# sonbui25/Multimodal-Aspect-Category-Sentiment-Analysis

Hardware: AMD Instinct MI355X
Metric: train samples/sec (fwd+bwd+step) FCMF seq128x36ROI (higher is better)
Workload: dtype bf16; 1 GPU; FCMF-base fine-tune step, BASELINE configs[1]: batch 64 reviews x 6 aspects per GPU, seq 128, 7 images x (49 patches + 36 ROIs), precomputed ResNet-152 features, dropout 0.1, clip 1.0 + 4-group AdamW + linear schedule; global_batch=64, per_gpu_batch=64, seq_len=128, parallelism=dp1, sample_unit=1 review = 6 aspect forwards

## Files before the change

### include/fcmf_hip.h

```cpp
#ifndef FCMF_HIP_H
#define FCMF_HIP_H
#include <stdint.h>

#ifdef __cplusplus
extern "C" {
#endif

#define FCMF_OK 0
#define FCMF_ERR_ARG (-1)
#define FCMF_ERR_LAUNCH (-2)
#define FCMF_ERR_UNSUPPORTED (-3)
#define FCMF_ERR_COMM (-4)

#define FCMF_F32 0
#define FCMF_BF16 1
#define FCMF_F64 2

#define FCMF_EPI_NONE 0
#define FCMF_EPI_GELU 1
#define FCMF_EPI_TANH 2
#define FCMF_EPI_DGELU 3
#define FCMF_EPI_DTANH 4
#define FCMF_EPI_ADD 5

int fcmf_abi_version(void);
const char* fcmf_build_info(void);

typedef struct fcmf_gemm_ctx fcmf_gemm_ctx;
int fcmf_gemm_ctx_create(fcmf_gemm_ctx** ctx);
int fcmf_gemm_ctx_destroy(fcmf_gemm_ctx* ctx);
int fcmf_gemm_ctx_set_workspace(fcmf_gemm_ctx* ctx, void* ptr, int64_t bytes);
int fcmf_gemm_ctx_tune(fcmf_gemm_ctx* ctx, int force_tile, int kb, int num_cus, int64_t nt_min_bytes);
const char* fcmf_gemm_ctx_last_kernel(const fcmf_gemm_ctx* ctx);

int fcmf_gemm(fcmf_gemm_ctx* ctx, const void* A, const void* B, void* C, const float* bias, void* aux, float* colsum,
              int M, int N, int K, int64_t lda, int64_t ldb, int64_t ldc,
              int trans_a, int trans_b, int in_dtype, int out_dtype,
              int epilogue, int accumulate, void* stream);

int fcmf_quant_fp8_rows(const void* x, int64_t ldx, void* q, int64_t ldq, float* scale, int rows, int K, int dtype, void* stream);
int fcmf_gemm_fp8(fcmf_gemm_ctx* ctx, const void* A, const float* sa, const void* B, const float* sb, void* C,
                  const float* bias, void* aux, float* colsum, int M, int N, int K, int64_t lda, int64_t ldb, int64_t ldc,
                  int epilogue, void* stream);

int fcmf_colsum(const void* X, float* out, int M, int N, int64_t ldx, int dtype,
                int accumulate, void* stream);

typedef struct {
  int dtype, G, heads, d, R, T1, T2, group_div;
  int64_t q_sg, q_sr, k1_sg, k1_st, k2_sg, k2_sr, k2_st, o_sg, o_sr;
  const void *q, *k1, *v1, *k2, *v2;
  const float* mask;
  const float* bias;
  float scale, dropout_p;
  uint64_t seed;
  int causal, head_quirk;
} fcmf_attn_desc;

int fcmf_attn_small_fwd(const fcmf_attn_desc* desc , void* out, float* lse, void* stream);
int fcmf_attn_small_bwd(const fcmf_attn_desc* desc , const void* out, const void* dout,
                        const float* lse, void* dq, void* dk1, void* dv1, void* dk2, void* dv2,
                        float* dbias, void* stream);
int fcmf_attn_small_bwd_grouped(const fcmf_attn_desc* desc, const void* out, const void* dout,
                                const float* lse, void* dq, void* dk1, void* dv1, void* dk2, void* dv2,
                                float* dbias, float* scratch, int64_t scratch_bytes, void* stream);

int fcmf_attn_mfma_fwd(const void* q, const void* k, const void* v, const float* mask,
                       void* out, float* lse, int G, int heads, int Tq, int Tk,
                       int64_t ldq, int64_t ldk, int64_t ldo, float scale,
                       float dropout_p, uint64_t seed, void* stream);
int fcmf_attn_mfma_bwd(const void* q, const void* k, const void* v, const float* mask,
                       const void* out, const void* dout, const float* lse,
                       void* dq, void* dk, void* dv, int G, int heads, int Tq, int Tk,
                       int64_t ldq, int64_t ldk, int64_t ldo, float scale,
                       float dropout_p, uint64_t seed, float* colsum, void* stream);

int fcmf_attn_probs(const fcmf_attn_desc* desc , float* probs, int64_t p_sg, int64_t p_sh, void* stream);
int fcmf_attn_mfma_probs(const void* q, const void* k, const float* mask, float* probs, int G, int heads,
                         int Tq, int Tk, int64_t ldq, int64_t ldk, int64_t p_sg, int64_t p_sh,
                         float scale, void* stream);

int fcmf_add_ln_fwd(const void* x, const void* res, int64_t res_stride, const float* gamma,
                    const float* beta, void* y, void* z, float* mean, float* rstd,
                    int rows, int H, float eps, float dropout_p, uint64_t seed, int dtype,
                    void* stream);
int fcmf_add_ln_bwd(const void* dy, const void* z, const float* gamma, const float* mean,
                    const float* rstd, void* dz, void* dx, float* dgamma, float* dbeta, float* dxsum,
                    float* workspace, int rows, int H, float dropout_p, uint64_t seed, int dtype,
                    void* stream);
int fcmf_add_ln_fwd_fp8(const void* x, const void* res, int64_t res_stride, const float* gamma, const float* beta, void* y,
                        void* z, float* mean, float* rstd, int rows, int H, float eps, float dropout_p, uint64_t seed,
                        int dtype, void* q8, float* qscale, void* stream);
int fcmf_add_ln_bwd_fp8(const void* dy, const void* z, const float* gamma, const float* mean, const float* rstd, void* dz,
                        void* dx, float* dgamma, float* dbeta, float* dxsum, float* workspace, int rows, int H,
                        float dropout_p, uint64_t seed, int dtype, void* q8, float* qscale, void* stream);
int64_t fcmf_add_ln_bwd_workspace(int rows, int H);

int fcmf_position_ids(const int64_t* ids, int64_t* pos, int nseq, int S, int pad_id, void* stream);
int fcmf_embed_ln_fwd(const int64_t* ids, const int64_t* pos, const int64_t* type_ids,
                      const float* word, const float* pos_table, const float* type_table,
                      const float* gamma, const float* beta, void* y, void* z, float* mean,
                      float* rstd, int ntok, int H, float eps, float dropout_p, uint64_t seed,
                      int dtype, void* stream);
int fcmf_embed_bwd(const void* dz, const int64_t* ids, const int64_t* pos, const int64_t* type_ids,
                   float* dword, float* dpos, float* dtype_table, int ntok, int H, int pad_id,
                   int dtype, void* stream);
int fcmf_embed_pos_bwd(const void* dz, const int64_t* pos, float* dpos, int nseq, int S, int H, int pad_id,
                       int dtype, void* stream);
int fcmf_embed_pos_type_bwd(const void* dz, const int64_t* pos, const int64_t* type_ids, float* dpos,
                            float* dtype_table, int nseq, int S, int H, int pad_id, int dtype, void* stream);

#define FCMF_BOX_FAST_TRIG 0x100
int fcmf_box_bias_fwd(const void* coords, int coord_dtype, const float* dim_mat, const float* wg_w,
                      const float* wg_b, float* bias, int G, int N, int heads, void* stream);
int fcmf_box_bias_bwd(const void* coords, int coord_dtype, const float* dim_mat, const float* wg_w,
                      const float* wg_b, const float* dbias, float* dwg_w, float* dwg_b, int G, int N,
                      int heads, void* stream);
int fcmf_box_embedding(const void* coords, int coord_dtype, const float* dim_mat, float* emb, int G,
                       int N, void* stream);

int fcmf_xent_fwd(const void* logits, int64_t ld, const int64_t* labels, float* loss_rows,
                  float* nvalid, int n, int C, int64_t ignore_index, int dtype, void* stream);
int fcmf_xent_bwd(const void* logits, int64_t ld, const int64_t* labels, void* dlogits,
                  int64_t ldd, const float* scale_ptr, float extra_scale, int n, int C,
                  int64_t ignore_index, int dtype, void* stream);

int fcmf_xent_mean(const float* loss_rows, const int64_t* labels, int n, int64_t ignore_index,
                   float mult, float* out2, void* stream);

int fcmf_bce_logits(const void* logits, int64_t ld, const float* target, int64_t ldt, int n, int C, const float* dloss,
                    float* loss, void* dlogits, int64_t ldd, float* probs, int dtype, void* stream);

int fcmf_additive_mask(const int64_t* mask, int64_t ld, float* out, int rows, int cols, float value,
                       void* stream);

int fcmf_cast(const void* src, void* dst, int64_t n, int src_dtype, int dst_dtype, void* stream);
int fcmf_cast_transpose(const float* src, void* dst, int rows, int cols, void* stream);
int fcmf_multi_cast_transpose(const int64_t* src_ptrs, const int64_t* dst_ptrs, const int32_t* dims,
                              const int32_t* tile_desc, int ntiles, void* stream);
int fcmf_dropout(const void* x, void* y, int64_t n, float p, uint64_t seed, int dtype, void* stream);
int fcmf_act_bwd(const void* dy, const void* aux, void* out, int64_t n, int kind, int dtype,
                 void* stream);
int fcmf_sum_axis(const void* in, void* out, int64_t outer, int reps, int64_t inner, int dtype,
                  void* stream);

int fcmf_embed_scale_fwd(const int64_t* ids, const float* weight, const float* pos_table, void* out, int n, int H, int S,
                         int64_t V, float scale, int dtype, void* stream);
int fcmf_embed_scale_bwd(const void* dy, const int64_t* ids, float* dweight, int n, int H, int64_t V, int32_t* oob_count,
                         float scale, int dtype, void* stream);
int fcmf_head_gather(const void* slot, void* out, int64_t ldo, int G, int T, int heads, int d, int dtype, void* stream);

int fcmf_multi_sumsq(const int64_t* g_ptrs, const int64_t* sizes, const int32_t* chunk_tensor,
                     const int64_t* chunk_offset, int nchunks, int chunk_size,
                     double* sumsq , double* per_tensor ,
                     void* stream);
int fcmf_multi_adamw(const int64_t* p_ptrs, const int64_t* g_ptrs, const int64_t* m_ptrs,
                     const int64_t* v_ptrs, const int64_t* bf16_ptrs, const int64_t* sizes,
                     const int32_t* group_of, const int32_t* chunk_tensor,
                     const int64_t* chunk_offset, int nchunks, int chunk_size,
                     const float* lr , const float* wd , int ngroups,
                     float beta1, float beta2, float eps, int step, const double* sumsq,
                     float max_norm, void* stream);
int fcmf_bertadam(float* p, const float* g, float* m, float* v, int64_t n, float lr_scheduled,
                  float beta1, float beta2, float eps, float weight_decay, float max_grad_norm,
                  double* scratch, void* stream);

int fcmf_conv_im2col(const void* src, int src_dtype, void* dst, int dst_dtype, int N, int H, int W, int C,
                     int64_t sn, int64_t sh, int64_t sw, int64_t sc, int kh, int kw, int stride, int pad,
                     int Kpad, void* stream);
int64_t fcmf_bn_stats_workspace(int64_t rows_per_group, int groups, int C);
int fcmf_bn_stats(const void* x, double* sums, int64_t rows_per_group, int groups, int C, int dtype, void* stream);
int fcmf_bn_finalize(const double* sums, const float* gamma, const float* beta, float* running_mean,
                     float* running_var, float* scale, float* shift, float* mean_out, float* rstd_out, int C,
                     int groups, int64_t count, float momentum, float eps, void* stream);
int fcmf_bn_apply(const void* x, const void* res, void* y, const float* scale, const float* shift, int64_t rows,
                  int C, int64_t rows_per_group, int relu, int dtype, void* stream);
int fcmf_bn_apply_pad(const void* x, const void* res, void* y_padded, const float* scale, const float* shift,
                      int64_t rows, int C, int64_t rows_per_group, int relu, int H, int W, int pad, int dtype, void* stream);
int fcmf_bn_finalize_apply(const void* x, const void* res, void* y, const double* sums, const float* gamma, const float* beta,
                           float* running_mean, float* running_var, float* mean_out, float* rstd_out, int C, int groups,
                           int64_t rows_per_group, float momentum, float eps, int relu, int H, int W, int pad, int dtype, void* stream);
int fcmf_conv_gemm(fcmf_gemm_ctx* ctx, const void* x, const void* w, void* y, int n, int Hp, int Wp, int C, int Ho, int Wo,
                   int kh, int kw, int stride, int Cout, void* stream);
int fcmf_gemm_colblocks(fcmf_gemm_ctx* ctx, const void* A, const void* B, float* C, int M, int N, int K, int64_t lda,
                        int64_t ldb, int64_t ldc, int trans_a, int trans_b, int col_block, int64_t col_block_stride,
                        int accumulate, void* stream);

int fcmf_gemm_dw_batched(fcmf_gemm_ctx* ctx, int count, const void* const* A, const void* const* B, void* const* C, int M, int N, int K,
                         int64_t lda, int64_t ldb, int64_t ldc, int accumulate, void* stream);
int fcmf_conv_gemm_runs(fcmf_gemm_ctx* ctx, const void* x, const void* w, void* y, float* stats, int n, int Hp, int Wp, int pix, int run,
                        int Ho, int Wo, int kh, int stride, int Cout, void* stream);
int fcmf_pack_rgb0(const void* src, int src_dtype, void* dst, int N, int H, int W, int64_t sn, int64_t sh, int64_t sw, int64_t sc,
                   int pad, int Wp, void* stream);
int fcmf_gemm_colstats(fcmf_gemm_ctx* ctx, const void* A, const void* B, void* C, float* stats, int M, int N, int K, int64_t lda,
                       int64_t ldb, int64_t ldc, void* stream);
int fcmf_conv_gemm_colstats(fcmf_gemm_ctx* ctx, const void* x, const void* w, void* y, float* stats, int n, int Hp, int Wp, int C,
                            int Ho, int Wo, int kh, int kw, int stride, int Cout, void* stream);
int fcmf_gemm_colstats_block_rows(const fcmf_gemm_ctx* ctx, int M, int N, int K);
int fcmf_bn_stats_blocks(const float* blockstats, double* sums, int64_t rows_per_group, int groups, int C, int block_rows, void* stream);
int fcmf_maxpool3x3s2(const void* x, void* y, int N, int H, int W, int C, int dtype, void* stream);
int fcmf_adaptive_avgpool(const void* x, float* y, int N, int H, int W, int C, int oh, int ow, int layout,
                          int dtype, void* stream);

int fcmf_bn_bwd(const void* g, const void* z, const void* y, const float* mean, const float* rstd, const float* gamma,
                double* sums, void* dy, void* gres, float* dgamma, float* dbeta, int64_t rows_per_group, int groups,
                int C, int training, int dtype, void* stream);
int fcmf_conv_col2im(const void* dA, void* dX, int N, int H, int W, int C, int kh, int kw, int stride, int pad,
                     int Kpad, int dtype, void* stream);
int fcmf_maxpool3x3s2_bwd(const void* x, const void* dy, void* dx, int N, int H, int W, int C, int dtype, void* stream);
int fcmf_adaptive_avgpool_bwd(const float* dy, void* dx, int N, int H, int W, int C, int oh, int ow, int layout,
                              int dtype, void* stream);

typedef struct {
  int64_t offset;
  int H, W;
  int64_t sC, sH, sW;
  int r0, r1, c0, c1;
  int flip, reserved;
} fcmf_crop_desc;

int fcmf_crop_resize_normalize(const uint8_t* src, int64_t src_bytes, const fcmf_crop_desc* descs, int n, int max_rows, int S,
                               const float* mean, const float* std, float* scratch, int64_t scratch_bytes, void* out,
                               int dtype, void* stream);

#define FCMF_DP_UNIQUE_ID_BYTES 128
int fcmf_dp_unique_id(void* out_host);
int fcmf_dp_comm_create(void** comm, const void* unique_id_host, int nranks, int rank);
int fcmf_dp_comm_destroy(void* comm);
int fcmf_dp_allreduce_bucket(void* comm, void* buf, int64_t count, int dtype, int average, void* stream);

#ifdef __cplusplus
}
#endif
#endif
```

### multimodal-aspect-category-sentiment-analysis_amd/csrc/gemm.hip

```cpp
#include "common.h"
#include <cstdio>

struct GemmParams {
  const void* A; const void* B; void* C; const float* bias; void* aux;
  int M, N, K;
  int64_t lda, ldb, ldc;
  int epilogue, accumulate, ksplit, ktiles_per_split;
  unsigned a_bytes, b_bytes;
  unsigned c_bytes;
  float* colsum;
  int tiles, total_items;
  float* ws;
  int nt_out;
  const float* sa; const float* sb;
  int cv_C, cv_logC, cv_Hp, cv_Wp, cv_Ho, cv_Wo, cv_kw, cv_inv_kw, cv_stride;
  float* colstats;
  int cv_logP;
  int tiles_per_mat;
};
constexpr int BATCH_MAX = 32;
struct BatchPtrs { const void* A[BATCH_MAX]; const void* B[BATCH_MAX]; void* C[BATCH_MAX]; };

__device__ __forceinline__ int64_t conv_row_base(const GemmParams& p, int row) {
  const int hw = p.cv_Ho * p.cv_Wo, n = row / hw, rem = row - n * hw, oy = rem / p.cv_Wo, ox = rem - oy * p.cv_Wo;
// ... 1082 lines not shown
  int kchunk;
};

template <typename TI, typename TC>
__global__ __launch_bounds__(256) void gemm_generic_kernel(GenericParams p) {
  constexpr int GT = 64, GK = 16, LDT = GT + 4;
  __shared__ float As[GK][LDT];
  __shared__ float Bs[GK][LDT];
  const int tid = threadIdx.x, lane = tid & 63, wave = tid >> 6;
  const int wm = wave >> 1, wn = wave & 1;
  const int i0 = blockIdx.y * GT, j0 = blockIdx.x * GT;
  const TI* A = reinterpret_cast<const TI*>(p.A);
  const TI* B = reinterpret_cast<const TI*>(p.B);
  const bool a_kfast = (p.a_sk == 1), b_kfast = (p.b_sk == 1);

  f32x4 acc[2][2];
#pragma unroll
  for (int a = 0; a < 2; ++a)
#pragma unroll
    for (int b = 0; b < 2; ++b) acc[a][b] = f32x4{0.f, 0.f, 0.f, 0.f};

  const int kbeg = p.kchunk > 0 ? blockIdx.z * p.kchunk : 0;
  const int kend = p.kchunk > 0 ? min(p.K, kbeg + p.kchunk) : p.K;
  for (int k0 = kbeg; k0 < kend; k0 += GK) {
#pragma unroll
    for (int it = 0; it < 4; ++it) {
      int e = tid + 256 * it;
      int ia, ka, jb, kb;
      if (a_kfast) { ka = e & 15; ia = e >> 4; } else { ia = e & 63; ka = e >> 6; }
      if (b_kfast) { kb = e & 15; jb = e >> 4; } else { jb = e & 63; kb = e >> 6; }
      float va = 0.f, vb = 0.f;
      if (i0 + ia < p.M && k0 + ka < kend) va = to_f32<TI>(A[(int64_t)(i0 + ia) * p.a_si + (int64_t)(k0 + ka) * p.a_sk]);
      if (j0 + jb < p.N && k0 + kb < kend) vb = to_f32<TI>(B[(int64_t)(j0 + jb) * p.b_sj + (int64_t)(k0 + kb) * p.b_sk]);
      As[ka][ia] = va;
      Bs[kb][jb] = vb;
    }
    __syncthreads();
#pragma unroll
    for (int k4 = 0; k4 < GK / 4; ++k4) {
      float a[2], b[2];
#pragma unroll
      for (int f = 0; f < 2; ++f) {
        a[f] = As[k4 * 4 + (lane >> 4)][wm * 32 + f * 16 + (lane & 15)];
        b[f] = Bs[k4 * 4 + (lane >> 4)][wn * 32 + f * 16 + (lane & 15)];
      }
#pragma unroll
      for (int fi = 0; fi < 2; ++fi)
#pragma unroll
        for (int fj = 0; fj < 2; ++fj)
          acc[fi][fj] = __builtin_amdgcn_mfma_f32_16x16x4f32(a[fi], b[fj], acc[fi][fj], 0, 0, 0);
    }
    __syncthreads();
  }
  TC* C = reinterpret_cast<TC*>(p.C);
  TC* AUX = reinterpret_cast<TC*>(p.aux);
#pragma unroll
  for (int fi = 0; fi < 2; ++fi)
#pragma unroll
    for (int fj = 0; fj < 2; ++fj)
#pragma unroll
      for (int r = 0; r < 4; ++r) {
        int i = i0 + wm * 32 + fi * 16 + (lane >> 4) * 4 + r;
        int j = j0 + wn * 32 + fj * 16 + (lane & 15);
        if (i >= p.M || j >= p.N) continue;
        float v = acc[fi][fj][r];
        if (p.bias) v += p.bias[j];
        int64_t off = (int64_t)i * p.ldc + j;
        if (p.epilogue != FCMF_EPI_NONE) {
          float a = 0.f;
          if (p.epilogue == FCMF_EPI_GELU) { if (AUX) AUX[off] = from_f32<TC>(v); }
          else if (p.epilogue != FCMF_EPI_TANH) a = to_f32<TC>(AUX[off]);
          v = apply_epilogue(v, p.epilogue, a);
        }
        if constexpr (sizeof(TC) == 4) {
          if (p.kchunk > 0) { atomicAdd(reinterpret_cast<float*>(C) + off, v); continue; }
        }
        if (p.accumulate) v += to_f32<TC>(C[off]);
        C[off] = from_f32<TC>(v);
        if (p.colsum) atomicAdd(p.colsum + j, v);
      }
}

template <typename T>
__global__ __launch_bounds__(256) void colsum_kernel(const T* __restrict__ X, float* __restrict__ out, int M, int N,
                                                     int64_t ldx, int rows_per_block, int vec) {
  __shared__ float4 red[4][64];
  const int lane = threadIdx.x & 63, wave = threadIdx.x >> 6;
  const int col = blockIdx.x * 256 + lane * 4;
  const int r0 = blockIdx.y * rows_per_block;
  const int r1 = min(M, r0 + rows_per_block);
  float4 s = make_float4(0.f, 0.f, 0.f, 0.f);
  if (vec && col + 3 < N) {
    int r = r0 + wave;
    for (; r + 12 < r1; r += 16) {
      const float4 v0 = Vec4<T>::load(X + (int64_t)r * ldx + col), v1 = Vec4<T>::load(X + (int64_t)(r + 4) * ldx + col);
      const float4 v2 = Vec4<T>::load(X + (int64_t)(r + 8) * ldx + col), v3 = Vec4<T>::load(X + (int64_t)(r + 12) * ldx + col);
      s.x += (v0.x + v1.x) + (v2.x + v3.x); s.y += (v0.y + v1.y) + (v2.y + v3.y);
      s.z += (v0.z + v1.z) + (v2.z + v3.z); s.w += (v0.w + v1.w) + (v2.w + v3.w);
    }
    for (; r < r1; r += 4) {
      const float4 v = Vec4<T>::load(X + (int64_t)r * ldx + col);
      s.x += v.x; s.y += v.y; s.z += v.z; s.w += v.w;
    }
  } else if (col < N) {
    for (int r = r0 + wave; r < r1; r += 4) {
      const T* p = X + (int64_t)r * ldx + col;
      s.x += to_f32<T>(p[0]);
      if (col + 1 < N) s.y += to_f32<T>(p[1]);
      if (col + 2 < N) s.z += to_f32<T>(p[2]);
      if (col + 3 < N) s.w += to_f32<T>(p[3]);
    }
  }
  red[wave][lane] = s;
  __syncthreads();
  if (wave == 0 && col < N) {
    const float4 a = red[0][lane], b = red[1][lane], c = red[2][lane], d = red[3][lane];
    atomicAdd(out + col, a.x + b.x + c.x + d.x);
    if (col + 1 < N) atomicAdd(out + col + 1, a.y + b.y + c.y + d.y);
    if (col + 2 < N) atomicAdd(out + col + 2, a.z + b.z + c.z + d.z);
    if (col + 3 < N) atomicAdd(out + col + 3, a.w + b.w + c.w + d.w);
  }
}

template <bool A_TR, bool B_TR, typename TC, int EPI>
__global__ __launch_bounds__(512, 1) void gemm_bf16_tile256_kernel(GemmParams p) {
  gemm_bf16_tile256_body<A_TR, B_TR, TC, EPI, 8, 32>(p);
}
__global__ __launch_bounds__(512, 1) void gemm_bf16_tile256k64_n128_kernel(GemmParams p) {
  gemm_bf16_tile256_body<false, false, bf16_t, FCMF_EPI_NONE, 4, 64, false, false, 2>(p);
}
__global__ __launch_bounds__(512, 1) void gemm_bf16_tile256k64_n64_kernel(GemmParams p) {
  gemm_bf16_tile256_body<false, false, bf16_t, FCMF_EPI_NONE, 2, 64, false, false, 1>(p);
}
__global__ __launch_bounds__(512, 1) void gemm_bf16_dw_batched_kernel(GemmParams p, BatchPtrs bp) {
  gemm_bf16_tile256_body<true, true, float, FCMF_EPI_NONE, 8, 32, false, true>(p, &bp);
}
template <bool B_TR, int EPI>
__global__ __launch_bounds__(512, 1) void gemm_bf16_tile192_kernel(GemmParams p) {
  gemm_bf16_tile256_body<false, B_TR, bf16_t, EPI, 6, 32>(p);
}
template <int EPI>
__global__ __launch_bounds__(512, 1) void gemm_bf16_tile256k64_kernel(GemmParams p) {
  gemm_bf16_tile256_body<false, false, bf16_t, EPI, 8, 64>(p);
}
template <int EPI>
__global__ __launch_bounds__(512, 1) void gemm_bf16_tile192k64_kernel(GemmParams p) {
  gemm_bf16_tile256_body<false, false, bf16_t, EPI, 6, 64>(p);
}

template <int EPI>
__global__ __launch_bounds__(512, 1) void gemm_fp8_tile192_kernel(GemmParams p) {
  gemm_bf16_tile256_body<false, false, bf16_t, EPI, 6, 64, true>(p);
}

__global__ __launch_bounds__(256) void splitk_reduce_frag_kernel(const float* __restrict__ ws, float* __restrict__ C, int M, int N,
                                                                 int64_t ldc, int ksplit, int tiles, int tiles_n, int accumulate,
                                                                 int cblk, int64_t cblk_stride) {
  const int64_t total = (int64_t)tiles * (GB * GB / 4);
  for (int64_t i = (int64_t)blockIdx.x * 256 + threadIdx.x; i < total; i += (int64_t)gridDim.x * 256) {
    const int tile = (int)(i >> 14), r = (int)(i & 16383);
    const int lane = r & 63, frag = (r >> 6) & 31, wave = r >> 11;
    const int fj = frag >> 3, fi = frag & 7, wm = wave >> 2, wn = wave & 3;
    const int row = (tile / tiles_n) * GB + wm * 128 + fi * 16 + (lane & 15);
    const int col = (tile % tiles_n) * GB + wn * 64 + fj * 16 + (lane >> 4) * 4;
    if (row >= M || col >= N) continue;
    float* c = cblk ? C + (int64_t)(col / cblk) * cblk_stride + (int64_t)row * ldc + (col % cblk) : C + (int64_t)row * ldc + col;
    f32x4 s = accumulate ? *reinterpret_cast<const f32x4*>(c) : f32x4{0.f, 0.f, 0.f, 0.f};
#pragma unroll 4
    for (int z = 0; z < ksplit; ++z) s += *reinterpret_cast<const f32x4*>(ws + ((int64_t)z * tiles + tile) * (GB * GB) + (int64_t)r * 4);
    *reinterpret_cast<f32x4*>(c) = s;
  }
}

__global__ __launch_bounds__(256) void splitk_reduce_frag_batched_kernel(const float* __restrict__ ws, BatchPtrs bp, int tiles_per_mat, int M,
                                                                         int N, int64_t ldc, int ksplit, int tiles, int tiles_n,
                                                                         int accumulate) {
  const int64_t total = (int64_t)tiles * (GB * GB / 4);
  for (int64_t i = (int64_t)blockIdx.x * 256 + threadIdx.x; i < total; i += (int64_t)gridDim.x * 256) {
    const int tile = (int)(i >> 14), r = (int)(i & 16383);
    const int b = tile / tiles_per_mat, local = tile - b * tiles_per_mat;
    const int lane = r & 63, frag = (r >> 6) & 31, wave = r >> 11;
    const int fj = frag >> 3, fi = frag & 7, wm = wave >> 2, wn = wave & 3;
    const int row = (local / tiles_n) * GB + wm * 128 + fi * 16 + (lane & 15);
    const int col = (local % tiles_n) * GB + wn * 64 + fj * 16 + (lane >> 4) * 4;
    if (row >= M || col >= N) continue;
    float* c = reinterpret_cast<float*>(bp.C[b]) + (int64_t)row * ldc + col;
    f32x4 s = accumulate ? *reinterpret_cast<const f32x4*>(c) : f32x4{0.f, 0.f, 0.f, 0.f};
#pragma unroll 4
    for (int z = 0; z < ksplit; ++z) s += *reinterpret_cast<const f32x4*>(ws + ((int64_t)z * tiles + tile) * (GB * GB) + (int64_t)r * 4);
    *reinterpret_cast<f32x4*>(c) = s;
  }
}

__global__ __launch_bounds__(256) void splitk_reduce_kernel(const float* __restrict__ ws, float* __restrict__ C, int M, int N,
                                                            int64_t ldc, int ksplit, int accumulate) {
  const int64_t total4 = (int64_t)M * N / 4;
  for (int64_t i = (int64_t)blockIdx.x * 256 + threadIdx.x; i < total4; i += (int64_t)gridDim.x * 256) {
    const int64_t e = i * 4, row = e / N, col = e - row * N;
    f32x4 s = accumulate ? *reinterpret_cast<const f32x4*>(C + row * ldc + col) : f32x4{0.f, 0.f, 0.f, 0.f};
#pragma unroll 4
    for (int z = 0; z < ksplit; ++z) s += *reinterpret_cast<const f32x4*>(ws + (int64_t)z * M * N + e);
    *reinterpret_cast<f32x4*>(C + row * ldc + col) = s;
  }
}
// ... 552 lines not shown
    for (int i = 0; i < count; ++i) {
      a.A = A[i]; a.B = B[i]; a.C = C[i];
      const int rc = gemm_impl(ctx, a, stream);
      if (rc != FCMF_OK) return rc;
    }
    return FCMF_OK;
  }
  const int tpm = ((M + GB - 1) / GB) * ((N + GB - 1) / GB), nk = (K + 31) / 32;
  const int chunks = (count + BATCH_MAX - 1) / BATCH_MAX;
  for (int c = 0, first = 0; c < chunks; ++c) {
    const int n = (count - first + (chunks - c) - 1) / (chunks - c);
    BatchPtrs bp{};
    for (int i = 0; i < n; ++i) { bp.A[i] = A[first + i]; bp.B[i] = B[first + i]; bp.C[i] = C[first + i]; }
    a.A = bp.A[0]; a.B = bp.B[0]; a.C = bp.C[0];
    GemmPlan pl;
    plan_begin(&pl, a, GK_DW_BATCHED);
    pl.tm = 256; pl.batch = &bp;
    pl.p = base_params(a, 2);
    pl.p.c_bytes = 0;
    pl.p.tiles_per_mat = tpm;
    const int tiles = n * tpm;
    plan_persistent_launch(&pl, persistent_list(cfg, pl.p, tiles, nk, batched_ksplit(cfg, tiles, nk), false));
    if (pl.p.ksplit > 1) { pl.p.ws = cfg.ws; plan_frag_reduce(&pl, RED_FRAG_BATCHED); }
    snprintf(pl.name, sizeof pl.name, "gemm_bf16_dw_batched_kernel");
    const int rc = run_named(ctx, pl, stream);
    if (rc != FCMF_OK) return rc;
    first += n;
  }
  return FCMF_OK;
}

struct ConvShape { int n, Hp, Wp, C, Ho, Wo, kh, kw, stride, Cout; };
static int conv_gemm_impl(fcmf_gemm_ctx* ctx, const void* x, const void* w, void* y, float* colstats, const ConvShape& s, void* stream) {
  const int n = s.n, Hp = s.Hp, Wp = s.Wp, C = s.C, Ho = s.Ho, Wo = s.Wo, kh = s.kh, kw = s.kw, stride = s.stride, Cout = s.Cout;
  if (!x || !w || !y || n <= 0 || Hp <= 0 || Wp <= 0 || C <= 0 || Ho <= 0 || Wo <= 0 || kh <= 0 || kw <= 0 || stride <= 0 || Cout <= 0)
    return FCMF_ERR_ARG;
  if ((C & (C - 1)) || C < 64 || kh * kw > 64) return FCMF_ERR_UNSUPPORTED;
  if ((Ho - 1) * stride + kh > Hp || (Wo - 1) * stride + kw > Wp) return FCMF_ERR_ARG;
  const int64_t in_bytes = (int64_t)n * Hp * Wp * C * 2, M = (int64_t)n * Ho * Wo;
  if (in_bytes >= (1ll << 31) || M >= (1ll << 31)) return FCMF_ERR_UNSUPPORTED;
  int logC = 0;
  while ((1 << logC) < C) ++logC;
  const ConvGeom cv{C, logC, Hp, Wp, Ho, Wo, kw, stride, in_bytes, logC};
  GemmArgs a = plain_bf16_args(x, w, y, (int)M, Cout, kh * kw * C);
  a.cv = &cv; a.colstats = colstats;
  return gemm_impl(ctx, a, stream);
}
extern "C" int fcmf_conv_gemm(fcmf_gemm_ctx* ctx, const void* x, const void* w, void* y, int n, int Hp, int Wp, int C, int Ho,
                              int Wo, int kh, int kw, int stride, int Cout, void* stream) {
  return conv_gemm_impl(ctx, x, w, y, nullptr, ConvShape{n, Hp, Wp, C, Ho, Wo, kh, kw, stride, Cout}, stream);
}

extern "C" int fcmf_gemm_colstats(fcmf_gemm_ctx* ctx, const void* A, const void* B, void* C, float* stats, int M, int N, int K,
                                  int64_t lda, int64_t ldb, int64_t ldc, void* stream) {
  if (!stats) return FCMF_ERR_ARG;
  GemmArgs a = plain_bf16_args(A, B, C, M, N, K);
  a.lda = lda; a.ldb = ldb; a.ldc = ldc; a.colstats = stats;
  return gemm_impl(ctx, a, stream);
}
extern "C" int fcmf_conv_gemm_colstats(fcmf_gemm_ctx* ctx, const void* x, const void* w, void* y, float* stats, int n, int Hp, int Wp,
                                       int C, int Ho, int Wo, int kh, int kw, int stride, int Cout, void* stream) {
  if (!stats) return FCMF_ERR_ARG;
  return conv_gemm_impl(ctx, x, w, y, stats, ConvShape{n, Hp, Wp, C, Ho, Wo, kh, kw, stride, Cout}, stream);
}

extern "C" int fcmf_conv_gemm_runs(fcmf_gemm_ctx* ctx, const void* x, const void* w, void* y, float* stats, int n, int Hp, int Wp, int pix,
                                   int run, int Ho, int Wo, int kh, int stride, int Cout, void* stream) {
  if (!x || !w || !y || n <= 0 || Hp <= 0 || Wp <= 0 || pix <= 0 || run <= 0 || Ho <= 0 || Wo <= 0 || kh <= 0 || stride <= 0 || Cout <= 0)
    return FCMF_ERR_ARG;
  if ((pix & (pix - 1)) || (run & (run - 1)) || run < 32 || run % pix || kh > 64 || (stride * pix) % 8) return FCMF_ERR_UNSUPPORTED;
  if ((Ho - 1) * stride + kh > Hp) return FCMF_ERR_ARG;
  const int64_t in_elems = (int64_t)n * Hp * Wp * pix, M = (int64_t)n * Ho * Wo;
  if ((((int64_t)(n - 1) * Hp + (Ho - 1) * stride + kh - 1) * Wp + (int64_t)(Wo - 1) * stride) * pix + run > in_elems) return FCMF_ERR_ARG;
  if (in_elems * 2 >= (1ll << 31) || M >= (1ll << 31)) return FCMF_ERR_UNSUPPORTED;
  int logC = 0, logP = 0;
  while ((1 << logC) < run) ++logC;
  while ((1 << logP) < pix) ++logP;
  const ConvGeom cv{run, logC, Hp, Wp, Ho, Wo, 1, stride, in_elems * 2, logP};
  GemmArgs a = plain_bf16_args(x, w, y, (int)M, Cout, kh * run);
  a.cv = &cv; a.colstats = stats;
  return gemm_impl(ctx, a, stream);
}

extern "C" int fcmf_colsum(const void* X, float* out, int M, int N, int64_t ldx, int dtype, int accumulate,
                           void* stream) {
  if (!X || !out || M < 0 || N <= 0) return FCMF_ERR_ARG;
  hipStream_t st = reinterpret_cast<hipStream_t>(stream);
  if (!accumulate) { if (hipMemsetAsync(out, 0, sizeof(float) * N, st) != hipSuccess) return FCMF_ERR_LAUNCH; }
  if (M == 0) return FCMF_OK;
  const int vec = (ldx % 4 == 0) && ((reinterpret_cast<uintptr_t>(X) & 15) == 0);
  const int bx = (N + 255) / 256;
  int rpb = 256;
  if ((int64_t)((M + 255) / 256) * bx < 256) {
    rpb = (int)(((int64_t)M * bx / 1024 + 3) & ~3ll);
    rpb = rpb < 16 ? 16 : (rpb > 256 ? 256 : rpb);
  }
  dim3 grid(bx, (M + rpb - 1) / rpb);
  if (dtype == FCMF_F32) hipLaunchKernelGGL((colsum_kernel<float>), grid, dim3(256), 0, st, (const float*)X, out, M, N, ldx, rpb, vec);
  else if (dtype == FCMF_BF16) hipLaunchKernelGGL((colsum_kernel<bf16_t>), grid, dim3(256), 0, st, (const bf16_t*)X, out, M, N, ldx, rpb, vec);
  else return FCMF_ERR_UNSUPPORTED;
  FCMF_CHECK_LAUNCH();
  return FCMF_OK;
}
```

### multimodal-aspect-category-sentiment-analysis_amd/csrc/misc.hip

```cpp
#include "common.h"

template <typename T>
__global__ __launch_bounds__(256) void xent_fwd_kernel(const T* __restrict__ logits, int64_t ld,
                                                       const int64_t* __restrict__ labels, float* __restrict__ loss_rows,
                                                       float* __restrict__ nvalid, int n, int C, int64_t ignore_index) {
  const int lane = threadIdx.x & 63;
  const int row = blockIdx.x * 4 + (threadIdx.x >> 6);
  if (row >= n) return;
  const int64_t lab = labels[row];
  if (lab == ignore_index) { if (lane == 0) loss_rows[row] = 0.f; return; }
  const T* lr = logits + (int64_t)row * ld;
  float m = -INFINITY;
  for (int c = lane; c < C; c += 64) m = fmaxf(m, to_f32<T>(lr[c]));
  m = wave_max(m);
  float s = 0.f;
  for (int c = lane; c < C; c += 64) s += __expf(to_f32<T>(lr[c]) - m);
  s = wave_sum(s);
  if (lane == 0) {
    loss_rows[row] = (m + __logf(s)) - to_f32<T>(lr[lab]);
    if (nvalid) atomicAdd(nvalid, 1.0f);
  }
}

__global__ __launch_bounds__(256) void xent_mean_kernel(const float* __restrict__ loss_rows, const int64_t* __restrict__ labels,
// ... 216 lines not shown
  const int tx = threadIdx.x & 63, ty = threadIdx.x >> 6;
#pragma unroll
  for (int i = 0; i < 16; ++i) {
    const int r = r0 + ty * 16 + i, c = c0 + tx;
    tile[ty * 16 + i][tx] = (r < R && c < C) ? src[(int64_t)r * C + c] : 0.f;
  }
  __syncthreads();
#pragma unroll
  for (int i = 0; i < 16; ++i) {
    const int c = c0 + ty * 16 + i, r = r0 + tx;
    if (c < C && r < R) dst[(int64_t)c * R + r] = (bf16_t)tile[tx][ty * 16 + i];
  }
}

template <typename T>
__global__ __launch_bounds__(256) void dropout_kernel(const T* __restrict__ x, T* __restrict__ y, int64_t n, float p,
                                                      float inv_keep, uint64_t seed) {
  for (int64_t i = (int64_t)blockIdx.x * 256 + threadIdx.x; i < n; i += (int64_t)gridDim.x * 256)
    y[i] = from_f32<T>(to_f32<T>(x[i]) * dropout_mult(seed, (uint64_t)i, p, inv_keep));
}

template <typename T>
__global__ __launch_bounds__(256) void act_bwd_kernel(const T* __restrict__ dy, const T* __restrict__ aux, T* __restrict__ out,
                                                      int64_t n, int kind) {
  for (int64_t i = (int64_t)blockIdx.x * 256 + threadIdx.x; i < n; i += (int64_t)gridDim.x * 256) {
    const float a = to_f32<T>(aux[i]), d = to_f32<T>(dy[i]);
    out[i] = from_f32<T>(kind == 0 ? d * (1.0f - a * a) : d * dgelu_f(a));
  }
}

template <typename T>
__global__ __launch_bounds__(256) void sum_axis_kernel(const T* __restrict__ in, T* __restrict__ out, int64_t outer,
                                                       int reps, int64_t inner) {
  const int64_t total = outer * inner;
  for (int64_t i = (int64_t)blockIdx.x * 256 + threadIdx.x; i < total; i += (int64_t)gridDim.x * 256) {
    const int64_t o = i / inner, c = i - o * inner;
    float s = 0.f;
    for (int r = 0; r < reps; ++r) s += to_f32<T>(in[(o * reps + r) * inner + c]);
    out[i] = from_f32<T>(s);
  }
}

__global__ __launch_bounds__(256) void multi_sumsq_kernel(const int64_t* __restrict__ g_ptrs, const int64_t* __restrict__ sizes,
                                                          const int32_t* __restrict__ chunk_tensor,
                                                          const int64_t* __restrict__ chunk_offset, int chunk_size,
                                                          double* __restrict__ sumsq, double* __restrict__ per_tensor) {
  __shared__ double red[4];
  const int t = chunk_tensor[blockIdx.x];
  const int64_t off = chunk_offset[blockIdx.x];
  const float* g = reinterpret_cast<const float*>(g_ptrs[t]) + off;
  int64_t n = sizes[t] - off;
  if (n > chunk_size) n = chunk_size;
  double s = 0.0;
  const bool vec = (reinterpret_cast<uintptr_t>(g) & 15) == 0;
  if (vec) {
    const int64_t n4 = n >> 2;
    for (int64_t i = threadIdx.x; i < n4; i += 256) {
      const float4 v = *reinterpret_cast<const float4*>(g + i * 4);
      s += (double)v.x * v.x + (double)v.y * v.y + (double)v.z * v.z + (double)v.w * v.w;
    }
    for (int64_t i = n4 * 4 + threadIdx.x; i < n; i += 256) s += (double)g[i] * g[i];
  } else {
    for (int64_t i = threadIdx.x; i < n; i += 256) s += (double)g[i] * g[i];
  }
  s = wave_sum_d(s);
  if ((threadIdx.x & 63) == 0) red[threadIdx.x >> 6] = s;
  __syncthreads();
  if (threadIdx.x == 0) {
    const double tot = red[0] + red[1] + red[2] + red[3];
    if (sumsq) atomicAdd(sumsq, tot);
    if (per_tensor) atomicAdd(per_tensor + t, tot);
  }
}

struct AdamArgs {
  const int64_t *p_ptrs, *g_ptrs, *m_ptrs, *v_ptrs, *bf16_ptrs, *sizes;
  const int32_t *group_of, *chunk_tensor;
  const int64_t* chunk_offset;
  int chunk_size;
  float lr[8], wd[8];
  float beta1, beta2, eps, bc1, bc2_sqrt;
  const double* sumsq;
  float max_norm;
};

__global__ __launch_bounds__(256) void multi_adamw_kernel(AdamArgs a) {
  const int t = a.chunk_tensor[blockIdx.x];
  const int64_t off = a.chunk_offset[blockIdx.x];
  float* p = reinterpret_cast<float*>(a.p_ptrs[t]) + off;
  const float* g = reinterpret_cast<const float*>(a.g_ptrs[t]) + off;
  float* m = reinterpret_cast<float*>(a.m_ptrs[t]) + off;
  float* v = reinterpret_cast<float*>(a.v_ptrs[t]) + off;
  bf16_t* sh = a.bf16_ptrs && a.bf16_ptrs[t] ? reinterpret_cast<bf16_t*>(a.bf16_ptrs[t]) + off : nullptr;
  int64_t n = a.sizes[t] - off;
  if (n > a.chunk_size) n = a.chunk_size;
  const int grp = a.group_of[t];
  const float lr = a.lr[grp], wd = a.wd[grp];
  float coef = 1.0f;
  if (a.max_norm > 0.f && a.sumsq) {
    const float tn = (float)sqrt(*a.sumsq);
    coef = fminf(1.0f, a.max_norm / (tn + 1e-6f));
  }
  const float step_size = lr / a.bc1;
  typedef float f4 __attribute__((ext_vector_type(4)));
  int64_t i0 = 0;
  if (((reinterpret_cast<uintptr_t>(p) | reinterpret_cast<uintptr_t>(g) | reinterpret_cast<uintptr_t>(m) | reinterpret_cast<uintptr_t>(v)) & 15) == 0 &&
      (!sh || (reinterpret_cast<uintptr_t>(sh) & 7) == 0)) {
    const int64_t n4 = n >> 2;
    for (int64_t i = threadIdx.x; i < n4; i += 256) {
      const f4 g4 = __builtin_nontemporal_load(reinterpret_cast<const f4*>(g) + i) * coef;
      f4 p4 = reinterpret_cast<const f4*>(p)[i] * (1.0f - lr * wd);
      const f4 m4 = a.beta1 * __builtin_nontemporal_load(reinterpret_cast<const f4*>(m) + i) + (1.0f - a.beta1) * g4;
      const f4 v4 = a.beta2 * __builtin_nontemporal_load(reinterpret_cast<const f4*>(v) + i) + (1.0f - a.beta2) * g4 * g4;
#pragma unroll
      for (int e = 0; e < 4; ++e) p4[e] -= step_size * (m4[e] / (sqrtf(v4[e]) / a.bc2_sqrt + a.eps));
      reinterpret_cast<f4*>(p)[i] = p4;
      __builtin_nontemporal_store(m4, reinterpret_cast<f4*>(m) + i);
      __builtin_nontemporal_store(v4, reinterpret_cast<f4*>(v) + i);
      if (sh) {
        bf16x4 o;
        o[0] = (bf16_t)p4[0]; o[1] = (bf16_t)p4[1]; o[2] = (bf16_t)p4[2]; o[3] = (bf16_t)p4[3];
        reinterpret_cast<bf16x4*>(sh)[i] = o;
      }
    }
    i0 = n4 << 2;
  }
  for (int64_t i = i0 + threadIdx.x; i < n; i += 256) {
    const float gi = g[i] * coef;
    float pi = p[i] * (1.0f - lr * wd);
    const float mi = a.beta1 * m[i] + (1.0f - a.beta1) * gi;
    const float vi = a.beta2 * v[i] + (1.0f - a.beta2) * gi * gi;
    const float denom = sqrtf(vi) / a.bc2_sqrt + a.eps;
    pi -= step_size * (mi / denom);
    p[i] = pi; m[i] = mi; v[i] = vi;
    if (sh) sh[i] = (bf16_t)pi;
  }
}

__global__ __launch_bounds__(256) void sumsq_kernel(const float* __restrict__ g, int64_t n, double* __restrict__ out) {
  __shared__ double red[4];
  double s = 0.0;
  for (int64_t i = (int64_t)blockIdx.x * 256 + threadIdx.x; i < n; i += (int64_t)gridDim.x * 256) s += (double)g[i] * g[i];
  s = wave_sum_d(s);
  if ((threadIdx.x & 63) == 0) red[threadIdx.x >> 6] = s;
  __syncthreads();
  if (threadIdx.x == 0) atomicAdd(out, red[0] + red[1] + red[2] + red[3]);
}

__global__ __launch_bounds__(256) void bertadam_kernel(float* __restrict__ p, const float* __restrict__ g, float* __restrict__ m,
                                                       float* __restrict__ v, int64_t n, float lr, float b1, float b2, float e,
                                                       float wd, float max_norm, const double* __restrict__ sumsq) {
  float coef = 1.0f;
  if (max_norm > 0.f) coef = fminf(1.0f, max_norm / ((float)sqrt(*sumsq) + 1e-6f));
  for (int64_t i = (int64_t)blockIdx.x * 256 + threadIdx.x; i < n; i += (int64_t)gridDim.x * 256) {
    const float gi = g[i] * coef;
    const float mi = b1 * m[i] + (1.0f - b1) * gi;
    const float vi = b2 * v[i] + (1.0f - b2) * gi * gi;
    float upd = mi / (sqrtf(vi) + e);
    if (wd > 0.f) upd += wd * p[i];
    p[i] -= lr * upd;
    m[i] = mi; v[i] = vi;
  }
}

static int grid_for(int64_t n, int per) {
  int64_t b = (n + per - 1) / per;
  return (int)(b > 4096 ? 4096 : (b < 1 ? 1 : b));
}

extern "C" int fcmf_abi_version(void) { return 4; }
extern "C" const char* fcmf_build_info(void) { return "libfcmf_hip gfx950 (CDNA4, wave64) abi 4"; }

extern "C" int fcmf_xent_fwd(const void* logits, int64_t ld, const int64_t* labels, float* loss_rows, float* nvalid, int n,
                             int C, int64_t ignore_index, int dtype, void* stream) {
  if (!logits || !labels || !loss_rows || n < 0 || C <= 0) return FCMF_ERR_ARG;
  if (n == 0) return FCMF_OK;
  hipStream_t st = reinterpret_cast<hipStream_t>(stream);
  if (C >= 1024) {
    const int es = dtype == FCMF_F32 ? 4 : 2;
    const int vec = ((reinterpret_cast<uintptr_t>(logits) & 15) == 0) && ((ld * es) % 16 == 0);
    if (dtype == FCMF_F32) hipLaunchKernelGGL((xent_fwd_wide_kernel<float>), dim3(n), dim3(256), 0, st, (const float*)logits, ld, labels, loss_rows, nvalid, C, ignore_index, vec);
    else if (dtype == FCMF_BF16) hipLaunchKernelGGL((xent_fwd_wide_kernel<bf16_t>), dim3(n), dim3(256), 0, st, (const bf16_t*)logits, ld, labels, loss_rows, nvalid, C, ignore_index, vec);
    else return FCMF_ERR_UNSUPPORTED;
    FCMF_CHECK_LAUNCH();
    return FCMF_OK;
  }
  dim3 grid((n + 3) / 4);
  if (dtype == FCMF_F32) hipLaunchKernelGGL((xent_fwd_kernel<float>), grid, dim3(256), 0, st, (const float*)logits, ld, labels, loss_rows, nvalid, n, C, ignore_index);
  else if (dtype == FCMF_BF16) hipLaunchKernelGGL((xent_fwd_kernel<bf16_t>), grid, dim3(256), 0, st, (const bf16_t*)logits, ld, labels, loss_rows, nvalid, n, C, ignore_index);
  else return FCMF_ERR_UNSUPPORTED;
  FCMF_CHECK_LAUNCH();
  return FCMF_OK;
}

extern "C" int fcmf_xent_mean(const float* loss_rows, const int64_t* labels, int n, int64_t ignore_index, float mult,
                              float* out2, void* stream) {
  if (!loss_rows || !labels || !out2 || n < 0) return FCMF_ERR_ARG;
  hipLaunchKernelGGL(xent_mean_kernel, dim3(1), dim3(256), 0, reinterpret_cast<hipStream_t>(stream), loss_rows, labels, n,
                     ignore_index, mult, out2);
  FCMF_CHECK_LAUNCH();
  return FCMF_OK;
}

extern "C" int fcmf_bce_logits(const void* logits, int64_t ld, const float* target, int64_t ldt, int n, int C, const float* dloss,
                               float* loss, void* dlogits, int64_t ldd, float* probs, int dtype, void* stream) {
  if (!logits || (!target && (loss || dlogits)) || n < 0 || C <= 0 || ld < C || (target && ldt < C) || (dlogits && ldd < C))
    return FCMF_ERR_ARG;
  if (n == 0) return FCMF_OK;
  hipStream_t st = reinterpret_cast<hipStream_t>(stream);
  if (dtype == FCMF_F32)
    hipLaunchKernelGGL((bce_logits_kernel<float>), dim3(1), dim3(256), 0, st, (const float*)logits, ld, target, ldt, n, C, dloss, loss,
                       (float*)dlogits, ldd, probs);
  else if (dtype == FCMF_BF16)
    hipLaunchKernelGGL((bce_logits_kernel<bf16_t>), dim3(1), dim3(256), 0, st, (const bf16_t*)logits, ld, target, ldt, n, C, dloss, loss,
                       (bf16_t*)dlogits, ldd, probs);
  else return FCMF_ERR_UNSUPPORTED;
// ... 135 lines not shown
}
template <typename T>
__global__ __launch_bounds__(256) void head_gather_kernel(const T* __restrict__ slot, T* __restrict__ out, int64_t ldo, int G, int Tn,
                                                          int heads, int d) {
  const int d4 = d >> 2;
  const int64_t total = (int64_t)G * Tn * heads * d4;
  for (int64_t i = (int64_t)blockIdx.x * 256 + threadIdx.x; i < total; i += (int64_t)gridDim.x * 256) {
    const int c = (int)(i % d4) * 4;
    const int64_t r = i / d4;
    const int h = (int)(r % heads);
    const int64_t gt = r / heads;
    const int g = (int)(gt / Tn);
    float4 acc = make_float4(0.f, 0.f, 0.f, 0.f);
    for (int sl = 0; sl < heads; ++sl) {
      if ((int)(((int64_t)sl * G + g) % heads) != h) continue;
      const float4 v = Vec4<T>::load(slot + (gt * heads + sl) * d + c);
      acc.x += v.x; acc.y += v.y; acc.z += v.z; acc.w += v.w;
    }
    Vec4<T>::store(out + gt * ldo + (int64_t)h * d + c, acc);
  }
}

extern "C" int fcmf_embed_scale_fwd(const int64_t* ids, const float* weight, const float* pos_table, void* out, int n, int H, int S,
                                    int64_t V, float scale, int dtype, void* stream) {
  if (!ids || !weight || !out || n < 0 || H <= 0 || H % 4 || S <= 0 || V <= 0) return FCMF_ERR_ARG;
  if (n == 0) return FCMF_OK;
  hipStream_t st = reinterpret_cast<hipStream_t>(stream);
  dim3 grid((n + 3) / 4);
  if (dtype == FCMF_F32) hipLaunchKernelGGL((embed_scale_fwd_kernel<float>), grid, dim3(256), 0, st, ids, weight, pos_table, (float*)out, n, H, S, scale, V);
  else if (dtype == FCMF_BF16) hipLaunchKernelGGL((embed_scale_fwd_kernel<bf16_t>), grid, dim3(256), 0, st, ids, weight, pos_table, (bf16_t*)out, n, H, S, scale, V);
  else return FCMF_ERR_UNSUPPORTED;
  FCMF_CHECK_LAUNCH();
  return FCMF_OK;
}

extern "C" int fcmf_embed_scale_bwd(const void* dy, const int64_t* ids, float* dweight, int n, int H, int64_t V, int32_t* oob_count,
                                    float scale, int dtype, void* stream) {
  if (!dy || !ids || !dweight || n < 0 || H <= 0 || H % 4 || V <= 0) return FCMF_ERR_ARG;
  if (n == 0) return FCMF_OK;
  hipStream_t st = reinterpret_cast<hipStream_t>(stream);
  dim3 grid((n + 3) / 4);
  if (dtype == FCMF_F32) hipLaunchKernelGGL((embed_scale_bwd_kernel<float>), grid, dim3(256), 0, st, (const float*)dy, ids, dweight, n, H, scale, V, oob_count);
  else if (dtype == FCMF_BF16) hipLaunchKernelGGL((embed_scale_bwd_kernel<bf16_t>), grid, dim3(256), 0, st, (const bf16_t*)dy, ids, dweight, n, H, scale, V, oob_count);
  else return FCMF_ERR_UNSUPPORTED;
  FCMF_CHECK_LAUNCH();
  return FCMF_OK;
}

extern "C" int fcmf_head_gather(const void* slot, void* out, int64_t ldo, int G, int T, int heads, int d, int dtype, void* stream) {
  if (!slot || !out || G < 0 || T <= 0 || heads <= 0 || d <= 0 || d % 4 || ldo < (int64_t)heads * d) return FCMF_ERR_ARG;
  if (G == 0) return FCMF_OK;
  hipStream_t st = reinterpret_cast<hipStream_t>(stream);
  dim3 grid(grid_for((int64_t)G * T * heads * (d / 4), 256));
  if (dtype == FCMF_F32) hipLaunchKernelGGL((head_gather_kernel<float>), grid, dim3(256), 0, st, (const float*)slot, (float*)out, ldo, G, T, heads, d);
  else if (dtype == FCMF_BF16) hipLaunchKernelGGL((head_gather_kernel<bf16_t>), grid, dim3(256), 0, st, (const bf16_t*)slot, (bf16_t*)out, ldo, G, T, heads, d);
  else return FCMF_ERR_UNSUPPORTED;
  FCMF_CHECK_LAUNCH();
  return FCMF_OK;
}

extern "C" int fcmf_sum_axis(const void* in, void* out, int64_t outer, int reps, int64_t inner, int dtype, void* stream) {
  if (!in || !out || outer < 0 || reps <= 0 || inner <= 0) return FCMF_ERR_ARG;
  if (outer == 0) return FCMF_OK;
  hipStream_t st = reinterpret_cast<hipStream_t>(stream);
  dim3 grid(grid_for(outer * inner, 256));
  if (dtype == FCMF_F32) hipLaunchKernelGGL((sum_axis_kernel<float>), grid, dim3(256), 0, st, (const float*)in, (float*)out, outer, reps, inner);
  else if (dtype == FCMF_BF16) hipLaunchKernelGGL((sum_axis_kernel<bf16_t>), grid, dim3(256), 0, st, (const bf16_t*)in, (bf16_t*)out, outer, reps, inner);
  else return FCMF_ERR_UNSUPPORTED;
  FCMF_CHECK_LAUNCH();
  return FCMF_OK;
}

extern "C" int fcmf_multi_sumsq(const int64_t* g_ptrs, const int64_t* sizes, const int32_t* chunk_tensor,
                                const int64_t* chunk_offset, int nchunks, int chunk_size, double* sumsq,
                                double* per_tensor, void* stream) {
  if (!g_ptrs || !sizes || !chunk_tensor || !chunk_offset || nchunks < 0 || chunk_size <= 0) return FCMF_ERR_ARG;
  if (nchunks == 0) return FCMF_OK;
  hipLaunchKernelGGL(multi_sumsq_kernel, dim3(nchunks), dim3(256), 0, reinterpret_cast<hipStream_t>(stream), g_ptrs, sizes,
                     chunk_tensor, chunk_offset, chunk_size, sumsq, per_tensor);
  FCMF_CHECK_LAUNCH();
  return FCMF_OK;
}

extern "C" int fcmf_multi_adamw(const int64_t* p_ptrs, const int64_t* g_ptrs, const int64_t* m_ptrs, const int64_t* v_ptrs,
                                const int64_t* bf16_ptrs, const int64_t* sizes, const int32_t* group_of,
                                const int32_t* chunk_tensor, const int64_t* chunk_offset, int nchunks, int chunk_size,
                                const float* lr, const float* wd, int ngroups, float beta1, float beta2, float eps, int step,
                                const double* sumsq, float max_norm, void* stream) {
  if (!p_ptrs || !g_ptrs || !m_ptrs || !v_ptrs || !sizes || !group_of || !chunk_tensor || !chunk_offset || !lr || !wd)
    return FCMF_ERR_ARG;
  if (ngroups <= 0 || ngroups > 8 || step < 1 || chunk_size <= 0 || nchunks < 0) return FCMF_ERR_ARG;
  if (nchunks == 0) return FCMF_OK;
  AdamArgs a{};
  a.p_ptrs = p_ptrs; a.g_ptrs = g_ptrs; a.m_ptrs = m_ptrs; a.v_ptrs = v_ptrs; a.bf16_ptrs = bf16_ptrs; a.sizes = sizes;
  a.group_of = group_of; a.chunk_tensor = chunk_tensor; a.chunk_offset = chunk_offset; a.chunk_size = chunk_size;
  for (int i = 0; i < ngroups; ++i) { a.lr[i] = lr[i]; a.wd[i] = wd[i]; }
  a.beta1 = beta1; a.beta2 = beta2; a.eps = eps;
  a.bc1 = (float)(1.0 - pow((double)beta1, (double)step));
  a.bc2_sqrt = (float)sqrt(1.0 - pow((double)beta2, (double)step));
  a.sumsq = sumsq; a.max_norm = max_norm;
  hipLaunchKernelGGL(multi_adamw_kernel, dim3(nchunks), dim3(256), 0, reinterpret_cast<hipStream_t>(stream), a);
  FCMF_CHECK_LAUNCH();
  return FCMF_OK;
}

extern "C" int fcmf_bertadam(float* p, const float* g, float* m, float* v, int64_t n, float lr_scheduled, float beta1,
                             float beta2, float eps, float weight_decay, float max_grad_norm, double* scratch,
                             void* stream) {
  if (!p || !g || !m || !v || n < 0) return FCMF_ERR_ARG;
  if (max_grad_norm > 0.f && !scratch) return FCMF_ERR_ARG;
  if (n == 0) return FCMF_OK;
  hipStream_t st = reinterpret_cast<hipStream_t>(stream);
  dim3 grid(grid_for(n, 1024));
  if (max_grad_norm > 0.f) {
    if (hipMemsetAsync(scratch, 0, sizeof(double), st) != hipSuccess) return FCMF_ERR_LAUNCH;
    hipLaunchKernelGGL(sumsq_kernel, grid, dim3(256), 0, st, g, n, scratch);
  }
  hipLaunchKernelGGL(bertadam_kernel, grid, dim3(256), 0, st, p, g, m, v, n, lr_scheduled, beta1, beta2, eps, weight_decay,
                     max_grad_norm, scratch);
  FCMF_CHECK_LAUNCH();
  return FCMF_OK;
}
```

### multimodal-aspect-category-sentiment-analysis_amd/csrc/norm.hip

```cpp
#include "common.h"

constexpr int LN_MAXP = 8;

template <typename T, int NP>
__global__ __launch_bounds__(256) void add_ln_fwd_kernel(const T* __restrict__ x, const T* __restrict__ res,
                                                         int64_t res_stride, const float* __restrict__ gamma,
                                                         const float* __restrict__ beta, T* __restrict__ y,
                                                         T* __restrict__ z, float* __restrict__ mean,
                                                         float* __restrict__ rstd, int rows, int H, float eps,
                                                         float p, uint64_t seed, unsigned char* __restrict__ q8 = nullptr,
                                                         float* __restrict__ qscale = nullptr) {
  const int lane = threadIdx.x & 63;
  const float inv_keep = p > 0.f ? 1.0f / (1.0f - p) : 1.0f;
  typedef typename Vec4<T>::raw Raw;
  const int stride = gridDim.x * 4;
  int row = blockIdx.x * 4 + (threadIdx.x >> 6);
  Raw nx[NP], nr[NP];
  auto fetch = [&](int r) {
    if (r < rows) {
#pragma unroll
      for (int i = 0; i < NP; ++i) {
        const int c = (i * 64 + lane) * 4;
        if (c < H) {
          nx[i] = Vec4<T>::load_raw(x + (int64_t)r * H + c);
// ... 145 lines not shown
      if (c < H) {
        float4 o;
        o.x = rs * (gy[i].x - s1 - xh[i].x * s2); o.y = rs * (gy[i].y - s1 - xh[i].y * s2);
        o.z = rs * (gy[i].z - s1 - xh[i].z * s2); o.w = rs * (gy[i].w - s1 - xh[i].w * s2);
        Vec4<T>::store(dz + (int64_t)row * H + c, o);
        if (dx) {
          const uint64_t base = (uint64_t)row * H + c;
          float dm[4];
          dropout_mult4(seed, base, p, inv_keep, dm);
          o.x *= dm[0]; o.y *= dm[1]; o.z *= dm[2]; o.w *= dm[3];
          Vec4<T>::store(dx + (int64_t)row * H + c, o);
        }
        ax[i].x += o.x; ax[i].y += o.y; ax[i].z += o.z; ax[i].w += o.w;
        if (q8) {
          o.x = to_f32<T>(from_f32<T>(o.x)); o.y = to_f32<T>(from_f32<T>(o.y)); o.z = to_f32<T>(from_f32<T>(o.z)); o.w = to_f32<T>(from_f32<T>(o.w));
          gy[i] = o;
        }
      }
    }
    if (q8) {
      float amax = 0.f;
#pragma unroll
      for (int i = 0; i < NP; ++i)
        if ((i * 64 + lane) * 4 < H) amax = fmaxf(amax, fmaxf(fmaxf(fabsf(gy[i].x), fabsf(gy[i].y)), fmaxf(fabsf(gy[i].z), fabsf(gy[i].w))));
      amax = wave_max(amax);
      const float sc = amax > 0.f ? amax * (1.0f / 448.0f) : 1.0f, inv = 1.0f / sc;
      if (lane == 0) qscale[row] = sc;
#pragma unroll
      for (int i = 0; i < NP; ++i) {
        const int c = (i * 64 + lane) * 4;
        if (c < H) {
          int w8 = 0;
          w8 = __builtin_amdgcn_cvt_pk_fp8_f32(gy[i].x * inv, gy[i].y * inv, w8, false);
          w8 = __builtin_amdgcn_cvt_pk_fp8_f32(gy[i].z * inv, gy[i].w * inv, w8, true);
          *reinterpret_cast<int*>(q8 + (int64_t)row * H + c) = w8;
        }
      }
    }
  }
#pragma unroll
  for (int step = 0; step < 2; ++step) {
    const int half = step == 0 ? 2 : 1;
    if (w >= half && w < 2 * half) {
#pragma unroll
      for (int i = 0; i < NP; ++i) { red[w - half][0][i][lane] = ag[i]; red[w - half][1][i][lane] = ab[i]; red[w - half][2][i][lane] = ax[i]; }
    }
    __syncthreads();
    if (w < half) {
#pragma unroll
      for (int i = 0; i < NP; ++i) {
        float4 a = red[w][0][i][lane], b = red[w][1][i][lane], c2 = red[w][2][i][lane];
        ag[i].x += a.x; ag[i].y += a.y; ag[i].z += a.z; ag[i].w += a.w;
        ab[i].x += b.x; ab[i].y += b.y; ab[i].z += b.z; ab[i].w += b.w;
        ax[i].x += c2.x; ax[i].y += c2.y; ax[i].z += c2.z; ax[i].w += c2.w;
      }
    }
    __syncthreads();
  }
  if (w == 0) {
#pragma unroll
    for (int i = 0; i < NP; ++i) {
      const int c = (i * 64 + lane) * 4;
      if (c < H) {
        if (partial) {
          float* pb = partial + (int64_t)blockIdx.x * 3 * H + c;
          *reinterpret_cast<float4*>(pb) = ag[i];
          *reinterpret_cast<float4*>(pb + H) = ab[i];
          *reinterpret_cast<float4*>(pb + 2 * H) = ax[i];
        } else {
          atomicAdd(dgamma + c + 0, ag[i].x); atomicAdd(dgamma + c + 1, ag[i].y);
          atomicAdd(dgamma + c + 2, ag[i].z); atomicAdd(dgamma + c + 3, ag[i].w);
          atomicAdd(dbeta + c + 0, ab[i].x); atomicAdd(dbeta + c + 1, ab[i].y);
          atomicAdd(dbeta + c + 2, ab[i].z); atomicAdd(dbeta + c + 3, ab[i].w);
          if (dxsum) {
            atomicAdd(dxsum + c + 0, ax[i].x); atomicAdd(dxsum + c + 1, ax[i].y);
            atomicAdd(dxsum + c + 2, ax[i].z); atomicAdd(dxsum + c + 3, ax[i].w);
          }
        }
      }
    }
  }
}

__global__ __launch_bounds__(256) void ln_partial_reduce_kernel(const float* __restrict__ partial, int nblocks, int H,
                                                                float* __restrict__ dgamma, float* __restrict__ dbeta,
                                                                float* __restrict__ dxsum) {
  __shared__ float red[4][64];
  const int lane = threadIdx.x & 63, w = threadIdx.x >> 6;
  const int col = blockIdx.x * 64 + lane, which = blockIdx.y;
  float* out = which == 0 ? dgamma : (which == 1 ? dbeta : dxsum);
  if (!out) return;
  const int per = (nblocks + gridDim.z - 1) / gridDim.z;
  const int b0 = blockIdx.z * per, b1 = min(nblocks, b0 + per);
  float s = 0.f;
  if (col < H)
    for (int b = b0 + w; b < b1; b += 4) s += partial[((int64_t)b * 3 + which) * H + col];
  red[w][lane] = s;
  __syncthreads();
  if (w == 0 && col < H) atomicAdd(out + col, red[0][lane] + red[1][lane] + red[2][lane] + red[3][lane]);
}

__global__ __launch_bounds__(64) void position_ids_kernel(const int64_t* __restrict__ ids, int64_t* __restrict__ pos,
                                                          int S, int pad_id) {
  const int lane = threadIdx.x;
  const int64_t* row = ids + (int64_t)blockIdx.x * S;
  int64_t* out = pos + (int64_t)blockIdx.x * S;
  int running = 0;
  for (int t0 = 0; t0 < S; t0 += 64) {
    const int t = t0 + lane;
    const bool nz = t < S && row[t] != pad_id;
    const unsigned long long b = __ballot(nz);
    const int incl = __popcll(b & ((lane == 63) ? ~0ull : ((1ull << (lane + 1)) - 1)));
    if (t < S) out[t] = nz ? (int64_t)(running + incl + pad_id) : (int64_t)pad_id;
    running += __popcll(b);
  }
}

template <typename T, int NP>
__global__ __launch_bounds__(256) void embed_ln_fwd_kernel(const int64_t* __restrict__ ids, const int64_t* __restrict__ pos,
                                                           const int64_t* __restrict__ tt, const float* __restrict__ word,
                                                           const float* __restrict__ ptab, const float* __restrict__ ttab,
                                                           const float* __restrict__ gamma, const float* __restrict__ beta,
                                                           T* __restrict__ y, T* __restrict__ z, float* __restrict__ mean,
                                                           float* __restrict__ rstd, int ntok, int H, float eps, float p,
                                                           uint64_t seed) {
  const int lane = threadIdx.x & 63;
  const int row = blockIdx.x * 4 + (threadIdx.x >> 6);
  if (row >= ntok) return;
  const float* wr = word + ids[row] * H;
  const float* pr = ptab + pos[row] * H;
  const float* tr = ttab + (tt ? tt[row] : 0) * H;
  float4 v[NP];
  float s = 0.f;
#pragma unroll
  for (int i = 0; i < NP; ++i) {
    const int c = (i * 64 + lane) * 4;
    if (c < H) {
      const float4 a = *reinterpret_cast<const float4*>(wr + c);
      const float4 b = *reinterpret_cast<const float4*>(tr + c);
      const float4 d = *reinterpret_cast<const float4*>(pr + c);
      float4 o; o.x = (a.x + b.x) + d.x; o.y = (a.y + b.y) + d.y; o.z = (a.z + b.z) + d.z; o.w = (a.w + b.w) + d.w;
      v[i] = o;
      s += o.x + o.y + o.z + o.w;
    }
  }
  const float mu = wave_sum(s) / (float)H;
  float q = 0.f;
#pragma unroll
  for (int i = 0; i < NP; ++i) {
    const int c = (i * 64 + lane) * 4;
    if (c < H) {
      float dx = v[i].x - mu, dy = v[i].y - mu, dz = v[i].z - mu, dw = v[i].w - mu;
      q += dx * dx + dy * dy + dz * dz + dw * dw;
    }
  }
  const float rs = rsqrtf(wave_sum(q) / (float)H + eps);
  if (lane == 0) { mean[row] = mu; rstd[row] = rs; }
  const float inv_keep = p > 0.f ? 1.0f / (1.0f - p) : 1.0f;
#pragma unroll
  for (int i = 0; i < NP; ++i) {
    const int c = (i * 64 + lane) * 4;
    if (c < H) {
      if (z) Vec4<T>::store(z + (int64_t)row * H + c, v[i]);
      const float4 g = *reinterpret_cast<const float4*>(gamma + c);
      const float4 b = *reinterpret_cast<const float4*>(beta + c);
      float4 o;
      o.x = (v[i].x - mu) * rs * g.x + b.x; o.y = (v[i].y - mu) * rs * g.y + b.y;
      o.z = (v[i].z - mu) * rs * g.z + b.z; o.w = (v[i].w - mu) * rs * g.w + b.w;
      if (p > 0.f) {
        const uint64_t base = (uint64_t)row * H + c;
        float dm[4];
        dropout_mult4(seed, base, p, inv_keep, dm);
        o.x *= dm[0]; o.y *= dm[1]; o.z *= dm[2]; o.w *= dm[3];
      }
      Vec4<T>::store(y + (int64_t)row * H + c, o);
    }
  }
}

template <typename T>
__global__ __launch_bounds__(256) void embed_bwd_kernel(const T* __restrict__ dz, const int64_t* __restrict__ ids,
                                                        const int64_t* __restrict__ pos, const int64_t* __restrict__ tt,
// ... 87 lines not shown
#pragma unroll
        for (int j = 0; j < E; ++j) atomicAdd(dpos + id * H + c0 + j, (float)v[j]);
      }
    }
#pragma unroll
    for (int j = 0; j < E; ++j) { rp[slot * H + c0 + j] = acc[j]; rt[slot * H + c0 + j] = tsum[j]; }
    if (cg == 0) p0s[slot] = (int)p0;
  }
  __syncthreads();
  for (int c = tid; c < H; c += 256) {
    float ts = 0.f;
    for (int k = 0; k < slots; ++k) ts += rt[k * H + c];
    if (dtt) atomicAdd(dtt + c, ts);
    for (int k = 0; k < slots; ++k) {
      const int pk = p0s[k];
      if (pk < 0) continue;
      bool first = true;
      for (int m = 0; m < k; ++m) first = first && p0s[m] != pk;
      if (!first) continue;
      float ps = 0.f;
      for (int m = k; m < slots; ++m)
        if (p0s[m] == pk) ps += rp[m * H + c];
      atomicAdd(dpos + (int64_t)pk * H + c, ps);
    }
  }
}

#define LN_DISPATCH_T(T, H)                         \
  do {                                              \
    const int np__ = ((H) + 255) / 256;             \
    if (np__ <= 1) LAUNCH_(T, 1);                   \
    else if (np__ <= 2) LAUNCH_(T, 2);              \
    else if (np__ <= 3) LAUNCH_(T, 3);              \
    else if (np__ <= 4) LAUNCH_(T, 4);              \
    else LAUNCH_(T, 8);                             \
  } while (0)
#define LN_DISPATCH(dtype, H)                                     \
  do {                                                            \
    if ((dtype) == FCMF_F32) LN_DISPATCH_T(float, H);             \
    else LN_DISPATCH_T(bf16_t, H);                                \
  } while (0)

static int add_ln_fwd_impl(const void* x, const void* res, int64_t res_stride, const float* gamma, const float* beta, void* y,
                           void* z, float* mean, float* rstd, int rows, int H, float eps, float dropout_p, uint64_t seed,
                           int dtype, void* stream, void* q8, float* qscale);
extern "C" int fcmf_add_ln_fwd(const void* x, const void* res, int64_t res_stride, const float* gamma,
                               const float* beta, void* y, void* z, float* mean, float* rstd, int rows, int H,
                               float eps, float dropout_p, uint64_t seed, int dtype, void* stream) {
  return add_ln_fwd_impl(x, res, res_stride, gamma, beta, y, z, mean, rstd, rows, H, eps, dropout_p, seed, dtype, stream, nullptr, nullptr);
}
extern "C" int fcmf_add_ln_fwd_fp8(const void* x, const void* res, int64_t res_stride, const float* gamma,
                                   const float* beta, void* y, void* z, float* mean, float* rstd, int rows, int H,
                                   float eps, float dropout_p, uint64_t seed, int dtype, void* q8, float* qscale, void* stream) {
  if (!q8 || !qscale) return FCMF_ERR_ARG;
  return add_ln_fwd_impl(x, res, res_stride, gamma, beta, y, z, mean, rstd, rows, H, eps, dropout_p, seed, dtype, stream, q8, qscale);
}
static int add_ln_fwd_impl(const void* x, const void* res, int64_t res_stride, const float* gamma, const float* beta, void* y,
                           void* z, float* mean, float* rstd, int rows, int H, float eps, float dropout_p, uint64_t seed,
                           int dtype, void* stream, void* q8, float* qscale) {
  if (!x || !gamma || !beta || !y || !mean || !rstd || rows < 0 || H <= 0) return FCMF_ERR_ARG;
  if (H % 4 != 0 || H > LN_MAXP * 256 || (res && res_stride % 4 != 0)) return FCMF_ERR_UNSUPPORTED;
  if (rows == 0) return FCMF_OK;
  hipStream_t st = reinterpret_cast<hipStream_t>(stream);
  const int nblk = (rows + 3) / 4;
  dim3 grid(nblk > 2048 ? 2048 : nblk);
  if (dtype != FCMF_F32 && dtype != FCMF_BF16) return FCMF_ERR_UNSUPPORTED;
#define LAUNCH_(T, NP) hipLaunchKernelGGL((add_ln_fwd_kernel<T, NP>), grid, dim3(256), 0, st, (const T*)x, (const T*)res, \
    res_stride, gamma, beta, (T*)y, (T*)z, mean, rstd, rows, H, eps, dropout_p, seed, (unsigned char*)q8, qscale)
  LN_DISPATCH(dtype, H);
#undef LAUNCH_
  FCMF_CHECK_LAUNCH();
  return FCMF_OK;
}

static int ln_bwd_blocks(int rows) {
  int blocks = (rows + 3) / 4;
  return blocks > 1024 ? 1024 : blocks;
}

extern "C" int64_t fcmf_add_ln_bwd_workspace(int rows, int H) { return (int64_t)ln_bwd_blocks(rows) * 3 * H; }

static int add_ln_bwd_impl(const void* dy, const void* z, const float* gamma, const float* mean, const float* rstd, void* dz,
                           void* dx, float* dgamma, float* dbeta, float* dxsum, float* workspace, int rows, int H,
                           float dropout_p, uint64_t seed, int dtype, void* stream, void* q8, float* qscale);
extern "C" int fcmf_add_ln_bwd(const void* dy, const void* z, const float* gamma, const float* mean, const float* rstd,
                               void* dz, void* dx, float* dgamma, float* dbeta, float* dxsum, float* workspace,
                               int rows, int H, float dropout_p, uint64_t seed, int dtype, void* stream) {
  return add_ln_bwd_impl(dy, z, gamma, mean, rstd, dz, dx, dgamma, dbeta, dxsum, workspace, rows, H, dropout_p, seed, dtype, stream, nullptr, nullptr);
}
extern "C" int fcmf_add_ln_bwd_fp8(const void* dy, const void* z, const float* gamma, const float* mean, const float* rstd,
                                   void* dz, void* dx, float* dgamma, float* dbeta, float* dxsum, float* workspace,
                                   int rows, int H, float dropout_p, uint64_t seed, int dtype, void* q8, float* qscale, void* stream) {
  if (!q8 || !qscale) return FCMF_ERR_ARG;
  return add_ln_bwd_impl(dy, z, gamma, mean, rstd, dz, dx, dgamma, dbeta, dxsum, workspace, rows, H, dropout_p, seed, dtype, stream, q8, qscale);
}
static int add_ln_bwd_impl(const void* dy, const void* z, const float* gamma, const float* mean, const float* rstd, void* dz,
                           void* dx, float* dgamma, float* dbeta, float* dxsum, float* workspace, int rows, int H,
                           float dropout_p, uint64_t seed, int dtype, void* stream, void* q8, float* qscale) {
  if (!dy || !z || !gamma || !mean || !rstd || !dz || !dgamma || !dbeta || rows < 0 || H <= 0) return FCMF_ERR_ARG;
  if (H % 4 != 0 || H > LN_MAXP * 256) return FCMF_ERR_UNSUPPORTED;
  if (dropout_p > 0.f && !dx) return FCMF_ERR_ARG;
  if (rows == 0) return FCMF_OK;
  hipStream_t st = reinterpret_cast<hipStream_t>(stream);
  const int blocks = ln_bwd_blocks(rows);
  if (dtype != FCMF_F32 && dtype != FCMF_BF16) return FCMF_ERR_UNSUPPORTED;
#define LAUNCH_(T, NP) hipLaunchKernelGGL((add_ln_bwd_kernel<T, NP>), dim3(blocks), dim3(256), 0, st, (const T*)dy, (const T*)z, \
    gamma, mean, rstd, (T*)dz, (T*)(dropout_p > 0.f ? dx : nullptr), dgamma, dbeta, dxsum, workspace, rows, H, dropout_p, seed, \
    (unsigned char*)q8, qscale)
  LN_DISPATCH(dtype, H);
#undef LAUNCH_
  if (workspace)
    hipLaunchKernelGGL(ln_partial_reduce_kernel, dim3((H + 63) / 64, 3, 8), dim3(256), 0, st, workspace, blocks, H, dgamma, dbeta, dxsum);
  FCMF_CHECK_LAUNCH();
  return FCMF_OK;
}

extern "C" int fcmf_position_ids(const int64_t* ids, int64_t* pos, int nseq, int S, int pad_id, void* stream) {
  if (!ids || !pos || nseq < 0 || S <= 0) return FCMF_ERR_ARG;
  if (nseq == 0) return FCMF_OK;
  hipLaunchKernelGGL(position_ids_kernel, dim3(nseq), dim3(64), 0, reinterpret_cast<hipStream_t>(stream), ids, pos, S, pad_id);
  FCMF_CHECK_LAUNCH();
  return FCMF_OK;
}

extern "C" int fcmf_embed_ln_fwd(const int64_t* ids, const int64_t* pos, const int64_t* type_ids, const float* word,
                                 const float* pos_table, const float* type_table, const float* gamma, const float* beta,
                                 void* y, void* z, float* mean, float* rstd, int ntok, int H, float eps, float dropout_p,
                                 uint64_t seed, int dtype, void* stream) {
  if (!ids || !pos || !word || !pos_table || !type_table || !gamma || !beta || !y || !mean || !rstd) return FCMF_ERR_ARG;
  if (H % 4 != 0 || H > LN_MAXP * 256) return FCMF_ERR_UNSUPPORTED;
  if (ntok <= 0) return ntok == 0 ? FCMF_OK : FCMF_ERR_ARG;
  hipStream_t st = reinterpret_cast<hipStream_t>(stream);
  dim3 grid((ntok + 3) / 4);
  if (dtype != FCMF_F32 && dtype != FCMF_BF16) return FCMF_ERR_UNSUPPORTED;
#define LAUNCH_(T, NP) hipLaunchKernelGGL((embed_ln_fwd_kernel<T, NP>), grid, dim3(256), 0, st, ids, pos, type_ids, word, \
    pos_table, type_table, gamma, beta, (T*)y, (T*)z, mean, rstd, ntok, H, eps, dropout_p, seed)
  LN_DISPATCH(dtype, H);
#undef LAUNCH_
  FCMF_CHECK_LAUNCH();
  return FCMF_OK;
}

extern "C" int fcmf_embed_bwd(const void* dz, const int64_t* ids, const int64_t* pos, const int64_t* type_ids, float* dword,
                              float* dpos, float* dtype_table, int ntok, int H, int pad_id, int dtype, void* stream) {
  if (!dz || !ids || !pos || !dword) return FCMF_ERR_ARG;
  if (H % 4 != 0) return FCMF_ERR_UNSUPPORTED;
  if (ntok <= 0) return ntok == 0 ? FCMF_OK : FCMF_ERR_ARG;
  hipStream_t st = reinterpret_cast<hipStream_t>(stream);
  dim3 grid((ntok + 3) / 4);
  const int rpb = 512;
  dim3 g2((H + 63) / 64, (ntok + rpb - 1) / rpb);
  if (dtype == FCMF_F32) {
    hipLaunchKernelGGL((embed_bwd_kernel<float>), grid, dim3(256), 0, st, (const float*)dz, ids, pos, type_ids, dword, dpos, dtype_table, ntok, H, pad_id);
    if (dtype_table) hipLaunchKernelGGL((embed_type0_kernel<float>), g2, dim3(256), 0, st, (const float*)dz, type_ids, dtype_table, ntok, H, rpb);
  } else if (dtype == FCMF_BF16) {
    hipLaunchKernelGGL((embed_bwd_kernel<bf16_t>), grid, dim3(256), 0, st, (const bf16_t*)dz, ids, pos, type_ids, dword, dpos, dtype_table, ntok, H, pad_id);
    if (dtype_table) hipLaunchKernelGGL((embed_type0_kernel<bf16_t>), g2, dim3(256), 0, st, (const bf16_t*)dz, type_ids, dtype_table, ntok, H, rpb);
  } else return FCMF_ERR_UNSUPPORTED;
  FCMF_CHECK_LAUNCH();
  return FCMF_OK;
}

extern "C" int fcmf_embed_pos_type_bwd(const void* dz, const int64_t* pos, const int64_t* type_ids, float* dpos, float* dtype_table,
                                       int nseq, int S, int H, int pad_id, int dtype, void* stream) {
  if (!dz || !pos || !dpos || nseq < 0 || S <= 0 || H <= 0) return FCMF_ERR_ARG;
  if (nseq == 0) return FCMF_OK;
  if (dtype != FCMF_F32 && dtype != FCMF_BF16) return FCMF_ERR_UNSUPPORTED;
  const int E = dtype == FCMF_F32 ? 4 : 8;
  if (H % E != 0 || H / E > 256 || (reinterpret_cast<uintptr_t>(dz) & 15)) return FCMF_ERR_UNSUPPORTED;
  hipStream_t st = reinterpret_cast<hipStream_t>(stream);
  const int slots = 256 / (H / E);
  const size_t smem = sizeof(float) * 2 * (size_t)slots * H + sizeof(int) * slots;
  dim3 grid(S, (nseq + 63) / 64);
  if (dtype == FCMF_F32) hipLaunchKernelGGL((embed_pos_type_bwd_kernel<float>), grid, dim3(256), smem, st, (const float*)dz, pos, type_ids, dpos, dtype_table, nseq, S, H, pad_id);
  else hipLaunchKernelGGL((embed_pos_type_bwd_kernel<bf16_t>), grid, dim3(256), smem, st, (const bf16_t*)dz, pos, type_ids, dpos, dtype_table, nseq, S, H, pad_id);
  FCMF_CHECK_LAUNCH();
  return FCMF_OK;
}

extern "C" int fcmf_embed_pos_bwd(const void* dz, const int64_t* pos, float* dpos, int nseq, int S, int H, int pad_id,
                                  int dtype, void* stream) {
  if (!dz || !pos || !dpos || nseq < 0 || S <= 0 || H <= 0) return FCMF_ERR_ARG;
  if (nseq == 0) return FCMF_OK;
  hipStream_t st = reinterpret_cast<hipStream_t>(stream);
  dim3 grid(S, (H + 255) / 256, (nseq + 63) / 64);
  if (dtype == FCMF_F32) hipLaunchKernelGGL((embed_pos_bwd_kernel<float>), grid, dim3(256), 0, st, (const float*)dz, pos, dpos, nseq, S, H, pad_id);
  else if (dtype == FCMF_BF16) hipLaunchKernelGGL((embed_pos_bwd_kernel<bf16_t>), grid, dim3(256), 0, st, (const bf16_t*)dz, pos, dpos, nseq, S, H, pad_id);
  else return FCMF_ERR_UNSUPPORTED;
  FCMF_CHECK_LAUNCH();
  return FCMF_OK;
}
```

### multimodal-aspect-category-sentiment-analysis_amd/fcmf_framework/_hip.py

```python
import ctypes
import os

import torch

_HERE = os.path.dirname(os.path.abspath(__file__))
LIB_PATH = os.path.join(_HERE, "libfcmf_hip.so")

F32, BF16, F64 = 0, 1, 2
BOX_FAST_TRIG = 0x100
EPI_NONE, EPI_GELU, EPI_TANH, EPI_DGELU, EPI_DTANH, EPI_ADD = 0, 1, 2, 3, 4, 5
ERR_UNSUPPORTED = -3

_c = ctypes
_vp, _i, _i64, _f, _u64 = _c.c_void_p, _c.c_int, _c.c_int64, _c.c_float, _c.c_uint64


class AttnDesc(ctypes.Structure):
    _fields_ = [
        ("dtype", _i), ("G", _i), ("heads", _i), ("d", _i), ("R", _i), ("T1", _i), ("T2", _i), ("group_div", _i),
        ("q_sg", _i64), ("q_sr", _i64), ("k1_sg", _i64), ("k1_st", _i64), ("k2_sg", _i64), ("k2_sr", _i64),
        ("k2_st", _i64), ("o_sg", _i64), ("o_sr", _i64),
        ("q", _vp), ("k1", _vp), ("v1", _vp), ("k2", _vp), ("v2", _vp),
        ("mask", _vp), ("bias", _vp),
        ("scale", _f), ("dropout_p", _f), ("seed", _u64), ("causal", _i), ("head_quirk", _i),
    ]


class CropDesc(ctypes.Structure):
    _fields_ = [
        ("offset", _i64), ("H", _i), ("W", _i), ("sC", _i64), ("sH", _i64), ("sW", _i64),
        ("r0", _i), ("r1", _i), ("c0", _i), ("c1", _i), ("flip", _i), ("reserved", _i),
    ]


SIGNATURES = {
    "fcmf_abi_version": [],
    "fcmf_build_info": [],
    "fcmf_gemm": [_vp, _vp, _vp, _vp, _vp, _vp, _vp, _i, _i, _i, _i64, _i64, _i64, _i, _i, _i, _i, _i, _i, _vp],
    "fcmf_gemm_ctx_create": [_c.POINTER(_vp)],
    "fcmf_gemm_ctx_destroy": [_vp],
    "fcmf_gemm_ctx_set_workspace": [_vp, _vp, _i64],
    "fcmf_gemm_ctx_tune": [_vp, _i, _i, _i, _i64],
    "fcmf_gemm_ctx_last_kernel": [_vp],
    "fcmf_gemm_colblocks": [_vp, _vp, _vp, _vp, _i, _i, _i, _i64, _i64, _i64, _i, _i, _i, _i64, _i, _vp],
    "fcmf_quant_fp8_rows": [_vp, _i64, _vp, _i64, _vp, _i, _i, _i, _vp],
    "fcmf_gemm_fp8": [_vp, _vp, _vp, _vp, _vp, _vp, _vp, _vp, _vp, _i, _i, _i, _i64, _i64, _i64, _i, _vp],
    "fcmf_colsum": [_vp, _vp, _i, _i, _i64, _i, _i, _vp],
    "fcmf_attn_small_fwd": [_c.POINTER(AttnDesc), _vp, _vp, _vp],
    "fcmf_attn_small_bwd": [_c.POINTER(AttnDesc), _vp, _vp, _vp, _vp, _vp, _vp, _vp, _vp, _vp, _vp],
    "fcmf_attn_small_bwd_grouped": [_c.POINTER(AttnDesc), _vp, _vp, _vp, _vp, _vp, _vp, _vp, _vp, _vp, _vp, _i64, _vp],
    "fcmf_attn_mfma_fwd": [_vp, _vp, _vp, _vp, _vp, _vp, _i, _i, _i, _i, _i64, _i64, _i64, _f, _f, _u64, _vp],
    "fcmf_attn_mfma_bwd": [_vp, _vp, _vp, _vp, _vp, _vp, _vp, _vp, _vp, _vp, _i, _i, _i, _i, _i64, _i64, _i64, _f, _f,
                           _u64, _vp, _vp],
    "fcmf_attn_probs": [_c.POINTER(AttnDesc), _vp, _i64, _i64, _vp],
    "fcmf_attn_mfma_probs": [_vp, _vp, _vp, _vp, _i, _i, _i, _i, _i64, _i64, _i64, _i64, _f, _vp],
    "fcmf_add_ln_fwd": [_vp, _vp, _i64, _vp, _vp, _vp, _vp, _vp, _vp, _i, _i, _f, _f, _u64, _i, _vp],
    "fcmf_add_ln_bwd": [_vp, _vp, _vp, _vp, _vp, _vp, _vp, _vp, _vp, _vp, _vp, _i, _i, _f, _u64, _i, _vp],
    "fcmf_add_ln_fwd_fp8": [_vp, _vp, _i64, _vp, _vp, _vp, _vp, _vp, _vp, _i, _i, _f, _f, _u64, _i, _vp, _vp, _vp],
    "fcmf_add_ln_bwd_fp8": [_vp, _vp, _vp, _vp, _vp, _vp, _vp, _vp, _vp, _vp, _vp, _i, _i, _f, _u64, _i, _vp, _vp, _vp],
    "fcmf_add_ln_bwd_workspace": [_i, _i],
    "fcmf_position_ids": [_vp, _vp, _i, _i, _i, _vp],
    "fcmf_embed_ln_fwd": [_vp, _vp, _vp, _vp, _vp, _vp, _vp, _vp, _vp, _vp, _vp, _vp, _i, _i, _f, _f, _u64, _i, _vp],
    "fcmf_embed_bwd": [_vp, _vp, _vp, _vp, _vp, _vp, _vp, _i, _i, _i, _i, _vp],
    "fcmf_embed_pos_bwd": [_vp, _vp, _vp, _i, _i, _i, _i, _i, _vp],
    "fcmf_embed_pos_type_bwd": [_vp, _vp, _vp, _vp, _vp, _i, _i, _i, _i, _i, _vp],
    "fcmf_box_bias_fwd": [_vp, _i, _vp, _vp, _vp, _vp, _i, _i, _i, _vp],
    "fcmf_box_bias_bwd": [_vp, _i, _vp, _vp, _vp, _vp, _vp, _vp, _i, _i, _i, _vp],
    "fcmf_box_embedding": [_vp, _i, _vp, _vp, _i, _i, _vp],
    "fcmf_xent_fwd": [_vp, _i64, _vp, _vp, _vp, _i, _i, _i64, _i, _vp],
    "fcmf_xent_bwd": [_vp, _i64, _vp, _vp, _i64, _vp, _f, _i, _i, _i64, _i, _vp],
    "fcmf_xent_mean": [_vp, _vp, _i, _i64, _f, _vp, _vp],
    "fcmf_bce_logits": [_vp, _i64, _vp, _i64, _i, _i, _vp, _vp, _vp, _i64, _vp, _i, _vp],
    "fcmf_crop_resize_normalize": [_vp, _i64, _vp, _i, _i, _i, _c.POINTER(_f), _c.POINTER(_f), _vp, _i64, _vp, _i, _vp],
    "fcmf_additive_mask": [_vp, _i64, _vp, _i, _i, _f, _vp],
    "fcmf_cast": [_vp, _vp, _i64, _i, _i, _vp],
    "fcmf_cast_transpose": [_vp, _vp, _i, _i, _vp],
    "fcmf_multi_cast_transpose": [_vp, _vp, _vp, _vp, _i, _vp],
    "fcmf_dropout": [_vp, _vp, _i64, _f, _u64, _i, _vp],
    "fcmf_act_bwd": [_vp, _vp, _vp, _i64, _i, _i, _vp],
    "fcmf_sum_axis": [_vp, _vp, _i64, _i, _i64, _i, _vp],
    "fcmf_embed_scale_fwd": [_vp, _vp, _vp, _vp, _i, _i, _i, _i64, _f, _i, _vp],
    "fcmf_embed_scale_bwd": [_vp, _vp, _vp, _i, _i, _i64, _vp, _f, _i, _vp],
    "fcmf_head_gather": [_vp, _vp, _i64, _i, _i, _i, _i, _i, _vp],
    "fcmf_multi_sumsq": [_vp, _vp, _vp, _vp, _i, _i, _vp, _vp, _vp],
    "fcmf_multi_adamw": [_vp, _vp, _vp, _vp, _vp, _vp, _vp, _vp, _vp, _i, _i, _c.POINTER(_f), _c.POINTER(_f), _i, _f, _f,
                         _f, _i, _vp, _f, _vp],
    "fcmf_bertadam": [_vp, _vp, _vp, _vp, _i64, _f, _f, _f, _f, _f, _f, _vp, _vp],
    "fcmf_conv_im2col": [_vp, _i, _vp, _i, _i, _i, _i, _i, _i64, _i64, _i64, _i64, _i, _i, _i, _i, _i, _vp],
    "fcmf_bn_stats": [_vp, _vp, _i64, _i, _i, _i, _vp],
    "fcmf_bn_stats_workspace": [_i64, _i, _i],
    "fcmf_bn_finalize": [_vp, _vp, _vp, _vp, _vp, _vp, _vp, _vp, _vp, _i, _i, _i64, _f, _f, _vp],
    "fcmf_bn_bwd": [_vp, _vp, _vp, _vp, _vp, _vp, _vp, _vp, _vp, _vp, _vp, _i64, _i, _i, _i, _i, _vp],
    "fcmf_conv_col2im": [_vp, _vp, _i, _i, _i, _i, _i, _i, _i, _i, _i, _i, _vp],
    "fcmf_maxpool3x3s2_bwd": [_vp, _vp, _vp, _i, _i, _i, _i, _i, _vp],
    "fcmf_adaptive_avgpool_bwd": [_vp, _vp, _i, _i, _i, _i, _i, _i, _i, _i, _vp],
    "fcmf_bn_apply": [_vp, _vp, _vp, _vp, _vp, _i64, _i, _i64, _i, _i, _vp],
    "fcmf_bn_apply_pad": [_vp, _vp, _vp, _vp, _vp, _i64, _i, _i64, _i, _i, _i, _i, _i, _vp],
    "fcmf_conv_gemm": [_vp, _vp, _vp, _vp, _i, _i, _i, _i, _i, _i, _i, _i, _i, _i, _vp],
    "fcmf_gemm_dw_batched": [_vp, _i, _vp, _vp, _vp, _i, _i, _i, _i64, _i64, _i64, _i, _vp],
    "fcmf_conv_gemm_runs": [_vp, _vp, _vp, _vp, _vp, _i, _i, _i, _i, _i, _i, _i, _i, _i, _i, _vp],
    "fcmf_pack_rgb0": [_vp, _i, _vp, _i, _i, _i, _i64, _i64, _i64, _i64, _i, _i, _vp],
    "fcmf_gemm_colstats": [_vp, _vp, _vp, _vp, _vp, _i, _i, _i, _i64, _i64, _i64, _vp],
    "fcmf_conv_gemm_colstats": [_vp, _vp, _vp, _vp, _vp, _i, _i, _i, _i, _i, _i, _i, _i, _i, _i, _vp],
    "fcmf_gemm_colstats_block_rows": [_vp, _i, _i, _i],
    "fcmf_bn_stats_blocks": [_vp, _vp, _i64, _i, _i, _i, _vp],
    "fcmf_bn_finalize_apply": [_vp, _vp, _vp, _vp, _vp, _vp, _vp, _vp, _vp, _vp, _i, _i, _i64, _f, _f, _i, _i, _i, _i, _i, _vp],
    "fcmf_maxpool3x3s2": [_vp, _vp, _i, _i, _i, _i, _i, _vp],
    "fcmf_adaptive_avgpool": [_vp, _vp, _i, _i, _i, _i, _i, _i, _i, _i, _vp],
    "fcmf_dp_unique_id": [_vp],
    "fcmf_dp_comm_create": [_c.POINTER(_vp), _vp, _i, _i],
    "fcmf_dp_comm_destroy": [_vp],
    "fcmf_dp_allreduce_bucket": [_vp, _vp, _i64, _i, _i, _vp],
}

_lib = None


class HipLibraryError(RuntimeError):
    pass


def lib():
    global _lib
    if _lib is None:
        if not os.path.exists(LIB_PATH):
            raise HipLibraryError(
                f"{LIB_PATH} not found: build it with `python __graft_entry__.py` or "
                f"`make -C multimodal-aspect-category-sentiment-analysis_amd/csrc` (hipcc, gfx950). "
                f"fcmf_framework has no CPU/PyTorch fallback.")
        l = ctypes.CDLL(LIB_PATH)
        for name, args in SIGNATURES.items():
            fn = getattr(l, name)
            fn.argtypes = args
            fn.restype = (ctypes.c_char_p if name in ("fcmf_build_info", "fcmf_gemm_ctx_last_kernel") else
                          ctypes.c_int64 if name in ("fcmf_add_ln_bwd_workspace", "fcmf_bn_stats_workspace") else ctypes.c_int)
        _lib = l
    return _lib


_ERR = {-1: "bad argument", -2: "kernel launch failed", -3: "unsupported configuration",
        -4: "RCCL unavailable or collective failed"}


def check(rc, what):
    if rc != 0:
        raise HipLibraryError(f"{what} failed: {_ERR.get(rc, rc)}")


def dt(t):
    if t.dtype == torch.float32:
        return F32
    if t.dtype == torch.bfloat16:
        return BF16
    if t.dtype == torch.float64:
        return F64
    raise HipLibraryError(f"unsupported dtype {t.dtype}")


def ptr(t):
    return 0 if t is None else t.data_ptr()


def stream():
    return _raw_stream(torch.cuda.current_device())


_raw_stream = getattr(torch._C, "_cuda_getCurrentRawStream", None) or (lambda idx: torch.cuda.current_stream(idx).cuda_stream)


# ... 50 lines not shown
```

### multimodal-aspect-category-sentiment-analysis_amd/fcmf_framework/fused.py

```python
import math

import os

import torch

from . import _hip as H
from . import ops


class QKVStorageMixin:

    def _fuse_qkv_storage(self):
        q, k, v = self.query, self.key, self.value
        Hh = q.weight.shape[0]
        W = torch.empty((3 * Hh, q.weight.shape[1]), dtype=q.weight.dtype, device=q.weight.device)
        b = torch.empty((3 * Hh,), dtype=q.bias.dtype, device=q.bias.device)
        for i, lin in enumerate((q, k, v)):
            W[i * Hh:(i + 1) * Hh].copy_(lin.weight.data)
            b[i * Hh:(i + 1) * Hh].copy_(lin.bias.data)
            lin.weight.data = W[i * Hh:(i + 1) * Hh]
            lin.bias.data = b[i * Hh:(i + 1) * Hh]
        self._qkv_w, self._qkv_b = W, b

    def _apply(self, fn, *a, **kw):
# ... 34 lines not shown
    st = _side.get(device)
    if st is None:
        st = _side[device] = torch.cuda.Stream(device=device)
    return st


class _SideGemms:

    def __init__(self, device):
        self.dev = device
        self.on = USE_SIDE_STREAM and not ops.tracing()
        self.used = False

    def launch(self, tensors, *a, **kw):
        if not self.on:
            return ops.gemm(*a, **kw)
        main, side = torch.cuda.current_stream(self.dev), _side_stream(self.dev)
        side.wait_stream(main)
        with torch.cuda.stream(side):
            ops.gemm(*a, **kw)
        for t in tensors:
            t.record_stream(side)
        self.used = True

    def join(self):
        if self.on and self.used:
            torch.cuda.current_stream(self.dev).wait_stream(_side_stream(self.dev))


def _use_mfma(dtype, Hd, heads, T):
    return dtype == torch.bfloat16 and Hd // heads == 64 and T <= 256 and ops.USE_MFMA_ATTENTION


def _qkv_desc(qkv, G, T, Hd, heads, mask, scale, p, seed):
    es = qkv.element_size()
    a = H.AttnDesc()
    a.dtype, a.G, a.heads, a.d, a.R, a.T1, a.T2, a.group_div = H.dt(qkv), G, heads, Hd // heads, T, T, 0, 1
    a.q_sg, a.q_sr, a.k1_sg, a.k1_st = T * 3 * Hd, 3 * Hd, T * 3 * Hd, 3 * Hd
    a.o_sg, a.o_sr = T * Hd, Hd
    base = qkv.data_ptr()
    a.q, a.k1, a.v1 = base, base + Hd * es, base + 2 * Hd * es
    a.mask, a.scale, a.dropout_p, a.seed = H.ptr(mask), scale, p, seed
    return a


def self_attention_fwd(qkv, mask, G, T, Hd, heads, p, seed):
    scale = 1.0 / math.sqrt(Hd // heads)
    out = torch.empty((G * T, Hd), dtype=qkv.dtype, device=qkv.device)
    lse = torch.empty((G, heads, T), dtype=torch.float32, device=qkv.device)
    es, base, L = qkv.element_size(), qkv.data_ptr(), H.lib()
    if _use_mfma(qkv.dtype, Hd, heads, T):
        H.check(L.fcmf_attn_mfma_fwd(base, base + Hd * es, base + 2 * Hd * es, H.ptr(mask), H.ptr(out), H.ptr(lse), G, heads,
                                     T, T, 3 * Hd, 3 * Hd, Hd, scale, p, seed, H.stream()), "fcmf_attn_mfma_fwd")
    else:
        a = _qkv_desc(qkv, G, T, Hd, heads, mask, scale, p, seed)
        H.check(L.fcmf_attn_small_fwd(a, H.ptr(out), H.ptr(lse), H.stream()), "fcmf_attn_small_fwd")
    return out, lse


def self_attention_probs(qkv, mask, G, T, Hd, heads, probs):
    scale = 1.0 / math.sqrt(Hd // heads)
    if tuple(probs.shape) != (G, heads, T, T) or probs.dtype != torch.float32 or not probs.is_contiguous():
        raise H.HipLibraryError(f"attention probabilities: need a contiguous float32 {(G, heads, T, T)} tensor")
    es, base, L = qkv.element_size(), qkv.data_ptr(), H.lib()
    if _use_mfma(qkv.dtype, Hd, heads, T):
        H.check(L.fcmf_attn_mfma_probs(base, base + Hd * es, H.ptr(mask), H.ptr(probs), G, heads, T, T, 3 * Hd, 3 * Hd,
                                       heads * T * T, T * T, scale, H.stream()), "fcmf_attn_mfma_probs")
    else:
        a = _qkv_desc(qkv, G, T, Hd, heads, mask, scale, 0.0, 0)
        H.check(L.fcmf_attn_probs(a, H.ptr(probs), heads * T * T, T * T, H.stream()), "fcmf_attn_probs")


def self_attention_bwd(qkv, mask, out, lse, dout, G, T, Hd, heads, p, seed, bias_grad=None):
    scale = 1.0 / math.sqrt(Hd // heads)
    es, base, L = qkv.element_size(), qkv.data_ptr(), H.lib()
    if _use_mfma(qkv.dtype, Hd, heads, T):
        dqkv = torch.empty_like(qkv)
        db = dqkv.data_ptr()
        part = None if bias_grad is None else torch.empty((G, 3 * Hd), dtype=torch.float32, device=qkv.device)
        H.check(L.fcmf_attn_mfma_bwd(base, base + Hd * es, base + 2 * Hd * es, H.ptr(mask), H.ptr(out), H.ptr(dout), H.ptr(lse),
                                     db, db + Hd * es, db + 2 * Hd * es, G, heads, T, T, 3 * Hd, 3 * Hd, Hd, scale, p, seed,
                                     H.ptr(part), H.stream()), "fcmf_attn_mfma_bwd")
        if part is not None:
            H.check(L.fcmf_colsum(H.ptr(part), H.ptr(bias_grad), G, 3 * Hd, 3 * Hd, H.dt(part), 1, H.stream()), "fcmf_colsum")
        return dqkv
    a = _qkv_desc(qkv, G, T, Hd, heads, mask, scale, p, seed)
    nch = max(1, (T + 127) // 128)
    dq = torch.empty((nch, G, T, Hd), dtype=qkv.dtype, device=qkv.device)
    dk = torch.empty((G, T, Hd), dtype=qkv.dtype, device=qkv.device)
    dv = torch.empty((G, T, Hd), dtype=qkv.dtype, device=qkv.device)
    H.check(L.fcmf_attn_small_bwd(a, H.ptr(out), H.ptr(dout), H.ptr(lse), H.ptr(dq), H.ptr(dk), H.ptr(dv), 0, 0, 0, H.stream()),
            "fcmf_attn_small_bwd")
    dqkv = torch.cat((ops._sum_leading(dq), dk, dv), dim=-1).view(G * T, 3 * Hd)
    if bias_grad is not None:
        H.check(L.fcmf_colsum(H.ptr(dqkv), H.ptr(bias_grad), G * T, 3 * Hd, 3 * Hd, H.dt(dqkv), 1, H.stream()), "fcmf_colsum")
    return dqkv


def _want_q(rows, Hd, dtype):
    return ops.fp8_enabled() and dtype == torch.bfloat16 and Hd % 128 == 0 and rows >= 256


def _q_buffers(rows, Hd, device):
    return torch.empty((rows, Hd), dtype=torch.uint8, device=device), torch.empty(rows, dtype=torch.float32, device=device)


def _ln_fwd(x, res, res_ld, g, b, eps, p, seed, quant=False):
    rows, Hd = x.shape
    y = torch.empty_like(x)
    mean = torch.empty(rows, dtype=torch.float32, device=x.device)
    rstd = torch.empty(rows, dtype=torch.float32, device=x.device)
    if quant:
        q, sc = _q_buffers(rows, Hd, x.device)
        H.check(H.lib().fcmf_add_ln_fwd_fp8(H.ptr(x), H.ptr(res), res_ld, H.ptr(g), H.ptr(b), H.ptr(y), H.ptr(x), H.ptr(mean),
                                            H.ptr(rstd), rows, Hd, eps, p, seed, H.dt(x), H.ptr(q), H.ptr(sc), H.stream()), "fcmf_add_ln_fwd_fp8")
        return y, x, mean, rstd, (q, sc)
    H.check(H.lib().fcmf_add_ln_fwd(H.ptr(x), H.ptr(res), res_ld, H.ptr(g), H.ptr(b), H.ptr(y), H.ptr(x), H.ptr(mean),
                                    H.ptr(rstd), rows, Hd, eps, p, seed, H.dt(x), H.stream()), "fcmf_add_ln_fwd")
    return y, x, mean, rstd, None


def _ln_bwd(dy, z, g, mean, rstd, p, seed, dg, db, dxsum, quant=False):
    dz = torch.empty_like(z)
    dx = torch.empty_like(z) if p > 0 else None
    ws = ops.ln_workspace(z.shape[0], z.shape[1], z.device)
    if quant:
        q, sc = _q_buffers(z.shape[0], z.shape[1], z.device)
        H.check(H.lib().fcmf_add_ln_bwd_fp8(H.ptr(dy), H.ptr(z), H.ptr(g), H.ptr(mean), H.ptr(rstd), H.ptr(dz), H.ptr(dx), H.ptr(dg),
                                            H.ptr(db), H.ptr(dxsum), H.ptr(ws), z.shape[0], z.shape[1], p, seed, H.dt(z), H.ptr(q),
                                            H.ptr(sc), H.stream()), "fcmf_add_ln_bwd_fp8")
        return dz, (dx if dx is not None else dz), (q, sc)
    H.check(H.lib().fcmf_add_ln_bwd(H.ptr(dy), H.ptr(z), H.ptr(g), H.ptr(mean), H.ptr(rstd), H.ptr(dz), H.ptr(dx), H.ptr(dg),
                                    H.ptr(db), H.ptr(dxsum), H.ptr(ws), z.shape[0], z.shape[1], p, seed, H.dt(z), H.stream()),
            "fcmf_add_ln_bwd")
    return dz, (dx if dx is not None else dz), None


def _post_fwd(c, res, res_ld, wo, bo, g1, be1, w1, b1, w2, b2, g2, be2, eps, p, seeds):
    dt = c.dtype
    M, Hd = c.shape
    I = w1.shape[0]
    co, c1, c2 = ops.as_compute(wo, dt), ops.as_compute(w1, dt), ops.as_compute(w2, dt)
    h = torch.empty((M, Hd), dtype=dt, device=c.device)
    ops.gemm_nt(c, wo, co, h, M, Hd, Hd, Hd, bias=bo.detach())
    h1, z1, m1, r1, h1q = _ln_fwd(h, res, res_ld, g1, be1, eps, p, seeds[0], quant=_want_q(M, Hd, dt))
    u = torch.empty((M, I), dtype=dt, device=c.device)
    a = torch.empty((M, I), dtype=dt, device=c.device)
    ops.gemm_nt(h1, w1, c1, a, M, I, Hd, Hd, bias=b1.detach(), aux=u, epi=H.EPI_GELU, xq=h1q)
    f = torch.empty((M, Hd), dtype=dt, device=c.device)
    ops.gemm_nt(a, w2, c2, f, M, Hd, I, I, bias=b2.detach())
    y, z2, m2, r2, _ = _ln_fwd(f, h1, Hd, g2, be2, eps, p, seeds[1])
    return y, (z1, m1, r1, h1, u, a, z2, m2, r2)


def _post_bwd(dy, c, saved, wo, w1, w2, g1, g2, p, seeds, G, side):
    z1, m1, r1, h1, u, a, z2, m2, r2 = saved
    dt = c.dtype
    M, Hd = c.shape
    I = w1.shape[0]
    co, c1, c2 = ops.as_compute(wo, dt), ops.as_compute(w1, dt), ops.as_compute(w2, dt)
    dz2, df, dfq = _ln_bwd(dy, z2, g2, m2, r2, p, seeds[1], G["g2"], G["be2"], G["b2"], quant=_want_q(M, Hd, dt))
    du = torch.empty((M, I), dtype=dt, device=c.device)
    ops.gemm_dx(df, w2, c2, du, M, I, Hd, aux=u, epi=H.EPI_DGELU, colsum=G["b1"], dyq=dfq)
    side.launch((df, a), df, a, G["w2"], Hd, I, M, Hd, I, I, 1, 1, acc=True)
    dh1 = torch.empty((M, Hd), dtype=dt, device=c.device)
    ops.gemm_dx(du, w1, c1, dh1, M, Hd, I, aux=dz2, epi=H.EPI_ADD)
    side.launch((du, h1), du, h1, G["w1"], I, Hd, M, I, Hd, Hd, 1, 1, acc=True)
    dz1, dh, dhq = _ln_bwd(dh1, z1, g1, m1, r1, p, seeds[0], G["g1"], G["be1"], G["bo"], quant=_want_q(M, Hd, dt))
    dc = torch.empty((M, Hd), dtype=dt, device=c.device)
    ops.gemm_dx(dh, wo, co, dc, M, Hd, Hd, dyq=dhq)
    side.launch((dh, c), dh, c, G["wo"], Hd, Hd, M, Hd, Hd, Hd, 1, 1, acc=True)
    return dc, dz1


def _layer_grads(device, Hd, I, params):
    shapes = dict(wqkv=(3 * Hd, Hd), bqkv=(3 * Hd,), wo=(Hd, Hd), w1=(I, Hd), w2=(Hd, I), bo=(Hd,), b1=(I,), b2=(Hd,),
                  g1=(Hd,), be1=(Hd,), g2=(Hd,), be2=(Hd,))
    G, R = {}, {}
    for n, q in params.items():
        G[n], R[n] = ops.grad_dest(q, shapes[n], temp=False)
    rest = [n for n in params if G[n] is None]
    if rest:
        flat = torch.zeros(sum(math.prod(shapes[n]) for n in rest), dtype=torch.float32, device=device)
        off = 0
        for n in rest:
            k = math.prod(shapes[n])
            G[n] = R[n] = flat[off:off + k].view(shapes[n])
            off += k
    return G, R


def _split3(g, Hd):
    return (None, None, None) if g is None else (g[:Hd], g[Hd:2 * Hd], g[2 * Hd:])


class PostAttentionFn(torch.autograd.Function):

    @staticmethod
    def forward(ctx, c, res, wo, bo, g1, be1, w1, b1, w2, b2, g2, be2, eps, p, seed0, seed1):
        c2 = ops._rows(c).contiguous()
        r2 = ops._rows(res)
        if r2.stride(1) != 1:
            r2 = r2.contiguous()
        y, saved = _post_fwd(c2, r2, ops._ld(r2), wo, bo, g1, be1, w1, b1, w2, b2, g2, be2, eps, p, (seed0, seed1))
        ctx.save_for_backward(c2, wo, w1, w2, g1, g2, bo, be1, b1, b2, be2, *saved)
        ctx.cfg = (p, seed0, seed1, c.shape, res.shape)
        return y.view(c.shape)

    @staticmethod
    def backward(ctx, dy):
        c2, wo, w1, w2, g1, g2, bo, be1, b1, b2, be2, *saved = ctx.saved_tensors
        p, s0, s1, cshape, rshape = ctx.cfg
        G, R = _layer_grads(c2.device, c2.shape[1], w1.shape[0],
                            dict(wo=wo, w1=w1, w2=w2, bo=bo, b1=b1, b2=b2, g1=g1, be1=be1, g2=g2, be2=be2))
        side = _SideGemms(c2.device)
        dc, dres = _post_bwd(dy.reshape(c2.shape).contiguous(), c2, saved, wo, w1, w2, g1, g2, p, (s0, s1), G, side)
        side.join()
# ... 52 lines not shown
```

### multimodal-aspect-category-sentiment-analysis_amd/fcmf_framework/ops.py

```python
import ctypes
import math
import os
import weakref

import torch

from . import _hip as H

_compute_dtype = torch.float32


def set_compute_dtype(dtype):
    global _compute_dtype
    if dtype not in (torch.float32, torch.bfloat16):
        raise ValueError("compute dtype must be torch.float32 or torch.bfloat16")
    _compute_dtype = dtype


def compute_dtype():
    return _compute_dtype


_fp8 = False


def set_fp8(on):
    global _fp8
    _fp8 = bool(on)


def fp8_enabled():
    return _fp8 and _compute_dtype == torch.bfloat16


_output_attentions = False


def set_output_attentions(on):
    global _output_attentions
    _output_attentions = bool(on)


def output_attentions():
    return _output_attentions


_seed_base = 0x5DEECE66D
_seed_ctr = 0


def manual_seed(seed):
    global _seed_base, _seed_ctr
    _seed_base = (int(seed) * 0x9E3779B97F4A7C15 + 0x632BE59BD9B4E019) & 0xFFFFFFFFFFFFFFFF
    _seed_ctr = 0


def next_seed():
    global _seed_ctr
    _seed_ctr += 1
    x = (_seed_base + _seed_ctr * 0xD1342543DE82EF95) & 0xFFFFFFFFFFFFFFFF
    x ^= x >> 29
    return (x * 0xBF58476D1CE4E5B9) & 0xFFFFFFFFFFFFFFFF


VOCAB_PAD = 32


class _Shadows:

    def __init__(self):
        self.map = {}
        self.pad = {}
        self.mapT = {}
        self.mapD = {}
        self.mapQ = {}
        self.mapQT = {}
        self.mapH = {}
        self._mt_tables = None

    def get_t(self, w, owner=None):
        key = (w.data_ptr(), tuple(w.shape))
        ent = self.mapT.get(key)
        owner = w if owner is None else owner
        if ent is not None and ent[1] == w._version and not ent[2] and ent[4]() is owner:
            return ent[0]
        sh = ent[0] if ent is not None else torch.empty((w.shape[1], w.shape[0]), dtype=torch.bfloat16, device=w.device)
        src = w.detach()
        if not src.is_contiguous():
            src = src.contiguous()
        H.check(H.lib().fcmf_cast_transpose(H.ptr(src), H.ptr(sh), w.shape[0], w.shape[1], H.stream()), "fcmf_cast_transpose")
        self.mapT[key] = [sh, w._version, False, w.is_contiguous(), weakref.ref(owner), w.data_ptr() - owner.data_ptr()]
        return sh

    def _prune_transposed(self):
        dead = []
        for k, ent in self.mapT.items():
            o = ent[4]()
            if o is None or o.data_ptr() + ent[5] != k[0]:
                dead.append(k)
        for k in dead:
            del self.mapT[k]
        if dead:
            self._mt_tables = None

    def refresh_transposed(self):
        if not self.mapT:
            return
        self._prune_transposed()
        items = [(k, ent) for k, ent in self.mapT.items() if ent[3]]
        if not items:
            return
        sig = tuple((k[0], ent[0].data_ptr()) for k, ent in items)
        if self._mt_tables is None or self._mt_tables[0] != sig:
            dev = items[0][1][0].device
            desc = []
            for t, (k, ent) in enumerate(items):
                R, C = k[1]
                desc += [(t, r, c) for r in range((R + 63) // 64) for c in range((C + 63) // 64)]
            self._mt_tables = (sig,
                               torch.tensor([k[0] for k, _ in items], dtype=torch.int64, device=dev),
                               torch.tensor([ent[0].data_ptr() for _, ent in items], dtype=torch.int64, device=dev),
                               torch.tensor([list(k[1]) for k, _ in items], dtype=torch.int32, device=dev),
                               torch.tensor(desc, dtype=torch.int32, device=dev), len(desc))
        _, src, dst, dims, desc, n = self._mt_tables
        H.check(H.lib().fcmf_multi_cast_transpose(H.ptr(src), H.ptr(dst), H.ptr(dims), H.ptr(desc), n, H.stream()),
                "fcmf_multi_cast_transpose")
        for _, ent in items:
            ent[2] = False
            ent[1] = ent[4]()._version

    def head_nk(self, ws):
        key = tuple(w.data_ptr() for w in ws) + (tuple(ws[0].shape),)
        ent = self.mapH.get(key)
        if ent is None or any(r() is None for r in ent[2]):
            nh, E, d = ws[0].shape
            buf = torch.empty((len(ws) * nh * d, E), dtype=torch.bfloat16, device=ws[0].device)
            pieces = []
            for i, w in enumerate(ws):
                if w.dtype != torch.float32 or not w.is_contiguous() or tuple(w.shape) != (nh, E, d):
                    raise H.HipLibraryError("head_nk: dense float32 [n_head, E, d] parameters expected")
                for h in range(nh):
                    src, dst = w.detach()[h], buf[(i * nh + h) * d:(i * nh + h + 1) * d]
                    k2 = (src.data_ptr(), (E, d), key)
                    self.mapT[k2] = [dst, -1, True, True, weakref.ref(w), src.data_ptr() - w.data_ptr()]
                    pieces.append(k2)
            self._mt_tables = None
            ent = self.mapH[key] = (buf, pieces, [weakref.ref(w) for w in ws])
        buf, pieces, owners = ent
        for k2 in pieces:
            e = self.mapT.get(k2)
            if e is None or e[2] or e[1] != e[4]()._version:
                if e is None:
                    del self.mapH[key]
                    return self.head_nk(ws)
                self.refresh_transposed()
                break
        return buf

    def get_fp8(self, w, owner=None):
        key = (w.data_ptr(), tuple(w.shape))
        ent = self.mapQ.get(key)
        owner = w if owner is None else owner
        if ent is not None and ent[1] == w._version and not ent[2] and ent[3]() is owner:
            return ent[0]
        src = self.get(w) if w.is_contiguous() else w.detach().contiguous()
        q, sc = quant_fp8_rows(src, w.shape[0], w.shape[1], w.shape[1], out=None if ent is None else ent[0])
        self.mapQ[key] = [(q, sc), w._version, False, weakref.ref(owner)]
        return q, sc

    def get_fp8_t(self, w, owner=None):
        key = (w.data_ptr(), tuple(w.shape))
        ent = self.mapQT.get(key)
        owner = w if owner is None else owner
        if ent is not None and ent[1] == w._version and not ent[2] and ent[3]() is owner:
            return ent[0]
        wt = self.get_t(w, owner)
        q, sc = quant_fp8_rows(wt, wt.shape[0], wt.shape[1], wt.shape[1], out=None if ent is None else ent[0])
        self.mapQT[key] = [(q, sc), w._version, False, weakref.ref(owner)]
        return q, sc

    def padded(self, w):
        sh = self.get(w)
        return self.pad.get((w.data_ptr(), tuple(w.shape)), sh)

    def get(self, w):
        key = (w.data_ptr(), tuple(w.shape))
        ent = self.map.get(key)
        if ent is not None and ent[1] == w._version and not ent[2]:
            return ent[0]
        if ent is not None:
            sh = ent[0]
        elif w.dim() == 2 and w.shape[0] % VOCAB_PAD != 0:
            rows = (w.shape[0] + VOCAB_PAD - 1) // VOCAB_PAD * VOCAB_PAD
            full = torch.zeros((rows, w.shape[1]), dtype=torch.bfloat16, device=w.device)
            sh = full[:w.shape[0]]
            self.pad[key] = full
        else:
            sh = torch.empty(w.shape, dtype=torch.bfloat16, device=w.device)
        src = w.detach()
        if not src.is_contiguous():
            src = src.contiguous()
        H.check(H.lib().fcmf_cast(H.ptr(src), H.ptr(sh), src.numel(), H.F32, H.BF16, H.stream()), "fcmf_cast")
        self.map[key] = [sh, w._version, False]
        return sh

    def derived(self, w, tag, build):
        key = (w.data_ptr(), tuple(w.shape), tag)
        ent = self.mapD.get(key)
        if ent is not None and ent[1] == w._version and not ent[2]:
            return ent[0]
        t = build(w.detach())
        self.mapD[key] = [t, w._version, False]
        return t

    def peek(self, w):
        ent = self.map.get((w.data_ptr(), tuple(w.shape)))
        return None if ent is None else ent[0]

    def mark_fresh(self, w):
        ent = self.map.get((w.data_ptr(), tuple(w.shape)))
        if ent is not None:
            ent[1] = w._version
            ent[2] = False

    def mark_all_stale(self):
        for ent in self.map.values():
            ent[2] = True
        for ent in self.mapT.values():
            ent[2] = True
        for ent in self.mapD.values():
            ent[2] = True
        for m in (self.mapQ, self.mapQT):
            for k in [k for k, ent in m.items() if ent[3]() is None]:
                del m[k]
            for ent in m.values():
                ent[2] = True

    def clear(self):
        self.map.clear()
        self.pad.clear()
        self.mapT.clear()
        self.mapD.clear()
        self.mapQ.clear()
        self.mapQT.clear()
        self.mapH.clear()
        self._mt_tables = None


shadows = _Shadows()

_grad_arena = None


def set_grad_arena(arena):
    global _grad_arena
    _grad_arena = arena
    if arena is not None and deferred_dw.reset not in arena.on_zero:
        arena.on_zero.append(deferred_dw.reset)


def grad_arena():
    return _grad_arena


def grad_dest(param, shape, *, rows=None, in_place=True, temp=True, device=None):
    a = _grad_arena
    if a is not None and param is not None:
        if isinstance(param, (list, tuple)):
            ok = all(q.dtype == torch.float32 and q.is_contiguous() for q in param) and sum(q.numel() for q in param) == math.prod(shape)
        else:
            ok = param.dtype == torch.float32 and param.is_contiguous() and param.numel() == math.prod(shape)
        got = a.claim(param, rows) if ok else None
        if got is not None and (got[1] or in_place):
            buf, first = got
            if rows is None:
                buf = buf.view(shape)
                return buf, (buf if first else None)
            return buf, (a.grad_alias(param, shape) if first else None)
    if not temp:
        return None, None
    if device is None:
        device = (param[0] if isinstance(param, (list, tuple)) else param).device
    if rows is None:
        buf = torch.zeros(shape, dtype=torch.float32, device=device)
        return buf, buf
    buf = torch.zeros((rows,) + tuple(shape[1:]), dtype=torch.float32, device=device)
    return buf, buf[:shape[0]]


def as_compute(w, dtype):
    if dtype == torch.float32:
        return w.detach()
    return shadows.get(w)


def cast(x, dtype):
    if x.dtype == dtype:
        return x
    H.require_cuda(x)
    x = x.contiguous()
    y = torch.empty(x.shape, dtype=dtype, device=x.device)
    H.check(H.lib().fcmf_cast(H.ptr(x), H.ptr(y), x.numel(), H.dt(x), H.dt(y), H.stream()), "fcmf_cast")
    return y


class _CastFn(torch.autograd.Function):
    @staticmethod
    def forward(ctx, x, dtype):
        ctx.src = x.dtype
        return cast(x, dtype)

    @staticmethod
    def backward(ctx, dy):
        return cast(dy.contiguous(), ctx.src), None


def cast_ad(x, dtype):
    return x if x.dtype == dtype else _CastFn.apply(x, dtype)


def _rows(x):
    if x.dim() != 2:
        x = x.reshape(-1, x.shape[-1])
    if x.stride(1) != 1 or (x.shape[0] > 1 and x.stride(0) < x.shape[1]):
        x = x.contiguous()
    return x


_gemm_trace = None


def gemm_trace_begin():
    global _gemm_trace
    _gemm_trace = []


def gemm_trace_end():
    global _gemm_trace
    tr, _gemm_trace = _gemm_trace, None
    if not tr:
        return []
# ... 12 lines not shown

    def __enter__(self):
        if _gemm_trace is not None:
            self.e0, self.e1 = torch.cuda.Event(enable_timing=True), torch.cuda.Event(enable_timing=True)
            self.e0.record()
        return self

    def __exit__(self, *exc):
        if _gemm_trace is not None and exc[0] is None and self.flops is not None:
            self.e1.record()
            _gemm_trace.append((H.lib().fcmf_gemm_ctx_last_kernel(H.gemm_ctx()).decode(), float(self.flops), self.e0, self.e1))
        return False


DEFER_DW = os.environ.get("FCMF_DEFER_DW", "1") == "1"
DEFER_DW_MAX_BYTES = 48 << 30


class _DeferredDW:
    def __init__(self):
        self.q, self.bytes, self.armed = [], 0, False
        self.batched_launches = self.batched_matrices = 0

    def reset(self):
        self.q, self.bytes, self.armed = [], 0, False

    def wanted(self, A, B, C, ta, tb, bias, aux, epi, colsum):
        if not (DEFER_DW and ta and tb and bias is None and aux is None and colsum is None and epi == H.EPI_NONE
                and C.dtype == torch.float32 and A.dtype == torch.bfloat16 and B.dtype == torch.bfloat16):
            return False
        arena = _grad_arena
        if not (arena is not None and C.device == arena.flat.device
                and C.untyped_storage().data_ptr() == arena.flat.untyped_storage().data_ptr()):
            return False
        n = arena.uses(C.data_ptr())
        return n == 1 or (n > 1 and DEFER_SHARED_DW)

    def push(self, A, B, C, M, N, K, lda, ldb, ldc, acc):
        if not self.armed:
            try:
                torch.autograd.Variable._execution_engine.queue_callback(self.flush)
            except RuntimeError:
                return False
            self.armed = True
        self.q.append((A, B, C.data_ptr(), M, N, K, lda, ldb, ldc, bool(acc)))
        self.bytes += A.numel() * A.element_size() + B.numel() * B.element_size()
        if self.bytes > DEFER_DW_MAX_BYTES:
            self.flush(final=False)
        return True

    def flush(self, final=True, lo=None, hi=None):
        if lo is not None:
            q = [e for e in self.q if lo <= e[2] < hi]
            if not q:
                return
            self.q = [e for e in self.q if not (lo <= e[2] < hi)]
            self.bytes = sum(e[0].numel() * e[0].element_size() + e[1].numel() * e[1].element_size() for e in self.q)
        else:
            q, self.q, self.bytes = self.q, [], 0
        if final:
            self.armed = False
        groups = {}
        for e in q:
            groups.setdefault((e[0].device,) + e[3:], []).append(e)
        for key, es in groups.items():
            _, M, N, K, lda, ldb, ldc, acc = key
            H.require_cuda(es[0][0])
            with torch.cuda.device(key[0]):
                ctx = H.gemm_ctx(workspace=True)
                arr = lambda i: (ctypes.c_void_p * len(es))(*[e[i] if i == 2 else e[i].data_ptr() for e in es])
                with trace_launch(2.0 * M * N * K * len(es)):
                    H.check(H.lib().fcmf_gemm_dw_batched(ctx, len(es), arr(0), arr(1), arr(2), M, N, K, lda, ldb, ldc, int(acc), H.stream()),
                            "fcmf_gemm_dw_batched")
            self.batched_launches += 1
            self.batched_matrices += len(es)


deferred_dw = _DeferredDW()


def flush_deferred_dw(lo=None, hi=None):
    if deferred_dw.q:
        deferred_dw.flush(final=False, lo=lo, hi=hi)


def gemm(A, B, C, M, N, K, lda, ldb, ldc, ta, tb, bias=None, aux=None, epi=H.EPI_NONE, acc=False, colsum=None):
    H.require_cuda(A, B, C)
    if deferred_dw.wanted(A, B, C, ta, tb, bias, aux, epi, colsum) and deferred_dw.push(A, B, C, M, N, K, lda, ldb, ldc, acc):
        return
    ctx = H.gemm_ctx(workspace=acc or C.dtype == torch.float32)
    with trace_launch(2.0 * M * N * K):
        H.check(H.lib().fcmf_gemm(ctx, H.ptr(A), H.ptr(B), H.ptr(C), H.ptr(bias), H.ptr(aux), H.ptr(colsum), M, N, K, lda, ldb, ldc,
                                  int(ta), int(tb), H.dt(A), H.dt(C), epi, int(acc), H.stream()), "fcmf_gemm")


DEFER_SHARED_DW = os.environ.get("FCMF_DEFER_SHARED_DW", "0") == "1"
HEAD_WGRAD_DIRECT = os.environ.get("FCMF_HEAD_WGRAD_DIRECT", "1") == "1"


def head_weight_grad(x2, dy2, params):
    a = _grad_arena
    if a is None or dy2.dtype != torch.bfloat16 or x2.dtype != torch.bfloat16 or not HEAD_WGRAD_DIRECT:
        return None
    nh, E, d = params[0].shape
    if any(p.dtype != torch.float32 or tuple(p.shape) != (nh, E, d) for p in params) or d % 4:
        return None
    M, N = x2.shape[0], len(params) * nh * d
    if E < 256 or N < 256 or dy2.shape[1] != N or not dy2.is_contiguous():
        return None
    got = a.claim(list(params))
    if got is None or not got[1]:
        return None
    with trace_launch(2.0 * E * N * M) as t:
        rc = H.lib().fcmf_gemm_colblocks(H.gemm_ctx(workspace=True), H.ptr(x2), H.ptr(dy2), H.ptr(got[0]), E, N, M, _ld(x2), N, d, 1, 1,
                                         d, E * d, 0, H.stream())
        if rc == H.ERR_UNSUPPORTED:
            t.flops = None
            a.release(params)
            return None
        H.check(rc, "fcmf_gemm_colblocks")
    return [a.grad_alias(p, (nh, E, d)) for p in params]


def quant_fp8_rows(x, rows, K, ldx, out=None):
    H.require_cuda(x)
    if out is None:
        q = torch.empty((rows, K), dtype=torch.uint8, device=x.device)
        sc = torch.empty(rows, dtype=torch.float32, device=x.device)
    else:
        q, sc = out
    H.check(H.lib().fcmf_quant_fp8_rows(H.ptr(x), ldx, H.ptr(q), K, H.ptr(sc), rows, K, H.dt(x), H.stream()), "fcmf_quant_fp8_rows")
    return q, sc


def _fp8_ok(M, N, K, ldc, *tensors):
    return (fp8_enabled() and K % 128 == 0 and N % 8 == 0 and ldc % 8 == 0 and M >= 256 and N >= 256
            and all(t is None or t.dtype == torch.bfloat16 for t in tensors))


def gemm_fp8(xq, sx, wq, sw, C, M, N, K, bias=None, aux=None, epi=H.EPI_NONE, colsum=None):
    with trace_launch(2.0 * M * N * K):
        H.check(H.lib().fcmf_gemm_fp8(H.gemm_ctx(), H.ptr(xq), H.ptr(sx), H.ptr(wq), H.ptr(sw), H.ptr(C), H.ptr(bias), H.ptr(aux), H.ptr(colsum),
                                      M, N, K, K, K, N, epi, H.stream()), "fcmf_gemm_fp8")


def gemm_nt(x, weight, w_compute, y, M, N, K, ldx, bias=None, aux=None, epi=H.EPI_NONE, colsum=None, owner=None, xq=None):
    if _grad_arena is not None and (owner is not None or weight is not None):
        _grad_arena.note_forward((owner if owner is not None else weight).data_ptr())
    if weight is not None and weight.dtype == torch.float32 and weight.dim() == 2 and _fp8_ok(M, N, K, N, x, y, aux):
        xq, sx = quant_fp8_rows(x, M, K, ldx) if xq is None else xq
        wq, sw = shadows.get_fp8(weight, owner)
        gemm_fp8(xq, sx, wq, sw, y, M, N, K, bias=bias, aux=aux, epi=epi, colsum=colsum)
    else:
        gemm(x, w_compute, y, M, N, K, ldx, K, N, 0, 0, bias=bias, aux=aux, epi=epi, colsum=colsum)


def colsum(X, M, N, ldx):
    out = torch.empty(N, dtype=torch.float32, device=X.device)
    H.check(H.lib().fcmf_colsum(H.ptr(X), H.ptr(out), M, N, ldx, H.dt(X), 0, H.stream()), "fcmf_colsum")
    return out


def _ld(x):
    return x.stride(0) if x.shape[0] > 1 else x.shape[1]


# ... 300 lines not shown
        scale = (g.float() / nvalid[0]).reshape(1).contiguous()
        d = logits
        H.check(H.lib().fcmf_xent_bwd(H.ptr(logits), Vp, H.ptr(lb), H.ptr(d), Vp, H.ptr(scale), 1.0, M, V, ignore_index,
                                      H.dt(logits), H.stream()), "fcmf_xent_bwd")
        if Vp != V:
            d[:, V:].zero_()
        dx = dw = db = None
        if ctx.needs_input_grad[0]:
            dx = gemm_dx_long_k(d, w, M, K, Vp, K).view(xshape)
        if ctx.needs_input_grad[1]:
            dwp, dw = grad_dest(weight, (V, K), rows=Vp, device=x2.device)
            gemm(d, x2, dwp, Vp, K, M, Vp, _ld(x2), K, 1, 1, acc=True)
        if has_bias and ctx.needs_input_grad[2]:
            db = colsum(d, M, Vp, Vp)[:V]
        return dx, dw, db, None, None


def vocab_cross_entropy(x, weight, bias, labels, ignore_index=-100):
    return VocabCrossEntropyFn.apply(x, weight, bias, labels, int(ignore_index))


class FFNFn(torch.autograd.Function):

    @staticmethod
    def forward(ctx, x, w1, b1, w2, b2):
        x2 = _rows(x)
        c1, c2 = as_compute(w1, x2.dtype), as_compute(w2, x2.dtype)
        M = x2.shape[0]
        u = torch.empty((M, w1.shape[0]), dtype=x2.dtype, device=x2.device)
        a = _linear_fwd(x2, c1, b1.detach(), H.EPI_GELU, aux=u, master=w1)
        y = _linear_fwd(a, c2, b2.detach(), master=w2)
        ctx.save_for_backward(x2, w1, w2, u, a)
        ctx.xshape = x.shape
        return y.view(*x.shape[:-1], w2.shape[0])

    @staticmethod
    def backward(ctx, dy):
        x2, w1, w2, u, a = ctx.saved_tensors
        dy2 = dy.reshape(-1, dy.shape[-1]).contiguous()
        c1, c2 = as_compute(w1, x2.dtype), as_compute(w2, x2.dtype)
        du, dw2, db2 = _linear_bwd(a, c2, dy2, True, True, True, dx_epi=H.EPI_DGELU, dx_aux=u, master=w2)
        dx, dw1, db1 = _linear_bwd(x2, c1, du, ctx.needs_input_grad[0], True, True, master=w1)
        return (None if dx is None else dx.view(ctx.xshape)), dw1, db1, dw2, db2


def ffn(x, w1, b1, w2, b2):
    return FFNFn.apply(x, w1, b1, w2, b2)


def ln_workspace(rows, Hd, device):
    n = H.lib().fcmf_add_ln_bwd_workspace(rows, Hd)
    return torch.empty(n, dtype=torch.float32, device=device)


class AddLNFn(torch.autograd.Function):

    @staticmethod
    def forward(ctx, x, res, gamma, beta, eps, p, seed):
        x2 = _rows(x).contiguous()
        rows, Hd = x2.shape
        r2 = None if res is None else _rows(res)
        y = torch.empty_like(x2)
        z = torch.empty_like(x2)
        mean = torch.empty(rows, dtype=torch.float32, device=x2.device)
        rstd = torch.empty(rows, dtype=torch.float32, device=x2.device)
        H.require_cuda(x2)
        H.check(H.lib().fcmf_add_ln_fwd(H.ptr(x2), H.ptr(r2), 0 if r2 is None else _ld(r2), H.ptr(gamma), H.ptr(beta),
                                        H.ptr(y), H.ptr(z), H.ptr(mean), H.ptr(rstd), rows, Hd, eps, p, seed,
                                        H.dt(x2), H.stream()), "fcmf_add_ln_fwd")
        ctx.save_for_backward(z, gamma, mean, rstd, beta)
        ctx.p, ctx.seed, ctx.xshape = p, seed, x.shape
        ctx.res_shape = None if res is None else res.shape
        return y.view(x.shape)

    @staticmethod
    def backward(ctx, dy):
        z, gamma, mean, rstd, beta = ctx.saved_tensors
        rows, Hd = z.shape
        dy2 = dy.reshape(rows, Hd).contiguous()
        dz = torch.empty_like(z)
        dx = torch.empty_like(z) if ctx.p > 0 else None
        dgbuf, dg = grad_dest(gamma, (Hd,))
        dbbuf, db = grad_dest(beta, (Hd,))
        H.check(H.lib().fcmf_add_ln_bwd(H.ptr(dy2), H.ptr(z), H.ptr(gamma), H.ptr(mean), H.ptr(rstd), H.ptr(dz),
                                        H.ptr(dx), H.ptr(dgbuf), H.ptr(dbbuf), 0, H.ptr(ln_workspace(rows, Hd, z.device)), rows, Hd, ctx.p, ctx.seed, H.dt(z),
                                        H.stream()), "fcmf_add_ln_bwd")
        dxo = (dx if dx is not None else dz).view(ctx.xshape)
        dres = None if ctx.res_shape is None else dz.view(ctx.res_shape)
        return dxo, dres, dg, db, None, None, None


def add_layer_norm(x, res, gamma, beta, eps, p=0.0, training=False):
    p = float(p) if training else 0.0
    return AddLNFn.apply(x, res, gamma, beta, float(eps), p, next_seed() if p > 0 else 0)


class DropoutFn(torch.autograd.Function):
    @staticmethod
    def forward(ctx, x, p, seed):
        x2 = x.contiguous()
        y = torch.empty_like(x2)
        H.require_cuda(x2)
        H.check(H.lib().fcmf_dropout(H.ptr(x2), H.ptr(y), x2.numel(), p, seed, H.dt(x2), H.stream()), "fcmf_dropout")
        ctx.p, ctx.seed = p, seed
        return y

    @staticmethod
    def backward(ctx, dy):
        d = dy.contiguous()
        o = torch.empty_like(d)
        H.check(H.lib().fcmf_dropout(H.ptr(d), H.ptr(o), d.numel(), ctx.p, ctx.seed, H.dt(d), H.stream()), "fcmf_dropout")
        return o, None, None


def dropout(x, p, training):
    if not training or p <= 0:
        return x
    return DropoutFn.apply(x, float(p), next_seed())


def position_ids(input_ids, pad_id):
    ids = input_ids.contiguous()
    H.require_cuda(ids)
    pos = torch.empty_like(ids)
    H.check(H.lib().fcmf_position_ids(H.ptr(ids), H.ptr(pos), ids.shape[0], ids.shape[1], pad_id, H.stream()),
            "fcmf_position_ids")
    return pos


class EmbedLNFn(torch.autograd.Function):

    @staticmethod
    def forward(ctx, ids, pos, tt, word, ptab, ttab, gamma, beta, eps, p, seed, pad_id, out_dtype):
        ids, pos = ids.contiguous(), pos.contiguous()
        tt = None if tt is None else tt.contiguous()
        ntok, Hd = ids.numel(), word.shape[1]
        y = torch.empty((ntok, Hd), dtype=out_dtype, device=word.device)
        z = torch.empty_like(y)
        mean = torch.empty(ntok, dtype=torch.float32, device=word.device)
        rstd = torch.empty(ntok, dtype=torch.float32, device=word.device)
        H.require_cuda(ids, word)
        H.check(H.lib().fcmf_embed_ln_fwd(H.ptr(ids), H.ptr(pos), H.ptr(tt), H.ptr(word), H.ptr(ptab), H.ptr(ttab),
                                          H.ptr(gamma), H.ptr(beta), H.ptr(y), H.ptr(z), H.ptr(mean), H.ptr(rstd),
                                          ntok, Hd, eps, p, seed, H.dt(y), H.stream()), "fcmf_embed_ln_fwd")
        ctx.save_for_backward(ids, pos, tt, z, gamma, mean, rstd)
        ctx.p, ctx.seed, ctx.pad_id = p, seed, pad_id
        ctx.params = (word, ptab, ttab, gamma, beta)
        return y.view(*ids.shape, Hd)

    @staticmethod
    def backward(ctx, dy):
        ids, pos, tt, z, gamma, mean, rstd = ctx.saved_tensors
        ntok, Hd = z.shape
        d = dy.reshape(ntok, Hd).contiguous()
        L = H.lib()
        if ctx.p > 0:
            o = torch.empty_like(d)
            H.check(L.fcmf_dropout(H.ptr(d), H.ptr(o), d.numel(), ctx.p, ctx.seed, H.dt(d), H.stream()), "fcmf_dropout")
            d = o
        dz = torch.empty_like(z)
        word, ptab, ttab, gpar, bpar = ctx.params
        dg, _ = grad_dest(gpar, (Hd,), in_place=False, device=z.device)
        db, _ = grad_dest(bpar, (Hd,), in_place=False, device=z.device)
        H.check(L.fcmf_add_ln_bwd(H.ptr(d), H.ptr(z), H.ptr(gamma), H.ptr(mean), H.ptr(rstd), H.ptr(dz), 0, H.ptr(dg),
                                  H.ptr(db), 0, H.ptr(ln_workspace(ntok, Hd, z.device)), ntok, Hd, 0.0, 0, H.dt(z), H.stream()), "fcmf_add_ln_bwd")
        dwordbuf, dword = grad_dest(word, word.shape, device=z.device)
        dpos, _ = grad_dest(ptab, ptab.shape, in_place=False, device=z.device)
        dtt, _ = grad_dest(ttab, ttab.shape, in_place=False, device=z.device)
        two_d = ids.dim() == 2 and pos.is_contiguous()
# ... 328 lines not shown
```

### multimodal-aspect-category-sentiment-analysis_amd/fcmf_framework/optimization.py

```python
import ctypes
import math

import torch
from torch.optim import Optimizer
from torch.optim.optimizer import required

from . import _hip as H
from . import ops


def warmup_cosine(x, warmup=0.002):
    if x < warmup:
        return x / warmup
    return 0.5 * (1.0 + math.cos(math.pi * x))


def warmup_constant(x, warmup=0.002):
    if x < warmup:
        return x / warmup
    return 1.0


def warmup_linear(x, warmup=0.002):
    if x < warmup:
        return x / warmup
    return 1.0 - x


SCHEDULES = {
    'warmup_cosine': warmup_cosine,
    'warmup_constant': warmup_constant,
    'warmup_linear': warmup_linear,
}


def get_linear_schedule_with_warmup(optimizer, num_warmup_steps, num_training_steps, last_epoch=-1):
    def lr_lambda(step):
        if step < num_warmup_steps:
            return float(step) / float(max(1, num_warmup_steps))
        return max(0.0, float(num_training_steps - step) / float(max(1, num_training_steps - num_warmup_steps)))
    return torch.optim.lr_scheduler.LambdaLR(optimizer, lr_lambda, last_epoch)


class BertAdam(Optimizer):

    def __init__(self, params, lr=required, warmup=-1, t_total=-1, schedule='warmup_linear',
                 b1=0.9, b2=0.999, e=1e-6, weight_decay=0.01, max_grad_norm=1.0):
        if lr is not required and lr < 0.0:
            raise ValueError("Invalid learning rate: {} - should be >= 0.0".format(lr))
        if schedule not in SCHEDULES:
            raise ValueError("Invalid schedule parameter: {}".format(schedule))
        if not 0.0 <= warmup < 1.0 and not warmup == -1:
            raise ValueError("Invalid warmup: {} - should be in [0.0, 1.0[ or -1".format(warmup))
        if not 0.0 <= b1 < 1.0:
            raise ValueError("Invalid b1 parameter: {} - should be in [0.0, 1.0[".format(b1))
        if not 0.0 <= b2 < 1.0:
            raise ValueError("Invalid b2 parameter: {} - should be in [0.0, 1.0[".format(b2))
        if not e >= 0.0:
            raise ValueError("Invalid epsilon value: {} - should be >= 0.0".format(e))
        defaults = dict(lr=lr, schedule=schedule, warmup=warmup, t_total=t_total, b1=b1, b2=b2, e=e,
                        weight_decay=weight_decay, max_grad_norm=max_grad_norm)
        super().__init__(params, defaults)
        self._scratch = None

    def _lr(self, group, state):
        if group['t_total'] != -1:
            return group['lr'] * SCHEDULES[group['schedule']](state['step'] / group['t_total'], group['warmup'])
        return group['lr']

    def get_lr(self):
        lr = []
        for group in self.param_groups:
            for p in group['params']:
                state = self.state[p]
                if len(state) == 0:
                    return [0]
                lr.append(self._lr(group, state))
        return lr

    def step(self, closure=None):
        loss = closure() if closure is not None else None
        L = H.lib()
        for group in self.param_groups:
            for p in group['params']:
                if p.grad is None:
                    continue
                grad = p.grad.data
                if grad.is_sparse:
                    raise RuntimeError('Adam does not support sparse gradients, please consider SparseAdam instead')
                H.require_cuda(p)
                state = self.state[p]
                if len(state) == 0:
                    state['step'] = 0
                    state['next_m'] = torch.zeros_like(p.data)
                    state['next_v'] = torch.zeros_like(p.data)
                if self._scratch is None or self._scratch.device != p.device:
                    self._scratch = torch.zeros(1, dtype=torch.float64, device=p.device)
                g = grad.contiguous().float()
                H.check(L.fcmf_bertadam(H.ptr(p.data), H.ptr(g), H.ptr(state['next_m']), H.ptr(state['next_v']),
                                        p.numel(), float(self._lr(group, state)), group['b1'], group['b2'], group['e'],
                                        group['weight_decay'], group['max_grad_norm'], H.ptr(self._scratch),
                                        H.stream()), "fcmf_bertadam")
                state['step'] += 1
        ops.shadows.mark_all_stale()
        return loss


class FusedAdamW(Optimizer):
    CHUNK = 65536

    def __init__(self, params, lr=1e-3, betas=(0.9, 0.999), eps=1e-8, weight_decay=1e-2):
        if lr < 0.0 or eps < 0.0 or not 0.0 <= betas[0] < 1.0 or not 0.0 <= betas[1] < 1.0:
            raise ValueError("invalid AdamW hyper-parameter")
        super().__init__(params, dict(lr=lr, betas=betas, eps=eps, weight_decay=weight_decay))
        if len(self.param_groups) > 8:
            raise ValueError("FusedAdamW supports at most 8 parameter groups")
        self._tables = None
        self._sumsq = None
        self.last_grad_norm = None

    def _build(self, plist, device):
        sizes = [p.numel() for p, _ in plist]
        ct, co = [], []
        for t, n in enumerate(sizes):
            for off in range(0, n, self.CHUNK):
                ct.append(t)
                co.append(off)
        for p, _ in plist:
            st = self.state[p]
            if len(st) == 0:
                st['step'] = 0
                st['exp_avg'] = torch.zeros_like(p.data)
                st['exp_avg_sq'] = torch.zeros_like(p.data)
        i64 = lambda xs: torch.tensor(xs, dtype=torch.int64, device=device)
        self._tables = dict(
            key=tuple(id(p) for p, _ in plist),
            p=i64([p.data_ptr() for p, _ in plist]),
            m=i64([self.state[p]['exp_avg'].data_ptr() for p, _ in plist]),
            v=i64([self.state[p]['exp_avg_sq'].data_ptr() for p, _ in plist]),
            sizes=i64(sizes),
            group=torch.tensor([g for _, g in plist], dtype=torch.int32, device=device),
            ct=torch.tensor(ct, dtype=torch.int32, device=device), co=i64(co), nchunks=len(ct),
            pptr=[p.data_ptr() for p, _ in plist],
            mvptr=[(self.state[p]['exp_avg'].data_ptr(), self.state[p]['exp_avg_sq'].data_ptr()) for p, _ in plist])

    def load_state_dict(self, state_dict):
        super().load_state_dict(state_dict)
        for st in self.state.values():
            if 'step' in st and torch.is_tensor(st['step']):
                st['step'] = int(st['step'].item())
        self._tables = None

    @torch.no_grad()
    def step(self, closure=None, max_grad_norm=None):
        loss = None
        if closure is not None:
            with torch.enable_grad():
                loss = closure()
        plist = [(p, gi) for gi, g in enumerate(self.param_groups) for p in g['params'] if p.grad is not None]
        if not plist:
            return loss
        device = plist[0][0].device
        for p, _ in plist:
            H.require_cuda(p)
            if p.dtype != torch.float32 or p.grad.dtype != torch.float32:
                raise H.HipLibraryError("FusedAdamW expects float32 master parameters and gradients")
            if not p.is_contiguous() or not p.grad.is_contiguous():
                raise H.HipLibraryError("FusedAdamW expects contiguous parameters and gradients")
        T = self._tables
        if (T is None or T['key'] != tuple(id(p) for p, _ in plist) or T['pptr'] != [p.data_ptr() for p, _ in plist]
                or T['mvptr'] != [(self.state[p]['exp_avg'].data_ptr(), self.state[p]['exp_avg_sq'].data_ptr())
                                  if len(self.state[p]) else None for p, _ in plist]):
            self._build(plist, device)
            T = self._tables
        sh = [ops.shadows.peek(p) for p, _ in plist]
        gl, sl = [p.grad.data_ptr() for p, _ in plist], [0 if s is None else s.data_ptr() for s in sh]
        if T.get('gl') != gl:
            T['gl'], T['g_ptrs'] = gl, torch.tensor(gl, dtype=torch.int64).to(device, non_blocking=True)
        if T.get('sl') != sl:
            T['sl'], T['sh_ptrs'] = sl, torch.tensor(sl, dtype=torch.int64).to(device, non_blocking=True)
        g_ptrs, sh_ptrs = T['g_ptrs'], T['sh_ptrs']
        L = H.lib()
        st = H.stream()
        if self._sumsq is None or self._sumsq.device != device:
            self._sumsq = torch.zeros(1, dtype=torch.float64, device=device)
        mg = -1.0
        if max_grad_norm is not None and max_grad_norm > 0:
            self._sumsq.zero_()
            H.check(L.fcmf_multi_sumsq(H.ptr(g_ptrs), H.ptr(T['sizes']), H.ptr(T['ct']), H.ptr(T['co']), T['nchunks'],
                                       self.CHUNK, H.ptr(self._sumsq), 0, st), "fcmf_multi_sumsq")
            mg = float(max_grad_norm)
            self.last_grad_norm = self._sumsq
        steps = {int(self.state[p]['step']) for p, _ in plist}
        if len(steps) != 1:
            raise H.HipLibraryError("FusedAdamW: parameters with different step counts are not supported")
        step = steps.pop() + 1
        ng = len(self.param_groups)
        lr = (ctypes.c_float * 8)(*[float(g['lr']) for g in self.param_groups] + [0.0] * (8 - ng))
        wd = (ctypes.c_float * 8)(*[float(g['weight_decay']) for g in self.param_groups] + [0.0] * (8 - ng))
        b1, b2 = self.param_groups[0]['betas']
        eps = self.param_groups[0]['eps']
        H.check(L.fcmf_multi_adamw(H.ptr(T['p']), H.ptr(g_ptrs), H.ptr(T['m']), H.ptr(T['v']), H.ptr(sh_ptrs),
                                   H.ptr(T['sizes']), H.ptr(T['group']), H.ptr(T['ct']), H.ptr(T['co']), T['nchunks'],
                                   self.CHUNK, lr, wd, ng, b1, b2, eps, step, H.ptr(self._sumsq), mg, st),
                "fcmf_multi_adamw")
        ops.shadows.mark_all_stale()
        ops.shadows.refresh_transposed()
        for (p, _), s in zip(plist, sh):
            self.state[p]['step'] = step
            if s is not None:
                ops.shadows.mark_fresh(p)
        return loss

    def grad_norm(self):
        return None if self.last_grad_norm is None else self.last_grad_norm.sqrt().float()
```

Measured before the change: 1742 samples/s.

## Fuse transposed bf16 shadow refresh into AdamW and batch deferred LN/colsum reductions

```diff
diff --git a/include/fcmf_hip.h b/include/fcmf_hip.h
--- a/include/fcmf_hip.h
+++ b/include/fcmf_hip.h
@@ -95,6 +95,29 @@
                         void* dx, float* dgamma, float* dbeta, float* dxsum, float* workspace, int rows, int H,
                         float dropout_p, uint64_t seed, int dtype, void* q8, float* qscale, void* stream);
 int64_t fcmf_add_ln_bwd_workspace(int rows, int H);
+int fcmf_add_ln_bwd_partials(const void* dy, const void* z, const float* gamma, const float* mean, const float* rstd,
+                             void* dz, void* dx, float* workspace, int rows, int H, float dropout_p, uint64_t seed,
+                             int dtype, void* stream);
+typedef struct {
+  const float* partial;
+  float* dgamma;
+  float* dbeta;
+  float* dxsum;
+  int nblocks;
+  int H;
+  int accumulate;
+  int reserved;
+} fcmf_ln_reduce_entry;
+int fcmf_ln_partial_reduce_batched(const fcmf_ln_reduce_entry* entries , int n, void* stream);
+typedef struct {
+  const float* X;
+  float* out;
+  int64_t ldx;
+  int M, N;
+  int accumulate;
+  int reserved;
+} fcmf_colsum_entry;
+int fcmf_colsum_batched(const fcmf_colsum_entry* entries , int n, void* stream);
 
 int fcmf_position_ids(const int64_t* ids, int64_t* pos, int nseq, int S, int pad_id, void* stream);
 int fcmf_embed_ln_fwd(const int64_t* ids, const int64_t* pos, const int64_t* type_ids,
@@ -161,6 +184,14 @@
                      const float* lr , const float* wd , int ngroups,
                      float beta1, float beta2, float eps, int step, const double* sumsq,
                      float max_norm, void* stream);
+int fcmf_multi_adamw_wt(const int64_t* p_ptrs, const int64_t* g_ptrs, const int64_t* m_ptrs,
+                        const int64_t* v_ptrs, const int64_t* bf16_ptrs, const int64_t* sizes,
+                        const int32_t* group_of, const int32_t* chunk_tensor,
+                        const int64_t* chunk_offset, int nchunks, int chunk_size,
+                        const float* lr , const float* wd , int ngroups,
+                        float beta1, float beta2, float eps, int step, const double* sumsq,
+                        float max_norm, const int64_t* t_ptrs, const int32_t* t_dims,
+                        const int32_t* tile_desc, int ntiles, void* stream);
 int fcmf_bertadam(float* p, const float* g, float* m, float* v, int64_t n, float lr_scheduled,
                   float beta1, float beta2, float eps, float weight_decay, float max_grad_norm,
                   double* scratch, void* stream);
diff --git a/multimodal-aspect-category-sentiment-analysis_amd/csrc/gemm.hip b/multimodal-aspect-category-sentiment-analysis_amd/csrc/gemm.hip
--- a/multimodal-aspect-category-sentiment-analysis_amd/csrc/gemm.hip
+++ b/multimodal-aspect-category-sentiment-analysis_amd/csrc/gemm.hip
@@ -1188,12 +1188,11 @@
 }
 
 template <typename T>
-__global__ __launch_bounds__(256) void colsum_kernel(const T* __restrict__ X, float* __restrict__ out, int M, int N,
-                                                     int64_t ldx, int rows_per_block, int vec) {
-  __shared__ float4 red[4][64];
+__device__ __forceinline__ void colsum_body(const T* __restrict__ X, float* __restrict__ out, int M, int N, int64_t ldx,
+                                            int rows_per_block, int vec, int colblock, int rowblock, float4 (*red)[64]) {
   const int lane = threadIdx.x & 63, wave = threadIdx.x >> 6;
-  const int col = blockIdx.x * 256 + lane * 4;
-  const int r0 = blockIdx.y * rows_per_block;
+  const int col = colblock * 256 + lane * 4;
+  const int r0 = rowblock * rows_per_block;
   const int r1 = min(M, r0 + rows_per_block);
   float4 s = make_float4(0.f, 0.f, 0.f, 0.f);
   if (vec && col + 3 < N) {
@@ -1226,6 +1225,27 @@
     if (col + 2 < N) atomicAdd(out + col + 2, a.z + b.z + c.z + d.z);
     if (col + 3 < N) atomicAdd(out + col + 3, a.w + b.w + c.w + d.w);
   }
+}
+
+template <typename T>
+__global__ __launch_bounds__(256) void colsum_kernel(const T* __restrict__ X, float* __restrict__ out, int M, int N,
+                                                     int64_t ldx, int rows_per_block, int vec) {
+  __shared__ float4 red[4][64];
+  colsum_body<T>(X, out, M, N, ldx, rows_per_block, vec, blockIdx.x, blockIdx.y, red);
+}
+
+constexpr int COLSUM_BATCH = 64;
+struct ColsumBatch {
+  const float* X[COLSUM_BATCH];
+  float* out[COLSUM_BATCH];
+  int M[COLSUM_BATCH], N[COLSUM_BATCH], rpb[COLSUM_BATCH], vec[COLSUM_BATCH];
+  int64_t ldx[COLSUM_BATCH];
+};
+__global__ __launch_bounds__(256) void colsum_batched_kernel(ColsumBatch t) {
+  __shared__ float4 red[4][64];
+  const int e = blockIdx.z;
+  if ((int)blockIdx.x * 256 >= t.N[e] || (int)blockIdx.y * t.rpb[e] >= t.M[e]) return;
+  colsum_body<float>(t.X[e], t.out[e], t.M[e], t.N[e], t.ldx[e], t.rpb[e], t.vec[e], blockIdx.x, blockIdx.y, red);
 }
 
 template <bool A_TR, bool B_TR, typename TC, int EPI>
@@ -1944,6 +1964,16 @@
   return gemm_impl(ctx, a, stream);
 }
 
+static int colsum_rows_per_block(int M, int N) {
+  const int bx = (N + 255) / 256;
+  int rpb = 256;
+  if ((int64_t)((M + 255) / 256) * bx < 256) {
+    rpb = (int)(((int64_t)M * bx / 1024 + 3) & ~3ll);
+    rpb = rpb < 16 ? 16 : (rpb > 256 ? 256 : rpb);
+  }
+  return rpb;
+}
+
 extern "C" int fcmf_colsum(const void* X, float* out, int M, int N, int64_t ldx, int dtype, int accumulate,
                            void* stream) {
   if (!X || !out || M < 0 || N <= 0) return FCMF_ERR_ARG;
@@ -1952,11 +1982,7 @@
   if (M == 0) return FCMF_OK;
   const int vec = (ldx % 4 == 0) && ((reinterpret_cast<uintptr_t>(X) & 15) == 0);
   const int bx = (N + 255) / 256;
-  int rpb = 256;
-  if ((int64_t)((M + 255) / 256) * bx < 256) {
-    rpb = (int)(((int64_t)M * bx / 1024 + 3) & ~3ll);
-    rpb = rpb < 16 ? 16 : (rpb > 256 ? 256 : rpb);
-  }
+  const int rpb = colsum_rows_per_block(M, N);
   dim3 grid(bx, (M + rpb - 1) / rpb);
   if (dtype == FCMF_F32) hipLaunchKernelGGL((colsum_kernel<float>), grid, dim3(256), 0, st, (const float*)X, out, M, N, ldx, rpb, vec);
   else if (dtype == FCMF_BF16) hipLaunchKernelGGL((colsum_kernel<bf16_t>), grid, dim3(256), 0, st, (const bf16_t*)X, out, M, N, ldx, rpb, vec);
@@ -1964,3 +1990,32 @@
   FCMF_CHECK_LAUNCH();
   return FCMF_OK;
 }
+
+extern "C" int fcmf_colsum_batched(const fcmf_colsum_entry* entries, int n, void* stream) {
+  if (n < 0 || (n > 0 && !entries)) return FCMF_ERR_ARG;
+  for (int i = 0; i < n; ++i)
+    if (!entries[i].X || !entries[i].out || entries[i].M <= 0 || entries[i].N <= 0 || entries[i].ldx < entries[i].N) return FCMF_ERR_ARG;
+  hipStream_t st = reinterpret_cast<hipStream_t>(stream);
+  for (int i = 0; i < n; ++i)
+    if (!entries[i].accumulate && hipMemsetAsync(entries[i].out, 0, sizeof(float) * entries[i].N, st) != hipSuccess) return FCMF_ERR_LAUNCH;
+  int i0 = 0;
+  while (i0 < n) {
+    ColsumBatch t{};
+    int k = 0, gx = 0, gy = 0;
+    for (; i0 + k < n && k < COLSUM_BATCH; ++k) {
+      const fcmf_colsum_entry& e = entries[i0 + k];
+      bool clash = false;
+      for (int j = 0; j < k; ++j) clash = clash || t.out[j] == e.out;
+      if (clash) break;
+      t.X[k] = e.X; t.out[k] = e.out; t.M[k] = e.M; t.N[k] = e.N; t.ldx[k] = e.ldx;
+      t.rpb[k] = colsum_rows_per_block(e.M, e.N);
+      t.vec[k] = (e.ldx % 4 == 0) && ((reinterpret_cast<uintptr_t>(e.X) & 15) == 0);
+      gx = max(gx, (e.N + 255) / 256);
+      gy = max(gy, (e.M + t.rpb[k] - 1) / t.rpb[k]);
+    }
+    hipLaunchKernelGGL(colsum_batched_kernel, dim3(gx, gy, k), dim3(256), 0, st, t);
+    i0 += k;
+  }
+  FCMF_CHECK_LAUNCH();
+  return FCMF_OK;
+}
diff --git a/multimodal-aspect-category-sentiment-analysis_amd/csrc/misc.hip b/multimodal-aspect-category-sentiment-analysis_amd/csrc/misc.hip
--- a/multimodal-aspect-category-sentiment-analysis_amd/csrc/misc.hip
+++ b/multimodal-aspect-category-sentiment-analysis_amd/csrc/misc.hip
@@ -322,9 +322,130 @@
   float beta1, beta2, eps, bc1, bc2_sqrt;
   const double* sumsq;
   float max_norm;
+  int nflat;
+  const int64_t* t_ptrs;
+  const int32_t* t_dims;
+  const int32_t* tile_desc;
 };
 
+typedef float adam_f4 __attribute__((ext_vector_type(4)));
+
+__device__ __forceinline__ void adam_update4(const AdamArgs& a, float lr, float wd, float coef, float step_size, adam_f4 graw,
+                                             adam_f4 praw, adam_f4 mraw, adam_f4 vraw, adam_f4& p4, adam_f4& m4, adam_f4& v4) {
+  const adam_f4 g4 = graw * coef;
+  p4 = praw * (1.0f - lr * wd);
+  m4 = a.beta1 * mraw + (1.0f - a.beta1) * g4;
+  v4 = a.beta2 * vraw + (1.0f - a.beta2) * g4 * g4;
+#pragma unroll
+  for (int e = 0; e < 4; ++e) p4[e] -= step_size * (m4[e] / (sqrtf(v4[e]) / a.bc2_sqrt + a.eps));
+}
+__device__ __forceinline__ void adam_update1(const AdamArgs& a, float lr, float wd, float coef, float step_size, float graw,
+                                             float& pi, float& mi, float& vi) {
+  const float gi = graw * coef;
+  pi = pi * (1.0f - lr * wd);
+  mi = a.beta1 * mi + (1.0f - a.beta1) * gi;
+  vi = a.beta2 * vi + (1.0f - a.beta2) * gi * gi;
+  const float denom = sqrtf(vi) / a.bc2_sqrt + a.eps;
+  pi -= step_size * (mi / denom);
+}
+
+__device__ __forceinline__ void adamw_tiles(const AdamArgs& a, int item) {
+  __shared__ float tile[64][65];
+  const int32_t* d = a.tile_desc + 4 * (int64_t)item;
+  const int t = d[0], r0 = d[1] * 64, ct0 = d[2], nct = d[3];
+  const int R = a.t_dims[4 * t], C = a.t_dims[4 * t + 1], ldT = a.t_dims[4 * t + 2], roff = a.t_dims[4 * t + 3];
+  float* p = reinterpret_cast<float*>(a.p_ptrs[t]);
+  const float* g = reinterpret_cast<const float*>(a.g_ptrs[t]);
+  float* m = reinterpret_cast<float*>(a.m_ptrs[t]);
+  float* v = reinterpret_cast<float*>(a.v_ptrs[t]);
+  bf16_t* sh = a.bf16_ptrs && a.bf16_ptrs[t] ? reinterpret_cast<bf16_t*>(a.bf16_ptrs[t]) : nullptr;
+  bf16_t* dstT = reinterpret_cast<bf16_t*>(a.t_ptrs[t]);
+  const int grp = a.group_of[t];
+  const float lr = a.lr[grp], wd = a.wd[grp];
+  float coef = 1.0f;
+  if (a.max_norm > 0.f && a.sumsq) {
+    const float tn = (float)sqrt(*a.sumsq);
+    coef = fminf(1.0f, a.max_norm / (tn + 1e-6f));
+  }
+  const float step_size = lr / a.bc1;
+  const bool vec = (C & 3) == 0 &&
+      ((reinterpret_cast<uintptr_t>(p) | reinterpret_cast<uintptr_t>(g) | reinterpret_cast<uintptr_t>(m) | reinterpret_cast<uintptr_t>(v)) & 15) == 0 &&
+      (!sh || (reinterpret_cast<uintptr_t>(sh) & 7) == 0);
+  const bool vecT = (ldT & 7) == 0 && (roff & 7) == 0 && (reinterpret_cast<uintptr_t>(dstT) & 15) == 0;
+  const int tid = threadIdx.x;
+  for (int ct = ct0; ct < ct0 + nct; ++ct) {
+    const int c0 = ct * 64;
+    if (vec) {
+#pragma unroll
+      for (int it = 0; it < 4; ++it) {
+        const int idx = it * 256 + tid, r = idx >> 4, c = (idx & 15) * 4;
+        const int gr = r0 + r, gc = c0 + c;
+        if (gr < R && gc < C) {
+          const int64_t i = ((int64_t)gr * C + gc) >> 2;
+          adam_f4 p4, m4, v4;
+          adam_update4(a, lr, wd, coef, step_size, __builtin_nontemporal_load(reinterpret_cast<const adam_f4*>(g) + i),
+                       reinterpret_cast<const adam_f4*>(p)[i], __builtin_nontemporal_load(reinterpret_cast<const adam_f4*>(m) + i),
+                       __builtin_nontemporal_load(reinterpret_cast<const adam_f4*>(v) + i), p4, m4, v4);
+          reinterpret_cast<adam_f4*>(p)[i] = p4;
+          __builtin_nontemporal_store(m4, reinterpret_cast<adam_f4*>(m) + i);
+          __builtin_nontemporal_store(v4, reinterpret_cast<adam_f4*>(v) + i);
+          if (sh) {
+            bf16x4 o;
+            o[0] = (bf16_t)p4[0]; o[1] = (bf16_t)p4[1]; o[2] = (bf16_t)p4[2]; o[3] = (bf16_t)p4[3];
+            reinterpret_cast<bf16x4*>(sh)[i] = o;
+          }
+          tile[r][c] = p4[0]; tile[r][c + 1] = p4[1]; tile[r][c + 2] = p4[2]; tile[r][c + 3] = p4[3];
+        }
+      }
+    } else {
+      for (int it = 0; it < 16; ++it) {
+        const int idx = it * 256 + tid, r = idx >> 6, c = idx & 63;
+        const int gr = r0 + r, gc = c0 + c;
+        if (gr < R && gc < C) {
+          const int64_t i = (int64_t)gr * C + gc;
+          float pi = p[i], mi = m[i], vi = v[i];
+          adam_update1(a, lr, wd, coef, step_size, g[i], pi, mi, vi);
+          p[i] = pi; m[i] = mi; v[i] = vi;
+          if (sh) sh[i] = (bf16_t)pi;
+          tile[r][c] = pi;
+        }
+      }
+    }
+    __syncthreads();
+    if (vecT) {
+#pragma unroll
+      for (int it = 0; it < 2; ++it) {
+        const int idx = it * 256 + tid, cc = idx >> 3, rr = (idx & 7) * 8;
+        const int gc = c0 + cc, gr = r0 + rr;
+        if (gc < C && gr < R) {
+          bf16_t* o = dstT + (int64_t)gc * ldT + roff + gr;
+          if (gr + 8 <= R) {
+            bf16x8 w;
+#pragma unroll
+            for (int j = 0; j < 8; ++j) w[j] = (bf16_t)tile[rr + j][cc];
+            *reinterpret_cast<bf16x8*>(o) = w;
+          } else {
+            for (int j = 0; gr + j < R; ++j) o[j] = (bf16_t)tile[rr + j][cc];
+          }
+        }
+      }
+    } else {
+      const int tx = tid & 63, ty = tid >> 6;
+#pragma unroll
+      for (int i = 0; i < 16; ++i) {
+        const int gc = c0 + ty * 16 + i, gr = r0 + tx;
+        if (gc < C && gr < R) dstT[(int64_t)gc * ldT + roff + gr] = (bf16_t)tile[tx][ty * 16 + i];
+      }
+    }
+    __syncthreads();
+  }
+}
+
 __global__ __launch_bounds__(256) void multi_adamw_kernel(AdamArgs a) {
+  if ((int)blockIdx.x >= a.nflat) {
+    adamw_tiles(a, blockIdx.x - a.nflat);
+    return;
+  }
   const int t = a.chunk_tensor[blockIdx.x];
   const int64_t off = a.chunk_offset[blockIdx.x];
   float* p = reinterpret_cast<float*>(a.p_ptrs[t]) + off;
@@ -342,18 +463,16 @@
     coef = fminf(1.0f, a.max_norm / (tn + 1e-6f));
   }
   const float step_size = lr / a.bc1;
-  typedef float f4 __attribute__((ext_vector_type(4)));
+  typedef adam_f4 f4;
   int64_t i0 = 0;
   if (((reinterpret_cast<uintptr_t>(p) | reinterpret_cast<uintptr_t>(g) | reinterpret_cast<uintptr_t>(m) | reinterpret_cast<uintptr_t>(v)) & 15) == 0 &&
       (!sh || (reinterpret_cast<uintptr_t>(sh) & 7) == 0)) {
     const int64_t n4 = n >> 2;
     for (int64_t i = threadIdx.x; i < n4; i += 256) {
-      const f4 g4 = __builtin_nontemporal_load(reinterpret_cast<const f4*>(g) + i) * coef;
-      f4 p4 = reinterpret_cast<const f4*>(p)[i] * (1.0f - lr * wd);
-      const f4 m4 = a.beta1 * __builtin_nontemporal_load(reinterpret_cast<const f4*>(m) + i) + (1.0f - a.beta1) * g4;
-      const f4 v4 = a.beta2 * __builtin_nontemporal_load(reinterpret_cast<const f4*>(v) + i) + (1.0f - a.beta2) * g4 * g4;
-#pragma unroll
-      for (int e = 0; e < 4; ++e) p4[e] -= step_size * (m4[e] / (sqrtf(v4[e]) / a.bc2_sqrt + a.eps));
+      f4 p4, m4, v4;
+      adam_update4(a, lr, wd, coef, step_size, __builtin_nontemporal_load(reinterpret_cast<const f4*>(g) + i),
+                   reinterpret_cast<const f4*>(p)[i], __builtin_nontemporal_load(reinterpret_cast<const f4*>(m) + i),
+                   __builtin_nontemporal_load(reinterpret_cast<const f4*>(v) + i), p4, m4, v4);
       reinterpret_cast<f4*>(p)[i] = p4;
       __builtin_nontemporal_store(m4, reinterpret_cast<f4*>(m) + i);
       __builtin_nontemporal_store(v4, reinterpret_cast<f4*>(v) + i);
@@ -366,12 +485,8 @@
     i0 = n4 << 2;
   }
   for (int64_t i = i0 + threadIdx.x; i < n; i += 256) {
-    const float gi = g[i] * coef;
-    float pi = p[i] * (1.0f - lr * wd);
-    const float mi = a.beta1 * m[i] + (1.0f - a.beta1) * gi;
-    const float vi = a.beta2 * v[i] + (1.0f - a.beta2) * gi * gi;
-    const float denom = sqrtf(vi) / a.bc2_sqrt + a.eps;
-    pi -= step_size * (mi / denom);
+    float pi = p[i], mi = m[i], vi = v[i];
+    adam_update1(a, lr, wd, coef, step_size, g[i], pi, mi, vi);
     p[i] = pi; m[i] = mi; v[i] = vi;
     if (sh) sh[i] = (bf16_t)pi;
   }
@@ -673,15 +788,17 @@
   return FCMF_OK;
 }
 
-extern "C" int fcmf_multi_adamw(const int64_t* p_ptrs, const int64_t* g_ptrs, const int64_t* m_ptrs, const int64_t* v_ptrs,
-                                const int64_t* bf16_ptrs, const int64_t* sizes, const int32_t* group_of,
-                                const int32_t* chunk_tensor, const int64_t* chunk_offset, int nchunks, int chunk_size,
-                                const float* lr, const float* wd, int ngroups, float beta1, float beta2, float eps, int step,
-                                const double* sumsq, float max_norm, void* stream) {
-  if (!p_ptrs || !g_ptrs || !m_ptrs || !v_ptrs || !sizes || !group_of || !chunk_tensor || !chunk_offset || !lr || !wd)
-    return FCMF_ERR_ARG;
-  if (ngroups <= 0 || ngroups > 8 || step < 1 || chunk_size <= 0 || nchunks < 0) return FCMF_ERR_ARG;
-  if (nchunks == 0) return FCMF_OK;
+static int multi_adamw_impl(const int64_t* p_ptrs, const int64_t* g_ptrs, const int64_t* m_ptrs, const int64_t* v_ptrs,
+                            const int64_t* bf16_ptrs, const int64_t* sizes, const int32_t* group_of,
+                            const int32_t* chunk_tensor, const int64_t* chunk_offset, int nchunks, int chunk_size,
+                            const float* lr, const float* wd, int ngroups, float beta1, float beta2, float eps, int step,
+                            const double* sumsq, float max_norm, const int64_t* t_ptrs, const int32_t* t_dims,
+                            const int32_t* tile_desc, int ntiles, void* stream) {
+  if (!p_ptrs || !g_ptrs || !m_ptrs || !v_ptrs || !sizes || !group_of || !lr || !wd) return FCMF_ERR_ARG;
+  if (nchunks > 0 && (!chunk_tensor || !chunk_offset)) return FCMF_ERR_ARG;
+  if (ntiles > 0 && (!t_ptrs || !t_dims || !tile_desc)) return FCMF_ERR_ARG;
+  if (ngroups <= 0 || ngroups > 8 || step < 1 || chunk_size <= 0 || nchunks < 0 || ntiles < 0) return FCMF_ERR_ARG;
+  if (nchunks + ntiles == 0) return FCMF_OK;
   AdamArgs a{};
   a.p_ptrs = p_ptrs; a.g_ptrs = g_ptrs; a.m_ptrs = m_ptrs; a.v_ptrs = v_ptrs; a.bf16_ptrs = bf16_ptrs; a.sizes = sizes;
   a.group_of = group_of; a.chunk_tensor = chunk_tensor; a.chunk_offset = chunk_offset; a.chunk_size = chunk_size;
@@ -690,9 +807,30 @@
   a.bc1 = (float)(1.0 - pow((double)beta1, (double)step));
   a.bc2_sqrt = (float)sqrt(1.0 - pow((double)beta2, (double)step));
   a.sumsq = sumsq; a.max_norm = max_norm;
-  hipLaunchKernelGGL(multi_adamw_kernel, dim3(nchunks), dim3(256), 0, reinterpret_cast<hipStream_t>(stream), a);
-  FCMF_CHECK_LAUNCH();
-  return FCMF_OK;
+  a.nflat = nchunks; a.t_ptrs = t_ptrs; a.t_dims = t_dims; a.tile_desc = tile_desc;
+  hipLaunchKernelGGL(multi_adamw_kernel, dim3(nchunks + ntiles), dim3(256), 0, reinterpret_cast<hipStream_t>(stream), a);
+  FCMF_CHECK_LAUNCH();
+  return FCMF_OK;
+}
+
+extern "C" int fcmf_multi_adamw(const int64_t* p_ptrs, const int64_t* g_ptrs, const int64_t* m_ptrs, const int64_t* v_ptrs,
+                                const int64_t* bf16_ptrs, const int64_t* sizes, const int32_t* group_of,
+                                const int32_t* chunk_tensor, const int64_t* chunk_offset, int nchunks, int chunk_size,
+                                const float* lr, const float* wd, int ngroups, float beta1, float beta2, float eps, int step,
+                                const double* sumsq, float max_norm, void* stream) {
+  if (!chunk_tensor || !chunk_offset) return FCMF_ERR_ARG;
+  return multi_adamw_impl(p_ptrs, g_ptrs, m_ptrs, v_ptrs, bf16_ptrs, sizes, group_of, chunk_tensor, chunk_offset, nchunks, chunk_size,
+                          lr, wd, ngroups, beta1, beta2, eps, step, sumsq, max_norm, nullptr, nullptr, nullptr, 0, stream);
+}
+
+extern "C" int fcmf_multi_adamw_wt(const int64_t* p_ptrs, const int64_t* g_ptrs, const int64_t* m_ptrs, const int64_t* v_ptrs,
+                                   const int64_t* bf16_ptrs, const int64_t* sizes, const int32_t* group_of,
+                                   const int32_t* chunk_tensor, const int64_t* chunk_offset, int nchunks, int chunk_size,
+                                   const float* lr, const float* wd, int ngroups, float beta1, float beta2, float eps, int step,
+                                   const double* sumsq, float max_norm, const int64_t* t_ptrs, const int32_t* t_dims,
+                                   const int32_t* tile_desc, int ntiles, void* stream) {
+  return multi_adamw_impl(p_ptrs, g_ptrs, m_ptrs, v_ptrs, bf16_ptrs, sizes, group_of, chunk_tensor, chunk_offset, nchunks, chunk_size,
+                          lr, wd, ngroups, beta1, beta2, eps, step, sumsq, max_norm, t_ptrs, t_dims, tile_desc, ntiles, stream);
 }
 
 extern "C" int fcmf_bertadam(float* p, const float* g, float* m, float* v, int64_t n, float lr_scheduled, float beta1,
diff --git a/multimodal-aspect-category-sentiment-analysis_amd/csrc/norm.hip b/multimodal-aspect-category-sentiment-analysis_amd/csrc/norm.hip
--- a/multimodal-aspect-category-sentiment-analysis_amd/csrc/norm.hip
+++ b/multimodal-aspect-category-sentiment-analysis_amd/csrc/norm.hip
@@ -251,22 +251,48 @@
   }
 }
 
-__global__ __launch_bounds__(256) void ln_partial_reduce_kernel(const float* __restrict__ partial, int nblocks, int H,
-                                                                float* __restrict__ dgamma, float* __restrict__ dbeta,
-                                                                float* __restrict__ dxsum) {
-  __shared__ float red[4][64];
+__device__ __forceinline__ void ln_partial_reduce_body(const float* __restrict__ partial, int nblocks, int H,
+                                                       float* __restrict__ out, int colblock, int which, int zi, int nz,
+                                                       float (*red)[64]) {
   const int lane = threadIdx.x & 63, w = threadIdx.x >> 6;
-  const int col = blockIdx.x * 64 + lane, which = blockIdx.y;
-  float* out = which == 0 ? dgamma : (which == 1 ? dbeta : dxsum);
-  if (!out) return;
-  const int per = (nblocks + gridDim.z - 1) / gridDim.z;
-  const int b0 = blockIdx.z * per, b1 = min(nblocks, b0 + per);
+  const int col = colblock * 64 + lane;
+  const int per = (nblocks + nz - 1) / nz;
+  const int b0 = zi * per, b1 = min(nblocks, b0 + per);
   float s = 0.f;
   if (col < H)
     for (int b = b0 + w; b < b1; b += 4) s += partial[((int64_t)b * 3 + which) * H + col];
   red[w][lane] = s;
   __syncthreads();
   if (w == 0 && col < H) atomicAdd(out + col, red[0][lane] + red[1][lane] + red[2][lane] + red[3][lane]);
+}
+
+constexpr int LN_REDUCE_Z = 8;
+
+__global__ __launch_bounds__(256) void ln_partial_reduce_kernel(const float* __restrict__ partial, int nblocks, int H,
+                                                                float* __restrict__ dgamma, float* __restrict__ dbeta,
+                                                                float* __restrict__ dxsum) {
+  __shared__ float red[4][64];
+  const int which = blockIdx.y;
+  float* out = which == 0 ? dgamma : (which == 1 ? dbeta : dxsum);
+  if (!out) return;
+  ln_partial_reduce_body(partial, nblocks, H, out, blockIdx.x, which, blockIdx.z, gridDim.z, red);
+}
+
+constexpr int LN_REDUCE_BATCH = 64;
+struct LnReduceBatch {
+  const float* partial[LN_REDUCE_BATCH];
+  float* out[3][LN_REDUCE_BATCH];
+  int nblocks[LN_REDUCE_BATCH];
+  int H[LN_REDUCE_BATCH];
+};
+
+__global__ __launch_bounds__(256) void ln_partial_reduce_batched_kernel(LnReduceBatch t) {
+  __shared__ float red[4][64];
+  const int e = blockIdx.y, which = blockIdx.z / LN_REDUCE_Z, zi = blockIdx.z % LN_REDUCE_Z;
+  float* out = t.out[which][e];
+  const int H = t.H[e];
+  if (!out || (int)blockIdx.x * 64 >= H) return;
+  ln_partial_reduce_body(t.partial[e], t.nblocks[e], H, out, blockIdx.x, which, zi, LN_REDUCE_Z, red);
 }
 
 __global__ __launch_bounds__(64) void position_ids_kernel(const int64_t* __restrict__ ids, int64_t* __restrict__ pos,
@@ -520,7 +546,7 @@
 
 static int add_ln_bwd_impl(const void* dy, const void* z, const float* gamma, const float* mean, const float* rstd, void* dz,
                            void* dx, float* dgamma, float* dbeta, float* dxsum, float* workspace, int rows, int H,
-                           float dropout_p, uint64_t seed, int dtype, void* stream, void* q8, float* qscale);
+                           float dropout_p, uint64_t seed, int dtype, void* stream, void* q8, float* qscale, bool reduce = true);
 extern "C" int fcmf_add_ln_bwd(const void* dy, const void* z, const float* gamma, const float* mean, const float* rstd,
                                void* dz, void* dx, float* dgamma, float* dbeta, float* dxsum, float* workspace,
                                int rows, int H, float dropout_p, uint64_t seed, int dtype, void* stream) {
@@ -534,8 +560,9 @@
 }
 static int add_ln_bwd_impl(const void* dy, const void* z, const float* gamma, const float* mean, const float* rstd, void* dz,
                            void* dx, float* dgamma, float* dbeta, float* dxsum, float* workspace, int rows, int H,
-                           float dropout_p, uint64_t seed, int dtype, void* stream, void* q8, float* qscale) {
-  if (!dy || !z || !gamma || !mean || !rstd || !dz || !dgamma || !dbeta || rows < 0 || H <= 0) return FCMF_ERR_ARG;
+                           float dropout_p, uint64_t seed, int dtype, void* stream, void* q8, float* qscale, bool reduce) {
+  if (!dy || !z || !gamma || !mean || !rstd || !dz || (reduce && (!dgamma || !dbeta)) || rows < 0 || H <= 0) return FCMF_ERR_ARG;
+  if (!reduce && !workspace) return FCMF_ERR_ARG;
   if (H % 4 != 0 || H > LN_MAXP * 256) return FCMF_ERR_UNSUPPORTED;
   if (dropout_p > 0.f && !dx) return FCMF_ERR_ARG;
   if (rows == 0) return FCMF_OK;
@@ -547,8 +574,53 @@
     (unsigned char*)q8, qscale)
   LN_DISPATCH(dtype, H);
 #undef LAUNCH_
-  if (workspace)
-    hipLaunchKernelGGL(ln_partial_reduce_kernel, dim3((H + 63) / 64, 3, 8), dim3(256), 0, st, workspace, blocks, H, dgamma, dbeta, dxsum);
+  if (workspace && reduce)
+    hipLaunchKernelGGL(ln_partial_reduce_kernel, dim3((H + 63) / 64, 3, LN_REDUCE_Z), dim3(256), 0, st, workspace, blocks, H, dgamma, dbeta, dxsum);
+  FCMF_CHECK_LAUNCH();
+  return FCMF_OK;
+}
+
+extern "C" int fcmf_add_ln_bwd_partials(const void* dy, const void* z, const float* gamma, const float* mean, const float* rstd,
+                                        void* dz, void* dx, float* workspace, int rows, int H, float dropout_p, uint64_t seed,
+                                        int dtype, void* stream) {
+  return add_ln_bwd_impl(dy, z, gamma, mean, rstd, dz, dx, nullptr, nullptr, nullptr, workspace, rows, H, dropout_p, seed, dtype,
+                         stream, nullptr, nullptr, false);
+}
+
+extern "C" int fcmf_ln_partial_reduce_batched(const fcmf_ln_reduce_entry* entries, int n, void* stream) {
+  if (n < 0 || (n > 0 && !entries)) return FCMF_ERR_ARG;
+  for (int i = 0; i < n; ++i) {
+    const fcmf_ln_reduce_entry& e = entries[i];
+    if (!e.partial || e.nblocks <= 0 || e.H <= 0 || !e.dgamma || !e.dbeta) return FCMF_ERR_ARG;
+  }
+  hipStream_t st = reinterpret_cast<hipStream_t>(stream);
+  for (int i = 0; i < n; ++i) {
+    const fcmf_ln_reduce_entry& e = entries[i];
+    if (e.accumulate) continue;
+    float* outs[3] = {e.dgamma, e.dbeta, e.dxsum};
+    for (float* o : outs)
+      if (o && hipMemsetAsync(o, 0, sizeof(float) * e.H, st) != hipSuccess) return FCMF_ERR_LAUNCH;
+  }
+  int i0 = 0;
+  while (i0 < n) {
+    LnReduceBatch t{};
+    int k = 0, maxH = 0;
+    for (; i0 + k < n && k < LN_REDUCE_BATCH; ++k) {
+      const fcmf_ln_reduce_entry& e = entries[i0 + k];
+      const float* mine[3] = {e.dgamma, e.dbeta, e.dxsum};
+      bool clash = false;
+      for (int j = 0; j < k && !clash; ++j)
+        for (int a = 0; a < 3 && !clash; ++a)
+          for (int b = 0; b < 3; ++b)
+            if (mine[a] && mine[a] == t.out[b][j]) { clash = true; break; }
+      if (clash) break;
+      t.partial[k] = e.partial; t.out[0][k] = e.dgamma; t.out[1][k] = e.dbeta; t.out[2][k] = e.dxsum;
+      t.nblocks[k] = e.nblocks; t.H[k] = e.H;
+      if (e.H > maxH) maxH = e.H;
+    }
+    hipLaunchKernelGGL(ln_partial_reduce_batched_kernel, dim3((maxH + 63) / 64, k, 3 * LN_REDUCE_Z), dim3(256), 0, st, t);
+    i0 += k;
+  }
   FCMF_CHECK_LAUNCH();
   return FCMF_OK;
 }
diff --git a/multimodal-aspect-category-sentiment-analysis_amd/fcmf_framework/_hip.py b/multimodal-aspect-category-sentiment-analysis_amd/fcmf_framework/_hip.py
--- a/multimodal-aspect-category-sentiment-analysis_amd/fcmf_framework/_hip.py
+++ b/multimodal-aspect-category-sentiment-analysis_amd/fcmf_framework/_hip.py
@@ -24,6 +24,15 @@
         ("mask", _vp), ("bias", _vp),
         ("scale", _f), ("dropout_p", _f), ("seed", _u64), ("causal", _i), ("head_quirk", _i),
     ]
+
+
+class LnReduceEntry(ctypes.Structure):
+    _fields_ = [("partial", _vp), ("dgamma", _vp), ("dbeta", _vp), ("dxsum", _vp), ("nblocks", _i), ("H", _i),
+                ("accumulate", _i), ("reserved", _i)]
+
+
+class ColsumEntry(ctypes.Structure):
+    _fields_ = [("X", _vp), ("out", _vp), ("ldx", _i64), ("M", _i), ("N", _i), ("accumulate", _i), ("reserved", _i)]
 
 
 class CropDesc(ctypes.Structure):
@@ -46,6 +55,7 @@
     "fcmf_quant_fp8_rows": [_vp, _i64, _vp, _i64, _vp, _i, _i, _i, _vp],
     "fcmf_gemm_fp8": [_vp, _vp, _vp, _vp, _vp, _vp, _vp, _vp, _vp, _i, _i, _i, _i64, _i64, _i64, _i, _vp],
     "fcmf_colsum": [_vp, _vp, _i, _i, _i64, _i, _i, _vp],
+    "fcmf_colsum_batched": [_vp, _i, _vp],
     "fcmf_attn_small_fwd": [_c.POINTER(AttnDesc), _vp, _vp, _vp],
     "fcmf_attn_small_bwd": [_c.POINTER(AttnDesc), _vp, _vp, _vp, _vp, _vp, _vp, _vp, _vp, _vp, _vp],
     "fcmf_attn_small_bwd_grouped": [_c.POINTER(AttnDesc), _vp, _vp, _vp, _vp, _vp, _vp, _vp, _vp, _vp, _vp, _i64, _vp],
@@ -59,6 +69,8 @@
     "fcmf_add_ln_fwd_fp8": [_vp, _vp, _i64, _vp, _vp, _vp, _vp, _vp, _vp, _i, _i, _f, _f, _u64, _i, _vp, _vp, _vp],
     "fcmf_add_ln_bwd_fp8": [_vp, _vp, _vp, _vp, _vp, _vp, _vp, _vp, _vp, _vp, _vp, _i, _i, _f, _u64, _i, _vp, _vp, _vp],
     "fcmf_add_ln_bwd_workspace": [_i, _i],
+    "fcmf_add_ln_bwd_partials": [_vp, _vp, _vp, _vp, _vp, _vp, _vp, _vp, _i, _i, _f, _u64, _i, _vp],
+    "fcmf_ln_partial_reduce_batched": [_vp, _i, _vp],
     "fcmf_position_ids": [_vp, _vp, _i, _i, _i, _vp],
     "fcmf_embed_ln_fwd": [_vp, _vp, _vp, _vp, _vp, _vp, _vp, _vp, _vp, _vp, _vp, _vp, _i, _i, _f, _f, _u64, _i, _vp],
     "fcmf_embed_bwd": [_vp, _vp, _vp, _vp, _vp, _vp, _vp, _i, _i, _i, _i, _vp],
@@ -85,6 +97,8 @@
     "fcmf_multi_sumsq": [_vp, _vp, _vp, _vp, _i, _i, _vp, _vp, _vp],
     "fcmf_multi_adamw": [_vp, _vp, _vp, _vp, _vp, _vp, _vp, _vp, _vp, _i, _i, _c.POINTER(_f), _c.POINTER(_f), _i, _f, _f,
                          _f, _i, _vp, _f, _vp],
+    "fcmf_multi_adamw_wt": [_vp, _vp, _vp, _vp, _vp, _vp, _vp, _vp, _vp, _i, _i, _c.POINTER(_f), _c.POINTER(_f), _i, _f, _f,
+                            _f, _i, _vp, _f, _vp, _vp, _vp, _i, _vp],
     "fcmf_bertadam": [_vp, _vp, _vp, _vp, _i64, _f, _f, _f, _f, _f, _f, _vp, _vp],
     "fcmf_conv_im2col": [_vp, _i, _vp, _i, _i, _i, _i, _i, _i64, _i64, _i64, _i64, _i, _i, _i, _i, _i, _vp],
     "fcmf_bn_stats": [_vp, _vp, _i64, _i, _i, _i, _vp],
diff --git a/multimodal-aspect-category-sentiment-analysis_amd/fcmf_framework/fused.py b/multimodal-aspect-category-sentiment-analysis_amd/fcmf_framework/fused.py
--- a/multimodal-aspect-category-sentiment-analysis_amd/fcmf_framework/fused.py
+++ b/multimodal-aspect-category-sentiment-analysis_amd/fcmf_framework/fused.py
@@ -140,7 +140,7 @@
                                      db, db + Hd * es, db + 2 * Hd * es, G, heads, T, T, 3 * Hd, 3 * Hd, Hd, scale, p, seed,
                                      H.ptr(part), H.stream()), "fcmf_attn_mfma_bwd")
         if part is not None:
-            H.check(L.fcmf_colsum(H.ptr(part), H.ptr(bias_grad), G, 3 * Hd, 3 * Hd, H.dt(part), 1, H.stream()), "fcmf_colsum")
+            ops.colsum_partials(part, bias_grad)
         return dqkv
     a = _qkv_desc(qkv, G, T, Hd, heads, mask, scale, p, seed)
     nch = max(1, (T + 127) // 128)
@@ -181,16 +181,16 @@
 def _ln_bwd(dy, z, g, mean, rstd, p, seed, dg, db, dxsum, quant=False):
     dz = torch.empty_like(z)
     dx = torch.empty_like(z) if p > 0 else None
-    ws = ops.ln_workspace(z.shape[0], z.shape[1], z.device)
     if quant:
+        ws = ops.ln_workspace(z.shape[0], z.shape[1], z.device)
+        if ops.deferred_reduce.holds(dg, db, dxsum):
+            ops.deferred_reduce.flush(final=False)
         q, sc = _q_buffers(z.shape[0], z.shape[1], z.device)
         H.check(H.lib().fcmf_add_ln_bwd_fp8(H.ptr(dy), H.ptr(z), H.ptr(g), H.ptr(mean), H.ptr(rstd), H.ptr(dz), H.ptr(dx), H.ptr(dg),
                                             H.ptr(db), H.ptr(dxsum), H.ptr(ws), z.shape[0], z.shape[1], p, seed, H.dt(z), H.ptr(q),
                                             H.ptr(sc), H.stream()), "fcmf_add_ln_bwd_fp8")
         return dz, (dx if dx is not None else dz), (q, sc)
-    H.check(H.lib().fcmf_add_ln_bwd(H.ptr(dy), H.ptr(z), H.ptr(g), H.ptr(mean), H.ptr(rstd), H.ptr(dz), H.ptr(dx), H.ptr(dg),
-                                    H.ptr(db), H.ptr(dxsum), H.ptr(ws), z.shape[0], z.shape[1], p, seed, H.dt(z), H.stream()),
-            "fcmf_add_ln_bwd")
+    ops.ln_bwd(dy, z, g, mean, rstd, dz, dx, dg, db, dxsum, p, seed)
     return dz, (dx if dx is not None else dz), None
 
 
diff --git a/multimodal-aspect-category-sentiment-analysis_amd/fcmf_framework/ops.py b/multimodal-aspect-category-sentiment-analysis_amd/fcmf_framework/ops.py
--- a/multimodal-aspect-category-sentiment-analysis_amd/fcmf_framework/ops.py
+++ b/multimodal-aspect-category-sentiment-analysis_amd/fcmf_framework/ops.py
@@ -77,6 +77,7 @@
         self.mapQT = {}
         self.mapH = {}
         self._mt_tables = None
+        self.t_rebuilds = 0
 
     def get_t(self, w, owner=None):
         key = (w.data_ptr(), tuple(w.shape))
@@ -88,6 +89,7 @@
         src = w.detach()
         if not src.is_contiguous():
             src = src.contiguous()
+        self.t_rebuilds += 1
         H.check(H.lib().fcmf_cast_transpose(H.ptr(src), H.ptr(sh), w.shape[0], w.shape[1], H.stream()), "fcmf_cast_transpose")
         self.mapT[key] = [sh, w._version, False, w.is_contiguous(), weakref.ref(owner), w.data_ptr() - owner.data_ptr()]
         return sh
@@ -103,11 +105,42 @@
         if dead:
             self._mt_tables = None
 
-    def refresh_transposed(self):
+    def transposed_by_param(self, params):
+        self._prune_transposed()
+        by_ptr = {p.data_ptr(): i for i, p in enumerate(params)}
+        out = {}
+        for k, ent in self.mapT.items():
+            if not ent[3] or len(k) != 2:
+                continue
+            R, C = k[1]
+            ptr, r, idxs = k[0], 0, []
+            while r < R:
+                i = by_ptr.get(ptr)
+                if i is None or i in out:
+                    break
+                q = params[i]
+                if q.dim() != 2 or q.shape[1] != C or not q.is_contiguous() or q.dtype != torch.float32 or r + q.shape[0] > R:
+                    break
+                idxs.append((i, r))
+                r += q.shape[0]
+                ptr += q.numel() * 4
+            if r == R and idxs:
+                for i, r0 in idxs:
+                    out[i] = (k, ent[0], R, r0)
+        return out
+
+    def mark_transposed_fresh(self, keys):
+        for k in keys:
+            ent = self.mapT.get(k)
+            if ent is not None and ent[4]() is not None:
+                ent[2] = False
+                ent[1] = ent[4]()._version
+
+    def refresh_transposed(self, skip=()):
         if not self.mapT:
             return
         self._prune_transposed()
-        items = [(k, ent) for k, ent in self.mapT.items() if ent[3]]
+        items = [(k, ent) for k, ent in self.mapT.items() if ent[3] and k not in skip]
         if not items:
             return
         sig = tuple((k[0], ent[0].data_ptr()) for k, ent in items)
@@ -123,6 +156,7 @@
                                torch.tensor([list(k[1]) for k, _ in items], dtype=torch.int32, device=dev),
                                torch.tensor(desc, dtype=torch.int32, device=dev), len(desc))
         _, src, dst, dims, desc, n = self._mt_tables
+        self.t_rebuilds += 1
         H.check(H.lib().fcmf_multi_cast_transpose(H.ptr(src), H.ptr(dst), H.ptr(dims), H.ptr(desc), n, H.stream()),
                 "fcmf_multi_cast_transpose")
         for _, ent in items:
@@ -257,6 +291,8 @@
     _grad_arena = arena
     if arena is not None and deferred_dw.reset not in arena.on_zero:
         arena.on_zero.append(deferred_dw.reset)
+    if arena is not None and deferred_reduce.reset not in arena.on_zero:
+        arena.on_zero.append(deferred_reduce.reset)
 
 
 def grad_arena():
@@ -435,6 +471,131 @@
 def flush_deferred_dw(lo=None, hi=None):
     if deferred_dw.q:
         deferred_dw.flush(final=False, lo=lo, hi=hi)
+    flush_deferred_reduce(lo, hi)
+
+
+DEFER_LN_REDUCE = os.environ.get("FCMF_DEFER_LN_REDUCE", "1") == "1"
+
+
+class _PartialPool:
+
+    def __init__(self):
+        self.buf, self.off, self.need = None, 0, 0
+
+    def take(self, n, device):
+        n = (n + 63) // 64 * 64
+        self.need += n
+        if self.buf is not None and self.buf.device == device and self.off + n <= self.buf.numel():
+            t = self.buf[self.off:self.off + n]
+            self.off += n
+            return t
+        return torch.empty(n, dtype=torch.float32, device=device)
+
+    def rewind(self, device):
+        if self.need and (self.buf is None or self.buf.device != device or self.need > self.buf.numel()):
+            self.buf = torch.empty(self.need, dtype=torch.float32, device=device)
+        self.off = self.need = 0
+
+
+class _DeferredReduce:
+    def __init__(self):
+        self.q, self.armed, self.pool = [], False, _PartialPool()
+        self.batched_calls = self.batched_entries = 0
+
+    def reset(self):
+        dev = self.q[0][1].device if self.q else None
+        self.q, self.armed = [], False
+        if dev is not None:
+            self.pool.rewind(dev)
+
+    def wanted(self, *dests):
+        arena = _grad_arena
+        if not DEFER_LN_REDUCE or arena is None or not arena.flat.is_cuda:
+            return False
+        lo = arena.flat.data_ptr()
+        hi = lo + arena.flat.numel() * 4
+        for d in dests:
+            if d is not None and not (d.dtype == torch.float32 and d.device == arena.flat.device and lo <= d.data_ptr() < hi):
+                return False
+        if not self.armed:
+            try:
+                torch.autograd.Variable._execution_engine.queue_callback(self.flush)
+            except RuntimeError:
+                return False
+            self.armed = True
+        return True
+
+    def push_ln(self, part, nblocks, Hd, dg, db, dxsum):
+        self.q.append(("ln", part, nblocks, Hd, dg.data_ptr(), db.data_ptr(), 0 if dxsum is None else dxsum.data_ptr()))
+
+    def push_colsum(self, part, M, N, out):
+        self.q.append(("cs", part, M, N, out.data_ptr()))
+
+    def holds(self, *dests):
+        if not self.q:
+            return False
+        ptrs = {d.data_ptr() for d in dests if d is not None}
+        return any(not ptrs.isdisjoint(e[4:]) for e in self.q)
+
+    def flush(self, final=True, lo=None, hi=None):
+        if lo is not None:
+            q = [e for e in self.q if any(lo <= d < hi for d in e[4:] if d)]
+            self.q = [e for e in self.q if not any(lo <= d < hi for d in e[4:] if d)]
+        else:
+            q, self.q = self.q, []
+        if final:
+            self.armed = False
+        if not q:
+            return
+        dev = q[0][1].device
+        ln = [e for e in q if e[0] == "ln"]
+        cs = [e for e in q if e[0] == "cs"]
+        with torch.cuda.device(dev):
+            if ln:
+                arr = (H.LnReduceEntry * len(ln))(*[H.LnReduceEntry(e[1].data_ptr(), e[4], e[5], e[6] or None, e[2], e[3], 1, 0) for e in ln])
+                H.check(H.lib().fcmf_ln_partial_reduce_batched(arr, len(ln), H.stream()), "fcmf_ln_partial_reduce_batched")
+            if cs:
+                arr = (H.ColsumEntry * len(cs))(*[H.ColsumEntry(e[1].data_ptr(), e[4], e[3], e[2], e[3], 1, 0) for e in cs])
+                H.check(H.lib().fcmf_colsum_batched(arr, len(cs), H.stream()), "fcmf_colsum_batched")
+        self.batched_calls += bool(ln) + bool(cs)
+        self.batched_entries += len(q)
+        if not self.q:
+            self.pool.rewind(dev)
+
+
+deferred_reduce = _DeferredReduce()
+
+
+def flush_deferred_reduce(lo=None, hi=None):
+    if deferred_reduce.q:
+        deferred_reduce.flush(final=False, lo=lo, hi=hi)
+
+
+def ln_bwd(dy, z, gamma, mean, rstd, dz, dx, dg, db, dxsum, p, seed):
+    rows, Hd = z.shape
+    L = H.lib()
+    if rows > 0 and deferred_reduce.wanted(dg, db, dxsum):
+        n = L.fcmf_add_ln_bwd_workspace(rows, Hd)
+        ws = deferred_reduce.pool.take(n, z.device)
+        H.check(L.fcmf_add_ln_bwd_partials(H.ptr(dy), H.ptr(z), H.ptr(gamma), H.ptr(mean), H.ptr(rstd), H.ptr(dz), H.ptr(dx), H.ptr(ws),
+                                           rows, Hd, p, seed, H.dt(z), H.stream()), "fcmf_add_ln_bwd_partials")
+        deferred_reduce.push_ln(ws, n // (3 * Hd), Hd, dg, db, dxsum)
+        return
+    if deferred_reduce.holds(dg, db, dxsum):
+        deferred_reduce.flush(final=False)
+    H.check(L.fcmf_add_ln_bwd(H.ptr(dy), H.ptr(z), H.ptr(gamma), H.ptr(mean), H.ptr(rstd), H.ptr(dz), H.ptr(dx), H.ptr(dg), H.ptr(db),
+                              H.ptr(dxsum), H.ptr(ln_workspace(rows, Hd, z.device)), rows, Hd, p, seed, H.dt(z), H.stream()),
+            "fcmf_add_ln_bwd")
+
+
+def colsum_partials(part, out):
+    M, N = part.shape
+    if M > 0 and deferred_reduce.wanted(out):
+        deferred_reduce.push_colsum(part, M, N, out)
+        return
+    if deferred_reduce.holds(out):
+        deferred_reduce.flush(final=False)
+    H.check(H.lib().fcmf_colsum(H.ptr(part), H.ptr(out), M, N, N, H.dt(part), 1, H.stream()), "fcmf_colsum")
 
 
 def gemm(A, B, C, M, N, K, lda, ldb, ldc, ta, tb, bias=None, aux=None, epi=H.EPI_NONE, acc=False, colsum=None):
@@ -901,9 +1062,7 @@
         dx = torch.empty_like(z) if ctx.p > 0 else None
         dgbuf, dg = grad_dest(gamma, (Hd,))
         dbbuf, db = grad_dest(beta, (Hd,))
-        H.check(H.lib().fcmf_add_ln_bwd(H.ptr(dy2), H.ptr(z), H.ptr(gamma), H.ptr(mean), H.ptr(rstd), H.ptr(dz),
-                                        H.ptr(dx), H.ptr(dgbuf), H.ptr(dbbuf), 0, H.ptr(ln_workspace(rows, Hd, z.device)), rows, Hd, ctx.p, ctx.seed, H.dt(z),
-                                        H.stream()), "fcmf_add_ln_bwd")
+        ln_bwd(dy2, z, gamma, mean, rstd, dz, dx, dgbuf, dbbuf, None, ctx.p, ctx.seed)
         dxo = (dx if dx is not None else dz).view(ctx.xshape)
         dres = None if ctx.res_shape is None else dz.view(ctx.res_shape)
         return dxo, dres, dg, db, None, None, None
diff --git a/multimodal-aspect-category-sentiment-analysis_amd/fcmf_framework/optimization.py b/multimodal-aspect-category-sentiment-analysis_amd/fcmf_framework/optimization.py
--- a/multimodal-aspect-category-sentiment-analysis_amd/fcmf_framework/optimization.py
+++ b/multimodal-aspect-category-sentiment-analysis_amd/fcmf_framework/optimization.py
@@ -1,5 +1,6 @@
 import ctypes
 import math
+import os
 
 import torch
 from torch.optim import Optimizer
@@ -106,6 +107,9 @@
         return loss
 
 
+ADAMW_WT = os.environ.get("FCMF_ADAMW_WT", "1") == "1"
+
+
 class FusedAdamW(Optimizer):
     CHUNK = 65536
 
@@ -143,6 +147,36 @@
             ct=torch.tensor(ct, dtype=torch.int32, device=device), co=i64(co), nchunks=len(ct),
             pptr=[p.data_ptr() for p, _ in plist],
             mvptr=[(self.state[p]['exp_avg'].data_ptr(), self.state[p]['exp_avg_sq'].data_ptr()) for p, _ in plist])
+
+    def _plan_transposed(self, plist, T, device):
+        params = [p for p, _ in plist]
+        cover = ops.shadows.transposed_by_param(params)
+        ok = lambda i: all(a % 16 == 0 for a in (T['pptr'][i], T['gl'][i]) + T['mvptr'][i]) and params[i].shape[1] % 4 == 0 \
+            and T['sl'][i] % 8 == 0
+        bad = {cover[i][0] for i in cover if not ok(i)}
+        cover = {i: c for i, c in cover.items() if c[0] not in bad}
+        sig = tuple(sorted((i, c[0], c[1].data_ptr()) for i, c in cover.items())) + (tuple(T['gl']), tuple(T['sl']))
+        W = T.get('wt')
+        if W is not None and W['sig'] == sig:
+            return W
+        i64 = lambda xs: torch.tensor(xs, dtype=torch.int64, device=device)
+        i32 = lambda xs: torch.tensor(xs, dtype=torch.int32, device=device)
+        ct, co, tiles = [], [], []
+        t_ptrs, t_dims = [0] * len(params), [[0, 0, 0, 0] for _ in params]
+        for i, p in enumerate(params):
+            c = cover.get(i)
+            if c is None:
+                for off in range(0, p.numel(), self.CHUNK):
+                    ct.append(i)
+                    co.append(off)
+                continue
+            R, C = p.shape
+            t_ptrs[i], t_dims[i] = c[1].data_ptr(), [R, C, c[2], c[3]]
+            nct = (C + 63) // 64
+            tiles += [[i, tr, c0, min(4, nct - c0)] for tr in range((R + 63) // 64) for c0 in range(0, nct, 4)]
+        W = T['wt'] = dict(sig=sig, keys={c[0] for c in cover.values()}, ct=i32(ct or [0]), co=i64(co or [0]), nchunks=len(ct),
+                           t_ptrs=i64(t_ptrs), t_dims=i32(t_dims), tiles=i32(tiles or [[0, 0, 0, 0]]), ntiles=len(tiles))
+        return W
 
     def load_state_dict(self, state_dict):
         super().load_state_dict(state_dict)
@@ -200,12 +234,23 @@
         wd = (ctypes.c_float * 8)(*[float(g['weight_decay']) for g in self.param_groups] + [0.0] * (8 - ng))
         b1, b2 = self.param_groups[0]['betas']
         eps = self.param_groups[0]['eps']
-        H.check(L.fcmf_multi_adamw(H.ptr(T['p']), H.ptr(g_ptrs), H.ptr(T['m']), H.ptr(T['v']), H.ptr(sh_ptrs),
-                                   H.ptr(T['sizes']), H.ptr(T['group']), H.ptr(T['ct']), H.ptr(T['co']), T['nchunks'],
-                                   self.CHUNK, lr, wd, ng, b1, b2, eps, step, H.ptr(self._sumsq), mg, st),
-                "fcmf_multi_adamw")
+        W = self._plan_transposed(plist, T, device) if ADAMW_WT and ops.shadows.mapT else None
+        if W is not None and W['ntiles']:
+            H.check(L.fcmf_multi_adamw_wt(H.ptr(T['p']), H.ptr(g_ptrs), H.ptr(T['m']), H.ptr(T['v']), H.ptr(sh_ptrs),
+                                          H.ptr(T['sizes']), H.ptr(T['group']), H.ptr(W['ct']), H.ptr(W['co']), W['nchunks'],
+                                          self.CHUNK, lr, wd, ng, b1, b2, eps, step, H.ptr(self._sumsq), mg,
+                                          H.ptr(W['t_ptrs']), H.ptr(W['t_dims']), H.ptr(W['tiles']), W['ntiles'], st),
+                    "fcmf_multi_adamw_wt")
+            done = W['keys']
+        else:
+            H.check(L.fcmf_multi_adamw(H.ptr(T['p']), H.ptr(g_ptrs), H.ptr(T['m']), H.ptr(T['v']), H.ptr(sh_ptrs),
+                                       H.ptr(T['sizes']), H.ptr(T['group']), H.ptr(T['ct']), H.ptr(T['co']), T['nchunks'],
+                                       self.CHUNK, lr, wd, ng, b1, b2, eps, step, H.ptr(self._sumsq), mg, st),
+                    "fcmf_multi_adamw")
+            done = ()
         ops.shadows.mark_all_stale()
-        ops.shadows.refresh_transposed()
+        ops.shadows.mark_transposed_fresh(done)
+        ops.shadows.refresh_transposed(skip=done)
         for (p, _), s in zip(plist, sh):
             self.state[p]['step'] = step
             if s is not None:
```

Measured after the change: 1722 samples/s. 1.2% lower.
